# BoyBaykiller/IDKEngine

Measured on NVIDIA H100. Metric: Mrays/s Sponza-sized synthetic 1920x1080 8-bounce, higher is better.
Workload: dtype f32

## Files before the change

### idkengine_b200/csrc/idk_kernels.cuh

```cuda
#pragma once
#include "idk_device.cuh"
#include "../../include/idk_gpu_types.h"

#define IDK_BLOCK 256
#define IDK_WARPS (IDK_BLOCK / 32)
#define IDK_T2_BLOCK 256

struct DeviceScene {
    const float4* nodes;
    const float4* triRec;
    const int4* blasTris;
    const GpuBlasDesc* descs;
    const GpuBlasInstance* instances;
    const float4* xforms;
    const GpuMesh* meshes;
    const GpuMaterial* materials;
    const uint4* vertices;
    const GpuLight* lights;
    uint32_t instanceCount;
    uint32_t lightCount;
    float skyR, skyG, skyB;
    int stackSize;
    const float4* skyFaces;
    int skyFaceSize;
    const float4* tlasNodes;
    int useTlas;
    const float4* vtxFrame;
    const float4* surfRec;
    const struct TexRec* textures;
    uint32_t textureCount;
    const float* srgbLut;
};


#define IDK_TLAS_STACK_SIZE 24

struct __align__(16) PathState {
    float ox, oy, oz, prevIor;
    float pdx, pdy;
    uint32_t pix;
    uint32_t reseed;
    float tx, ty, tz;
    uint32_t rng;
    float rx, ry, rz;
    uint32_t pad;
};
static_assert(sizeof(PathState) == 64, "PathState must be 64 bytes");

struct HitRec { float bx, by, t; uint32_t tri; };

struct TraceCounters { unsigned long long steps, tris, instances, hits; unsigned int maxSteps[64]; };

__global__ void k_init_sample(uint32_t* counts, int nCounts, uint32_t* tickets, int nTickets, uint32_t primaryRays) {
    for (int i = threadIdx.x; i < nCounts; i += blockDim.x) counts[i] = i == 0 ? primaryRays : 0u;
    for (int i = threadIdx.x; i < nTickets; i += blockDim.x) tickets[i] = 0u;
}

__global__ void k_prepare_triangles(const int4* __restrict__ tris, const float* __restrict__ positions,
                                    float4* __restrict__ triRec, uint32_t count) {
    uint32_t i = blockIdx.x * blockDim.x + threadIdx.x;
    if (i >= count) return;
    int4 t = tris[i];
    f3 p0 = mk3(positions[3 * t.x], positions[3 * t.x + 1], positions[3 * t.x + 2]);
    f3 p1 = mk3(positions[3 * t.y], positions[3 * t.y + 1], positions[3 * t.y + 2]);
    f3 p2 = mk3(positions[3 * t.z], positions[3 * t.z + 1], positions[3 * t.z + 2]);
    f3 e1 = p1 - p0, e2 = p2 - p0;
    f3 n = cross3(e1, e2);
    triRec[4 * (size_t)i + 0] = make_float4(p0.x, p0.y, p0.z, e1.x);
    triRec[4 * (size_t)i + 1] = make_float4(e1.y, e1.z, e2.x, e2.y);
    triRec[4 * (size_t)i + 2] = make_float4(e2.z, n.x, n.y, n.z);
    triRec[4 * (size_t)i + 3] = make_float4(0.0f, 0.0f, 0.0f, 0.0f);
}

__global__ void k_prepare_vertices(const uint4* __restrict__ vertices, float4* __restrict__ vtxFrame, uint32_t count) {
    const uint32_t i = blockIdx.x * blockDim.x + threadIdx.x;
    if (i >= count) return;
    const uint4 v = vertices[i];
    const f3 n = decompress_sr11g11b10(v.w), t = decompress_sr11g11b10(v.z);
    vtxFrame[2 * (size_t)i] = make_float4(n.x, n.y, n.z, t.x);
    vtxFrame[2 * (size_t)i + 1] = make_float4(t.y, t.z, 0.0f, 0.0f);
}

__global__ void k_prepare_surfaces(const GpuMesh* __restrict__ meshes, const GpuMaterial* __restrict__ materials,
                                   float4* __restrict__ surfRec, uint32_t meshCount) {
    const uint32_t i = blockIdx.x * blockDim.x + threadIdx.x;
    if (i >= meshCount) return;
    const GpuMesh& mesh = meshes[i];
    const GpuMaterial& mat = materials[mesh.MaterialId];
    const uint32_t c = mat.BaseColorFactor;
    const f3 albedo = mk3((float)(c & 255u) / 255.0f, (float)((c >> 8) & 255u) / 255.0f, (float)((c >> 16) & 255u) / 255.0f);
    const float alpha = (float)((c >> 24) & 255u) / 255.0f;
    f3 emissive = mk3(mat.EmissiveFactor[0], mat.EmissiveFactor[1], mat.EmissiveFactor[2]);
    emissive = emissive * 1.0f + mesh.EmissiveBias * albedo;
    const f3 ab = mk3(mat.Absorbance[0], mat.Absorbance[1], mat.Absorbance[2]) + mk3(mesh.AbsorbanceBias[0], mesh.AbsorbanceBias[1], mesh.AbsorbanceBias[2]);
    const f3 absorbance = mk3(fmaxf(ab.x, 0.0f), fmaxf(ab.y, 0.0f), fmaxf(ab.z, 0.0f));
    const float metallic = clamp1(mat.MetallicFactor + mesh.SpecularBias, 0.0f, 1.0f);
    const float roughness = clamp1(mat.RoughnessFactor + mesh.RoughnessBias, 0.0f, 1.0f);
    const float transmission = clamp1(mat.TransmissionFactor + mesh.TransmissionBias, 0.0f, 1.0f);
    const float ior = fmaxf(mat.IOR + mesh.IORBias, 1.0f);
    const bool textured = (mat.BaseColorTexture | mat.MetallicRoughnessTexture | mat.NormalTexture | mat.EmissiveTexture | mat.TransmissionTexture) != 0;
    const uint32_t flags = (mat.IsVolumetric != 0 ? 1u : 0u) | (mesh.TintOnTransmissive != 0 ? 2u : 0u) | (textured ? 4u : 0u);
    float4* o = surfRec + 5 * (size_t)i;
    o[0] = make_float4(albedo.x, albedo.y, albedo.z, alpha);
    o[1] = make_float4(emissive.x, emissive.y, emissive.z, metallic);
    o[2] = make_float4(absorbance.x, absorbance.y, absorbance.z, roughness);
    o[3] = make_float4(transmission, ior, mat.AlphaCutoff, mesh.NormalMapStrength);
    o[4] = make_float4(__uint_as_float(flags), 0.0f, 0.0f, 0.0f);
}

struct AcceptAll {
    __device__ __forceinline__ bool operator()(const DeviceScene&, uint32_t, float, float, float) const { return true; }
    __device__ __forceinline__ AcceptAll at(const DeviceScene&, uint32_t, f3) const { return *this; }
};
template <bool STATS, bool ANY, class Accept = AcceptAll>
__device__ __forceinline__ bool intersect_blas(const DeviceScene& sc, const float4* nodes, uint32_t triOffset, f3 lo, f3 ld, f3 inv,
                                               bool rootTest, uint32_t* stack, HitRec& hit, uint32_t& S, uint32_t& T, float& cost,
                                               const Accept& accept = Accept()) {
    float tMinLeft, tMinRight;
    if (rootTest) {
        const float4 a = ldg4(nodes + 2), b = ldg4(nodes + 3);
        if (!(ray_box(lo, inv, a, b, tMinLeft) && tMinLeft < hit.t)) return false;
    }
    bool blasHit = false;
    uint32_t sp = 0;
    uint32_t top = 2;
    while (true) {
        if (STATS) { S++; cost += 1.0f; }
        const NodePair pr = ldg_pair(nodes + 2 * (size_t)top);
        const float4 lA = pr.lA, lB = pr.lB, rA = pr.rA, rB = pr.rB;
        const int lChild = __float_as_int(lA.w), lCount = __float_as_int(lB.w);
        const int rChild = __float_as_int(rA.w), rCount = __float_as_int(rB.w);

        const bool hitLeft = ray_box(lo, inv, lA, lB, tMinLeft) && tMinLeft <= hit.t;
        const bool hitRight = ray_box(lo, inv, rA, rB, tMinRight) && tMinRight <= hit.t;

        const bool intersectLeft = hitLeft && lCount > 0;
        const bool intersectRight = hitRight && rCount > 0;
        if (intersectLeft || intersectRight) {
            uint32_t first = intersectLeft ? (uint32_t)lChild : (uint32_t)rChild;
            uint32_t end = !intersectRight ? (uint32_t)(lChild + lCount) : (uint32_t)(rChild + rCount);
            first += triOffset;
            end += triOffset;
            if (STATS) { T += end - first; cost += (float)(end - first) * 1.1f; }
            for (uint32_t i = first; i < end; i++) {
                float4 a, b, c;
                ldg_tri(sc.triRec, i, a, b, c);
                float bx, by, t;
                if (ray_triangle(lo, ld, mk3(a.x, a.y, a.z), mk3(a.w, b.x, b.y), mk3(b.z, b.w, c.x), mk3(c.y, c.z, c.w), bx, by, t) && t < hit.t && accept(sc, i, bx, by, t)) {
                    blasHit = true;
                    hit.tri = i;
                    hit.bx = bx;
                    hit.by = by;
                    hit.t = t;
                    if (ANY) return true;
                }
            }
        }

        const bool traverseLeft = hitLeft && lCount == 0;
        const bool traverseRight = hitRight && rCount == 0;
        if (traverseLeft || traverseRight) {
            if (traverseLeft && traverseRight) {
                const bool leftFirst = ANY || tMinLeft < tMinRight;
                top = leftFirst ? (uint32_t)lChild : (uint32_t)rChild;
                stack[(sp++) * IDK_BLOCK] = leftFirst ? (uint32_t)rChild : (uint32_t)lChild;
            } else {
                top = traverseLeft ? (uint32_t)lChild : (uint32_t)rChild;
            }
        } else {
            if (sp == 0) break;
            top = stack[(--sp) * IDK_BLOCK];
        }
    }
    return blasHit;
}

template <bool STATS, bool ANY, class Accept = AcceptAll>
__device__ __forceinline__ bool trace_instance(const DeviceScene& sc, uint32_t inst, f3 o, f3 d, bool rootTest, uint32_t* stack,
                                               HitRec& hit, uint32_t& hitXform, uint32_t& S, uint32_t& T, uint32_t& I, float& cost,
                                               const Accept& accept = Accept()) {
    const GpuBlasInstance bi = sc.instances[inst];
    const int nodeOffset = sc.descs[bi.BlasId].NodeOffset;
    const uint32_t triOffset = (uint32_t)sc.descs[bi.BlasId].TriangleOffset;
    const float4* xf = sc.xforms + 9 * (size_t)bi.MeshTransformId + 3;
    const float4 r0 = ldg4(xf), r1 = ldg4(xf + 1), r2 = ldg4(xf + 2);
    const f3 lo = xform_point(r0, r1, r2, o);
    const f3 ld = xform_vector(r0, r1, r2, d);
    const f3 inv = mk3(1.0f / ld.x, 1.0f / ld.y, 1.0f / ld.z);
    if (STATS) I++;
    if (!intersect_blas<STATS, ANY>(sc, sc.nodes + 2 * (size_t)nodeOffset, triOffset, lo, ld, inv, rootTest, stack, hit, S, T, cost,
                                    accept.at(sc, bi.MeshTransformId, ld))) return false;
    hitXform = bi.MeshTransformId;
    return true;
}

template <bool STATS, bool ANY, class Accept = AcceptAll>
__device__ __forceinline__ bool trace_ray(const DeviceScene& sc, f3 o, f3 d, float tMax, bool traceLights,
                                          uint32_t* stack, HitRec& hit, uint32_t& hitXform, uint32_t& S, uint32_t& T, uint32_t& I, float& cost,
                                          const Accept& accept = Accept()) {
    hit.t = tMax;
    hit.tri = ~0u;
    hit.bx = 0.0f;
    hit.by = 0.0f;
    hitXform = 0;

    if (traceLights) {
        for (uint32_t i = 0; i < sc.lightCount; i++) {
            const GpuLight& L = sc.lights[i];
            float tMin, tMx;
            if (ray_sphere(o, d, mk3(L.Position[0], L.Position[1], L.Position[2]), L.Radius, tMin, tMx) && tMin < hit.t) {
                hit.t = tMin < 0.0f ? tMx : tMin;
                hitXform = i;
                hit.tri = ~0u;
                if (ANY) return true;
            }
        }
    }

    if (sc.useTlas) {
        const f3 inv = mk3(1.0f / d.x, 1.0f / d.y, 1.0f / d.z);
        uint32_t tstack[IDK_TLAS_STACK_SIZE];
        uint32_t sp = 0, top = 0;
        while (true) {
            const float4 pA = ldg4(sc.tlasNodes + 2 * (size_t)top);
            const uint32_t word = __float_as_uint(pA.w);
            const uint32_t id = word & 0x7FFFFFFFu;
            if (word >> 31) {
                const bool instHit = trace_instance<STATS, ANY>(sc, id, o, d, false, stack, hit, hitXform, S, T, I, cost, accept);
                if (ANY && instHit) return true;
                if (sp == 0) break;
                top = tstack[--sp];
                continue;
            }
            const NodePair pr = ldg_pair(sc.tlasNodes + 2 * (size_t)id);
            const float4 lA = pr.lA, lB = pr.lB, rA = pr.rA, rB = pr.rB;
            float tMinLeft, tMinRight;
            const bool traverseLeft = ray_box(o, inv, lA, lB, tMinLeft) && tMinLeft < hit.t;
            const bool traverseRight = ray_box(o, inv, rA, rB, tMinRight) && tMinRight < hit.t;
            if (traverseLeft || traverseRight) {
                if (traverseLeft && traverseRight) {
                    const bool leftCloser = tMinLeft < tMinRight;
                    top = leftCloser ? id : id + 1;
                    tstack[sp++] = leftCloser ? id + 1 : id;
                } else {
                    top = traverseLeft ? id : id + 1;
                }
            } else {
                if (sp == 0) break;
                top = tstack[--sp];
            }
        }
    } else {
        for (uint32_t inst = 0; inst < sc.instanceCount; inst++) {
            const bool instHit = trace_instance<STATS, ANY>(sc, inst, o, d, true, stack, hit, hitXform, S, T, I, cost, accept);
            if (ANY && instHit) return true;
        }
    }
    return !ANY && hit.t != tMax;
}

struct TraverseArgs {
    DeviceScene sc;
    const PathState* state;
    const uint32_t* perm;
    const uint32_t* count;
    uint32_t* ticket;
    HitRec* hits;
    uint32_t* hitXform;
    float* debugCost;
    TraceCounters* counters;
    int traceLights;
    int bounce;
};

template <bool STATS>
__global__ void __launch_bounds__(IDK_BLOCK) k_traverse(TraverseArgs a) {
    extern __shared__ uint32_t s_stack[];
    uint32_t* stack = s_stack + threadIdx.x;
    const uint32_t lane = threadIdx.x & 31;
    const uint32_t count = *a.count;
    uint32_t S = 0, T = 0, I = 0, H = 0;
    for (;;) {
        uint32_t base = 0;
        if (lane == 0) base = atomicAdd(a.ticket, 32u);
        base = __shfl_sync(0xffffffffu, base, 0);
        if (base >= count) break;
        const uint32_t gid = base + lane;
        if (gid < count) {
            const uint32_t src = a.perm ? a.perm[gid] : gid;
            const float4* sp = reinterpret_cast<const float4*>(a.state + src);
            const float4 s0 = sp[0], s1 = sp[1];
            const f3 o = mk3(s0.x, s0.y, s0.z);
            const f3 d = decode_unit_vec(s1.x, s1.y);
            HitRec hit;
            uint32_t xf;
            float cost = 0.0f;
            const uint32_t stepsBefore = S;
            trace_ray<STATS, false>(a.sc, o, d, IDK_FLOAT_MAX, a.traceLights != 0, stack, hit, xf, S, T, I, cost);
            if (STATS) atomicMax(&a.counters->maxSteps[a.bounce & 63], S - stepsBefore);
            reinterpret_cast<float4*>(a.hits)[gid] = make_float4(hit.bx, hit.by, hit.t, __uint_as_float(hit.tri));
            a.hitXform[gid] = xf;
            if (STATS) {
                a.debugCost[gid] = cost;
                if (hit.tri != ~0u) H++;
            }
        }
    }
    if (STATS) {
        for (int off = 16; off > 0; off >>= 1) {
            S += __shfl_down_sync(0xffffffffu, S, off);
            T += __shfl_down_sync(0xffffffffu, T, off);
            I += __shfl_down_sync(0xffffffffu, I, off);
            H += __shfl_down_sync(0xffffffffu, H, off);
        }
        if (lane == 0) {
            atomicAdd(&a.counters->steps, (unsigned long long)S);
            atomicAdd(&a.counters->tris, (unsigned long long)T);
            atomicAdd(&a.counters->instances, (unsigned long long)I);
            atomicAdd(&a.counters->hits, (unsigned long long)H);
        }
    }
}


struct TraverseTuning { int setupThreshold; int leafThreshold; int packRays; };
#define IDK_T2_SETUP_THRESHOLD 12
#define IDK_T2_LEAF_THRESHOLD 4

template <bool STATS, bool TLAS>
__global__ void __launch_bounds__(IDK_T2_BLOCK) k_traverse2(TraverseArgs a, TraverseTuning tune) {
    extern __shared__ __align__(128) unsigned char s_dyn[];
    const DeviceScene& sc = a.sc;
    uint32_t* stack = reinterpret_cast<uint32_t*>(s_dyn) + threadIdx.x;
    const uint32_t lane = threadIdx.x & 31;
    const uint32_t laneLt = (1u << lane) - 1u;
    const uint32_t count = *a.count;
    enum { ST_SETUP = 0, ST_BOX = 1, ST_LEAF = 2, ST_EXIT = 3, ST_TLAS = 4 };
    const uint32_t totalWarps = gridDim.x * (IDK_T2_BLOCK / 32);
    const uint32_t quota = tune.packRays ? 32u : min(32u, max(1u, (count + totalWarps - 1) / totalWarps));
    const int setupThreshold = max(1, min(tune.setupThreshold, (int)(quota * 3 / 8)));
    const int leafThreshold = max(1, min(tune.leafThreshold, (int)(quota / 8)));

    int state = ST_SETUP;
    bool haveRay = false, finished = false, blasHit = false;
    uint32_t gid = 0, inst = 0, curXf = 0, hitXf = 0;
    f3 wo = mk3(0, 0, 0), wd = mk3(0, 0, 1);
    f3 lo = wo, ld = wd, inv = wd;
    HitRec hit;
    hit.bx = hit.by = 0.0f; hit.t = 0.0f; hit.tri = ~0u;
    const float4* nodes = sc.nodes;
    uint32_t triOffset = 0, top = 2, sp = 0, first = 0, end = 0;
    uint32_t S = 0, T = 0, I = 0, H = 0, rayS0 = 0;
    float cost = 0.0f;
    uint32_t tstack[TLAS ? IDK_TLAS_STACK_SIZE : 1];
    uint32_t tsp = 0, ttop = 0;
    f3 winv = wd;

    for (;;) {
        const uint32_t mBox = __ballot_sync(0xffffffffu, state == ST_BOX);
        const uint32_t mSetup = __ballot_sync(0xffffffffu, state == ST_SETUP);
        const uint32_t mLeaf = __ballot_sync(0xffffffffu, state == ST_LEAF);
        const uint32_t mTlas = TLAS ? __ballot_sync(0xffffffffu, state == ST_TLAS) : 0u;
        if ((mSetup | mBox | mLeaf | mTlas) == 0u) break;

        if (mSetup && (__popc(mSetup) >= setupThreshold || (mBox | mLeaf | mTlas) == 0u)) {
            const bool mine = state == ST_SETUP;
            if (mine && haveRay && inst >= sc.instanceCount) {
                reinterpret_cast<float4*>(a.hits)[gid] = make_float4(hit.bx, hit.by, hit.t, __uint_as_float(hit.tri));
                a.hitXform[gid] = hitXf;
                if (STATS) {
                    a.debugCost[gid] = cost;
                    if (hit.tri != ~0u) H++;
                    atomicMax(&a.counters->maxSteps[a.bounce & 63], S - rayS0);
                }
                haveRay = false;
            }
            const bool needFetch = mine && !haveRay && lane < quota;
            if (mine && !haveRay && lane >= quota) state = ST_EXIT;
            const uint32_t fm = __ballot_sync(0xffffffffu, needFetch);
            if (fm) {
                const int leader = __ffs(fm) - 1;
                uint32_t base = 0;
                if ((int)lane == leader) base = atomicAdd(a.ticket, (uint32_t)__popc(fm));
                base = __shfl_sync(0xffffffffu, base, leader);
                bool got = false;
                float4 s0 = make_float4(0.0f, 0.0f, 0.0f, 0.0f), s1 = s0;
                if (needFetch) {
                    gid = base + __popc(fm & laneLt);
                    if (gid < count) {
                        const uint32_t src = a.perm ? a.perm[gid] : gid;
                        const float4* spp = reinterpret_cast<const float4*>(a.state + src);
                        s0 = spp[0]; s1 = spp[1];
                        got = true;
                    }
                }
                if (needFetch) {
                    if (got) {
                        wo = mk3(s0.x, s0.y, s0.z);
                        wd = decode_unit_vec(s1.x, s1.y);
                        hit.t = IDK_FLOAT_MAX; hit.tri = ~0u; hit.bx = 0.0f; hit.by = 0.0f;
                        hitXf = 0;
                        cost = 0.0f;
                        if (a.traceLights) {
                            for (uint32_t i = 0; i < sc.lightCount; i++) {
                                const GpuLight& L = sc.lights[i];
                                float tMin, tMx;
                                if (ray_sphere(wo, wd, mk3(L.Position[0], L.Position[1], L.Position[2]), L.Radius, tMin, tMx) && tMin < hit.t) {
                                    hit.t = tMin < 0.0f ? tMx : tMin;
                                    hitXf = i;
                                    hit.tri = ~0u;
                                }
                            }
                        }
                        inst = 0;
                        haveRay = true;
                        rayS0 = S;
                        if (TLAS) {
                            winv = mk3(1.0f / wd.x, 1.0f / wd.y, 1.0f / wd.z);
                            ttop = 0; tsp = 0;
                            state = ST_TLAS;
                        }
                    } else {
                        state = ST_EXIT;
                    }
                }
            }
            if (!TLAS && mine && haveRay && inst < sc.instanceCount) {
                const GpuBlasInstance bi = sc.instances[inst];
                const int nodeOffset = sc.descs[bi.BlasId].NodeOffset;
                triOffset = (uint32_t)sc.descs[bi.BlasId].TriangleOffset;
                const float4* xf = sc.xforms + 9 * (size_t)bi.MeshTransformId + 3;
                const float4 r0 = ldg4(xf), r1 = ldg4(xf + 1), r2 = ldg4(xf + 2);
                lo = xform_point(r0, r1, r2, wo);
                ld = xform_vector(r0, r1, r2, wd);
                inv = mk3(1.0f / ld.x, 1.0f / ld.y, 1.0f / ld.z);
                nodes = sc.nodes + 2 * (size_t)nodeOffset;
                curXf = bi.MeshTransformId;
                if (STATS) I++;
                const float4 ra = ldg4(nodes + 2), rb = ldg4(nodes + 3);
                float tRoot;
                if (ray_box(lo, inv, ra, rb, tRoot) && tRoot < hit.t) {
                    state = ST_BOX;
                    top = 2; sp = 0; blasHit = false; finished = false;
                } else {
                    inst++;
                }
            }
        } else if (TLAS && mTlas && (__popc(mTlas) >= setupThreshold || (mBox | mLeaf) == 0u)) {
            if (state == ST_TLAS) {
                const float4 pA = ldg4(sc.tlasNodes + 2 * (size_t)ttop);
                const uint32_t word = __float_as_uint(pA.w);
                const uint32_t id = word & 0x7FFFFFFFu;
                if (word >> 31) {
                    const GpuBlasInstance bi = sc.instances[id];
                    const int nodeOffset = sc.descs[bi.BlasId].NodeOffset;
                    triOffset = (uint32_t)sc.descs[bi.BlasId].TriangleOffset;
                    const float4* xf = sc.xforms + 9 * (size_t)bi.MeshTransformId + 3;
                    const float4 r0 = ldg4(xf), r1 = ldg4(xf + 1), r2 = ldg4(xf + 2);
                    lo = xform_point(r0, r1, r2, wo);
                    ld = xform_vector(r0, r1, r2, wd);
                    inv = mk3(1.0f / ld.x, 1.0f / ld.y, 1.0f / ld.z);
                    nodes = sc.nodes + 2 * (size_t)nodeOffset;
                    curXf = bi.MeshTransformId;
                    if (STATS) I++;
                    state = ST_BOX;
                    top = 2; sp = 0; blasHit = false; finished = false;
                } else {
                    const NodePair pr = ldg_pair(sc.tlasNodes + 2 * (size_t)id);
                    float tMinLeft, tMinRight;
                    const bool traverseLeft = ray_box(wo, winv, pr.lA, pr.lB, tMinLeft) && tMinLeft < hit.t;
                    const bool traverseRight = ray_box(wo, winv, pr.rA, pr.rB, tMinRight) && tMinRight < hit.t;
                    if (traverseLeft || traverseRight) {
                        if (traverseLeft && traverseRight) {
                            const bool leftCloser = tMinLeft < tMinRight;
                            ttop = leftCloser ? id : id + 1;
                            tstack[tsp++] = leftCloser ? id + 1 : id;
                        } else {
                            ttop = traverseLeft ? id : id + 1;
                        }
                    } else if (tsp == 0u) {
                        inst = 0xFFFFFFFFu;
                        state = ST_SETUP;
                    } else {
                        ttop = tstack[--tsp];
                    }
                }
            }
        } else if (mLeaf && (__popc(mLeaf) >= leafThreshold || mBox == 0u)) {
            if (state == ST_LEAF) {
                float4 ta, tb, tc;
                ldg_tri(sc.triRec, first, ta, tb, tc);
                float bx, by, t;
                if (ray_triangle(lo, ld, mk3(ta.x, ta.y, ta.z), mk3(ta.w, tb.x, tb.y), mk3(tb.z, tb.w, tc.x), mk3(tc.y, tc.z, tc.w), bx, by, t) && t < hit.t) {
                    blasHit = true;
                    hit.tri = first; hit.bx = bx; hit.by = by; hit.t = t;
                }
                first++;
                if (first == end) {
                    if (finished) {
                        if (blasHit) hitXf = curXf;
                        if (TLAS) {
                            if (tsp == 0u) { inst = 0xFFFFFFFFu; state = ST_SETUP; }
                            else { ttop = tstack[--tsp]; state = ST_TLAS; }
                        } else { inst++; state = ST_SETUP; }
                    } else {
                        state = ST_BOX;
                    }
                }
            }
        } else {
            if (state == ST_BOX) {
                if (STATS) { S++; cost += 1.0f; }
                const NodePair pr = ldg_pair(nodes + 2 * (size_t)top);
                const float4 lA = pr.lA, lB = pr.lB, rA = pr.rA, rB = pr.rB;
                const int lChild = __float_as_int(lA.w), lCount = __float_as_int(lB.w);
                const int rChild = __float_as_int(rA.w), rCount = __float_as_int(rB.w);
                float tMinLeft, tMinRight;
                const bool hitLeft = ray_box(lo, inv, lA, lB, tMinLeft) && tMinLeft <= hit.t;
                const bool hitRight = ray_box(lo, inv, rA, rB, tMinRight) && tMinRight <= hit.t;
                const bool intersectLeft = hitLeft && lCount > 0;
                const bool intersectRight = hitRight && rCount > 0;
                bool pending = false;
                if (intersectLeft || intersectRight) {
                    first = (intersectLeft ? (uint32_t)lChild : (uint32_t)rChild) + triOffset;
                    end = (!intersectRight ? (uint32_t)(lChild + lCount) : (uint32_t)(rChild + rCount)) + triOffset;
                    if (STATS) { T += end - first; cost += (float)(end - first) * 1.1f; }
                    pending = first < end;
                }
                const bool traverseLeft = hitLeft && lCount == 0;
                const bool traverseRight = hitRight && rCount == 0;
                if (traverseLeft || traverseRight) {
                    if (traverseLeft && traverseRight) {
                        const bool leftCloser = tMinLeft < tMinRight;
                        top = leftCloser ? (uint32_t)lChild : (uint32_t)rChild;
                        stack[(sp++) * IDK_T2_BLOCK] = leftCloser ? (uint32_t)rChild : (uint32_t)lChild;
                    } else {
                        top = traverseLeft ? (uint32_t)lChild : (uint32_t)rChild;
                    }
                } else if (sp == 0u) {
                    finished = true;
                } else {
                    top = stack[(--sp) * IDK_T2_BLOCK];
                }
                if (pending) {
                    state = ST_LEAF;
                } else if (finished) {
                    if (blasHit) hitXf = curXf;
                    if (TLAS) {
                        if (tsp == 0u) { inst = 0xFFFFFFFFu; state = ST_SETUP; }
                        else { ttop = tstack[--tsp]; state = ST_TLAS; }
                    } else { inst++; state = ST_SETUP; }
                }
            }
        }
    }
    if (STATS) {
        for (int off = 16; off > 0; off >>= 1) {
            S += __shfl_down_sync(0xffffffffu, S, off);
            T += __shfl_down_sync(0xffffffffu, T, off);
            I += __shfl_down_sync(0xffffffffu, I, off);
            H += __shfl_down_sync(0xffffffffu, H, off);
        }
        if (lane == 0) {
            atomicAdd(&a.counters->steps, (unsigned long long)S);
            atomicAdd(&a.counters->tris, (unsigned long long)T);
            atomicAdd(&a.counters->instances, (unsigned long long)I);
            atomicAdd(&a.counters->hits, (unsigned long long)H);
        }
    }
}

struct TraceRaysArgs {
    DeviceScene sc;
    const float4* rays;
    uint4* hits;
    uint32_t count;
    uint32_t* ticket;
    int traceLights;
};

__global__ void __launch_bounds__(IDK_BLOCK) k_trace_rays(TraceRaysArgs a) {
    extern __shared__ uint32_t s_stack[];
    uint32_t* stack = s_stack + threadIdx.x;
    const uint32_t lane = threadIdx.x & 31;
    for (;;) {
        uint32_t base = 0;
        if (lane == 0) base = atomicAdd(a.ticket, 32u);
        base = __shfl_sync(0xffffffffu, base, 0);
        if (base >= a.count) break;
        const uint32_t gid = base + lane;
        if (gid < a.count) {
            const float4 r0 = a.rays[2 * (size_t)gid], r1 = a.rays[2 * (size_t)gid + 1];
            HitRec hit;
            uint32_t xf, S = 0, T = 0, I = 0;
            float cost = 0.0f;
            trace_ray<true, false>(a.sc, mk3(r0.x, r0.y, r0.z), mk3(r1.x, r1.y, r1.z), r0.w, a.traceLights != 0, stack, hit, xf, S, T, I, cost);
            a.hits[2 * (size_t)gid] = make_uint4(__float_as_uint(hit.bx), __float_as_uint(hit.by), __float_as_uint(hit.t), hit.tri);
            a.hits[2 * (size_t)gid + 1] = make_uint4(xf, S, T, 0u);
        }
    }
}

struct FrameParams {
    float invProj[16];
    float invView[16];
    float viewPos[3];
    float focalLength, lenseRadius;
    int width, height;
    int stripeH, tileIndex, tileCount;
    uint32_t accumulatedSamples;
    int doDebugTraversal, doTraceLights, doRussianRoulette;
};

__device__ __forceinline__ bool tile_owns_row(const FrameParams& f, int y, int& localRow) {
    const int stripe = y / f.stripeH;
    if (f.tileCount > 1 && (stripe % f.tileCount) != f.tileIndex) return false;
    localRow = (f.tileCount > 1 ? (stripe / f.tileCount) : stripe) * f.stripeH + (y % f.stripeH);
    return true;
}

__global__ void __launch_bounds__(64) k_raygen(FrameParams f, PathState* __restrict__ state) {
    const uint32_t n = 20;
    const uint32_t idx = blockIdx.y * gridDim.x + blockIdx.x;
    const uint32_t columnSize = gridDim.y * n;
    const uint32_t fullColumnCount = gridDim.x / n;
    const uint32_t lastColumnWidth = gridDim.x % n;
    const uint32_t columnIdx = idx / columnSize;
    const uint32_t idxInColumn = idx % columnSize;
    uint32_t columnWidth = n;
    if (columnIdx == fullColumnCount) columnWidth = lastColumnWidth;
    const uint32_t swy = idxInColumn / columnWidth;
    const uint32_t swx = idxInColumn % columnWidth + columnIdx * n;
    const int x = (int)(swx * 8 + threadIdx.x), y = (int)(swy * 8 + threadIdx.y);
    if (x >= f.width || y >= f.height) return;
    int localRow;
    if (!tile_owns_row(f, y, localRow)) return;

    const uint32_t gidX = blockIdx.x * 8 + threadIdx.x, gidY = blockIdx.y * 8 + threadIdx.y;
    uint32_t seed = (uint32_t)(y * 4096 + x) * (f.accumulatedSamples + 1u);
    const float sx = rnd01(seed), sy = rnd01(seed);
    const float ndcx = ((float)x + sx) / (float)f.width * 2.0f - 1.0f;
    const float ndcy = ((float)y + sy) / (float)f.height * 2.0f - 1.0f;
    const float rvx = f.invProj[0] * ndcx + f.invProj[4] * ndcy;
    const float rvy = f.invProj[1] * ndcx + f.invProj[5] * ndcy;
    f3 camDir = normalize3(mat4_mul_xyz(f.invView, rvx, rvy, -1.0f, 0.0f));
    const f3 focalPoint = mk3(f.viewPos[0], f.viewPos[1], f.viewPos[2]) + camDir * f.focalLength;
    float dx, dy;
    sample_disk(seed, dx, dy);
    const f3 pointOnLense = mat4_mul_xyz(f.invView, f.lenseRadius * dx, f.lenseRadius * dy, 0.0f, 1.0f);
    camDir = normalize3(focalPoint - pointOnLense);

    float pdx, pdy;
    encode_unit_vec(camDir, pdx, pdy);
    const uint32_t li = (uint32_t)localRow * (uint32_t)f.width + (uint32_t)x;
    float4* out = reinterpret_cast<float4*>(state + li);
    out[0] = make_float4(pointOnLense.x, pointOnLense.y, pointOnLense.z, 1.0f);
    out[1] = make_float4(pdx, pdy, __uint_as_float(li), __uint_as_float(gidY * 4096u + gidX));
    out[2] = make_float4(1.0f, 1.0f, 1.0f, __uint_as_float(seed));
    out[3] = make_float4(0.0f, 0.0f, 0.0f, 0.0f);
}

struct Surface {
    f3 Albedo; float Alpha;
    f3 Normal, Emissive, Absorbance;
    float Metallic, Roughness, Transmission, IOR, AlphaCutoff;
    bool IsVolumetric, TintOnTransmissive;
};


__device__ __forceinline__ float4 tex_sample(const DeviceScene& sc, unsigned long long handle, float u, float v) {
    return tex_sample_raw(sc.textures, sc.srgbLut, handle, u, v);
}
__device__ __forceinline__ void interp_texcoord(const DeviceScene& sc, int4 tri, float b0, float b1, float b2, float& u, float& v) {
    const uint4 v0 = __ldg(sc.vertices + tri.x), v1 = __ldg(sc.vertices + tri.y), v2 = __ldg(sc.vertices + tri.z);
    u = (__uint_as_float(v0.x) * b0 + __uint_as_float(v1.x) * b1) + __uint_as_float(v2.x) * b2;
    v = (__uint_as_float(v0.y) * b0 + __uint_as_float(v1.y) * b1) + __uint_as_float(v2.y) * b2;
}
__device__ __forceinline__ void surface_textured(const DeviceScene& sc, int meshId, float u, float v, Surface& s) {
    const GpuMesh& mesh = sc.meshes[meshId];
    const GpuMaterial& m = sc.materials[mesh.MaterialId];
    const uint32_t c = m.BaseColorFactor;
    const float4 base = tex_sample(sc, m.BaseColorTexture, u, v);
    s.Albedo = mk3(base.x * ((float)(c & 255u) / 255.0f), base.y * ((float)((c >> 8) & 255u) / 255.0f), base.z * ((float)((c >> 16) & 255u) / 255.0f));
    s.Alpha = base.w * ((float)((c >> 24) & 255u) / 255.0f);
    const float4 nt = tex_sample(sc, m.NormalTexture, u, v);
    s.Normal = mk3(nt.x * 2.0f - 1.0f, nt.y * 2.0f - 1.0f, sqrtf(fmaxf(1.0f - (nt.x * nt.x + nt.y * nt.y), 0.0f)));
    const float4 et = tex_sample(sc, m.EmissiveTexture, u, v);
    s.Emissive = mk3(et.x * m.EmissiveFactor[0], et.y * m.EmissiveFactor[1], et.z * m.EmissiveFactor[2]);
    s.Absorbance = mk3(m.Absorbance[0], m.Absorbance[1], m.Absorbance[2]);
    const float4 mr = tex_sample(sc, m.MetallicRoughnessTexture, u, v);
    s.Metallic = mr.x * m.MetallicFactor;
    s.Roughness = mr.y * m.RoughnessFactor;
    s.Transmission = tex_sample(sc, m.TransmissionTexture, u, v).x * m.TransmissionFactor;
    s.IOR = m.IOR;
    s.AlphaCutoff = m.AlphaCutoff;
    s.IsVolumetric = m.IsVolumetric != 0;
    s.Emissive = s.Emissive * 1.0f + mesh.EmissiveBias * s.Albedo;
    const f3 ab = s.Absorbance + mk3(mesh.AbsorbanceBias[0], mesh.AbsorbanceBias[1], mesh.AbsorbanceBias[2]);
    s.Absorbance = mk3(fmaxf(ab.x, 0.0f), fmaxf(ab.y, 0.0f), fmaxf(ab.z, 0.0f));
    s.Metallic = clamp1(s.Metallic + mesh.SpecularBias, 0.0f, 1.0f);
    s.Roughness = clamp1(s.Roughness + mesh.RoughnessBias, 0.0f, 1.0f);
    s.Transmission = clamp1(s.Transmission + mesh.TransmissionBias, 0.0f, 1.0f);
    s.IOR = fmaxf(s.IOR + mesh.IORBias, 1.0f);
    s.TintOnTransmissive = mesh.TintOnTransmissive != 0;
}

__device__ __forceinline__ void sky_face_to_cube(int face, int sc, int tc, int size, int& X, int& Y, int& Z) {
    switch (face) {
        case 0: X = size; Y = -tc; Z = -sc; break;
        case 1: X = -size; Y = -tc; Z = sc; break;
        case 2: X = sc; Y = size; Z = tc; break;
        case 3: X = sc; Y = -size; Z = -tc; break;
        case 4: X = sc; Y = -tc; Z = size; break;
        default: X = -sc; Y = -tc; Z = -size; break;
    }
}
struct CubeTexel { int face, x, y; };

__device__ __forceinline__ CubeTexel cube_texel_edge(int face, int x, int y, int size) {
    if (x >= 0 && x < size && y >= 0 && y < size) return CubeTexel{face, x, y};
    int s2 = 2 * x + 1 - size, t2 = 2 * y + 1 - size;
    int X, Y, Z;
    sky_face_to_cube(face, s2, t2, size, X, Y, Z);
    if (X > size || X < -size) { X = X > 0 ? size : -size; if (Y == size || Y == -size) Y += Y > 0 ? -1 : 1; else Z += Z > 0 ? -1 : 1; }
    else if (Y > size || Y < -size) { Y = Y > 0 ? size : -size; if (X == size || X == -size) X += X > 0 ? -1 : 1; else Z += Z > 0 ? -1 : 1; }
    else { Z = Z > 0 ? size : -size; if (X == size || X == -size) X += X > 0 ? -1 : 1; else Y += Y > 0 ? -1 : 1; }
    int nf, ns, nt;
    if (X == size) { nf = 0; ns = -Z; nt = -Y; } else if (X == -size) { nf = 1; ns = Z; nt = -Y; }
    else if (Y == size) { nf = 2; ns = X; nt = Z; } else if (Y == -size) { nf = 3; ns = X; nt = -Z; }
    else if (Z == size) { nf = 4; ns = X; nt = -Y; } else { nf = 5; ns = -X; nt = -Y; }
    return CubeTexel{nf, (ns + size - 1) / 2, (nt + size - 1) / 2};
}

__device__ __forceinline__ int cube_face_st(f3 d, float& s, float& t) {
    const float ax = fabsf(d.x), ay = fabsf(d.y), az = fabsf(d.z);
    int face;
    float scc, tc, ma;
    if (ax >= ay && ax >= az) { face = d.x >= 0.0f ? 0 : 1; scc = d.x >= 0.0f ? -d.z : d.z; tc = -d.y; ma = ax; }
    else if (ay >= az) { face = d.y >= 0.0f ? 2 : 3; scc = d.x; tc = d.y >= 0.0f ? d.z : -d.z; ma = ay; }
    else { face = d.z >= 0.0f ? 4 : 5; scc = d.z >= 0.0f ? d.x : -d.x; tc = -d.y; ma = az; }
    s = 0.5f * (scc / ma + 1.0f); t = 0.5f * (tc / ma + 1.0f);
    return face;
}

struct CubeFootprint { CubeTexel t00, t10, t01, t11; float fx, fy; int corner; };
__device__ __forceinline__ CubeFootprint cube_footprint(f3 d, int size) {
    float s, t;
    const int face = cube_face_st(d, s, t);
    const float px = s * (float)size - 0.5f, py = t * (float)size - 0.5f;
    const float fx0 = floorf(px), fy0 = floorf(py);
    CubeFootprint fp;
    fp.fx = px - fx0; fp.fy = py - fy0;
    const int x0 = (int)fx0, x1 = (int)fx0 + 1, y0 = (int)fy0, y1 = (int)fy0 + 1;
    const bool ox0 = x0 < 0, ox1 = x1 >= size, oy0 = y0 < 0, oy1 = y1 >= size;
    fp.corner = -1;
    if ((ox0 || ox1) && (oy0 || oy1)) fp.corner = (ox0 && oy0) ? 0 : (ox1 && oy0) ? 1 : (ox0 && oy1) ? 2 : 3;
    const CubeTexel none = {face, 0, 0};
    fp.t00 = fp.corner == 0 ? none : cube_texel_edge(face, x0, y0, size);
    fp.t10 = fp.corner == 1 ? none : cube_texel_edge(face, x1, y0, size);
    fp.t01 = fp.corner == 2 ? none : cube_texel_edge(face, x0, y1, size);
    fp.t11 = fp.corner == 3 ? none : cube_texel_edge(face, x1, y1, size);
    return fp;
}

__device__ __forceinline__ f3 sky_texel_in(const DeviceScene& sc, CubeTexel c) {
    const float4 t = __ldg(sc.skyFaces + ((size_t)c.face * sc.skyFaceSize + c.y) * sc.skyFaceSize + c.x);
    return mk3(t.x, t.y, t.z);
}

__device__ __forceinline__ f3 sample_sky(const DeviceScene& sc, f3 d) {
    if (sc.skyFaceSize == 0) return mk3(sc.skyR, sc.skyG, sc.skyB);
    const CubeFootprint fp = cube_footprint(d, sc.skyFaceSize);
    const f3 zero = mk3(0, 0, 0);
    f3 t00 = fp.corner == 0 ? zero : sky_texel_in(sc, fp.t00);
    f3 t10 = fp.corner == 1 ? zero : sky_texel_in(sc, fp.t10);
    f3 t01 = fp.corner == 2 ? zero : sky_texel_in(sc, fp.t01);
    f3 t11 = fp.corner == 3 ? zero : sky_texel_in(sc, fp.t11);
    if (fp.corner >= 0) {
        const f3 mean = ((t00 + t10) + (t01 + t11)) / 3.0f;
        if (fp.corner == 0) t00 = mean; else if (fp.corner == 1) t10 = mean; else if (fp.corner == 2) t01 = mean; else t11 = mean;
    }
    const f3 a = mix3(t00, t10, fp.fx);
    const f3 b = mix3(t01, t11, fp.fx);
    return mix3(a, b, fp.fy);
}

struct ShadeArgs {
    DeviceScene sc;
    FrameParams f;
    PathState* state;
    float4* aov;
    const uint32_t* alive;
    const HitRec* hits;
    const uint32_t* hitXform;
    const float* debugCost;
    const uint32_t* count;
    uint32_t* survivors;
    uint32_t* keysTmp;
    float4* radiance;
    float4* aovAlbedoFinal;
    float4* aovNormalFinal;
    const uint32_t* slotDelta;
    uint32_t stripePixels;
    int exportState;
    int firstHit;
    int lastBounce;
    int outputAovs;
};

#define IDK_EPOCH_MASK 0x3FFFFFFFu
__device__ __forceinline__ unsigned long long pack_status(uint32_t epoch, uint32_t flag, uint32_t value) {
    return ((unsigned long long)(epoch & IDK_EPOCH_MASK) << 34) | ((unsigned long long)flag << 32) | value;
}
__device__ __forceinline__ uint32_t status_epoch(unsigned long long sv) { return (uint32_t)(sv >> 34) & IDK_EPOCH_MASK; }

template <bool TEX>
__global__ void __launch_bounds__(IDK_BLOCK, 3) k_shade(ShadeArgs a) {
    const uint32_t count = *a.count;
    const DeviceScene& sc = a.sc;
    const FrameParams& f = a.f;

    for (uint32_t gid = blockIdx.x * blockDim.x + threadIdx.x; gid < count; gid += gridDim.x * blockDim.x) {
        bool survive = false;
        PathState st;
        float4 aov0 = make_float4(0.0f, 0.0f, 0.0f, 1.0f), aov1 = make_float4(0.0f, 0.0f, 0.0f, 0.0f);
        uint32_t sortingKey = 0;
        const uint32_t src = a.alive ? a.alive[gid] : gid;
        {
            {
                const float4* sp = reinterpret_cast<const float4*>(a.state + src);
                float4 v0 = sp[0], v1 = sp[1], v2 = sp[2], v3 = sp[3];
                st.ox = v0.x; st.oy = v0.y; st.oz = v0.z; st.prevIor = v0.w;
                st.pdx = v1.x; st.pdy = v1.y; st.pix = __float_as_uint(v1.z); st.reseed = __float_as_uint(v1.w);
                st.tx = v2.x; st.ty = v2.y; st.tz = v2.z; st.rng = __float_as_uint(v2.w);
                st.rx = v3.x; st.ry = v3.y; st.rz = v3.z; st.pad = 0;
            }
            if (a.outputAovs && !a.firstHit) { aov0 = a.aov[2 * (size_t)src]; aov1 = a.aov[2 * (size_t)src + 1]; }
            const uint32_t slot = (a.slotDelta && !a.firstHit) ? gid + a.slotDelta[src / a.stripePixels] : gid;
            uint32_t rng = a.firstHit ? st.rng : (slot * 4096u + f.accumulatedSamples);
            const uint32_t reseed = a.firstHit ? st.reseed : slot;

            const float4 hv = reinterpret_cast<const float4*>(a.hits)[gid];
            const float hitT = hv.z;
            const uint32_t hitTri = __float_as_uint(hv.w);
            const uint32_t hitXf = a.hitXform[gid];
            const bool hitScene = hitT != IDK_FLOAT_MAX;
            const f3 rayDir = decode_unit_vec(st.pdx, st.pdy);
            f3 origin = mk3(st.ox, st.oy, st.oz);
            f3 thr = mk3(st.tx, st.ty, st.tz);
            f3 rad = mk3(st.rx, st.ry, st.rz);

            if (a.firstHit && f.doDebugTraversal) {
                st.prevIor = a.debugCost[gid];
                survive = false;
            } else if (hitScene) {
                origin = origin + rayDir * hitT;
                Surface s;
                s.Albedo = mk3(1.0f, 1.0f, 1.0f); s.Alpha = 1.0f;
                s.Normal = mk3(0.0f, 0.0f, 0.0f); s.Emissive = mk3(0.0f, 0.0f, 0.0f); s.Absorbance = mk3(0.0f, 0.0f, 0.0f);
                s.Metallic = 0.0f; s.Roughness = 0.0f; s.Transmission = 0.0f; s.IOR = 1.5f; s.AlphaCutoff = 0.5f;
                s.IsVolumetric = false; s.TintOnTransmissive = true;
                f3 geometricNormal = mk3(0.0f, 0.0f, 0.0f);
                bool passThrough = false;
                const bool hitLight = hitTri == ~0u;
                if (!hitLight) {
                    sortingKey = hitTri;
                    const int4 tri = __ldg(sc.blasTris + hitTri);
                    const float4* vf = sc.vtxFrame;
                    const float4 a0 = ldg4(vf + 2 * (size_t)tri.x), a1 = ldg4(vf + 2 * (size_t)tri.x + 1);
                    const float4 c0 = ldg4(vf + 2 * (size_t)tri.y), c1 = ldg4(vf + 2 * (size_t)tri.y + 1);
                    const float4 e0 = ldg4(vf + 2 * (size_t)tri.z), e1 = ldg4(vf + 2 * (size_t)tri.z + 1);
                    const float4* xf = sc.xforms + 9 * (size_t)hitXf + 3;
                    const float4 r0 = ldg4(xf), r1 = ldg4(xf + 1), r2 = ldg4(xf + 2);
                    const float4* sr = sc.surfRec + 5 * (size_t)tri.w;
                    const float4 s0 = ldg4(sr), s1 = ldg4(sr + 1), s2 = ldg4(sr + 2), s3 = ldg4(sr + 3), s4 = ldg4(sr + 4);
                    const float b0 = hv.x, b1 = hv.y, b2 = 1.0f - hv.x - hv.y;
                    const f3 interpNormal = normalize3((mk3(a0.x, a0.y, a0.z) * b0 + mk3(c0.x, c0.y, c0.z) * b1) + mk3(e0.x, e0.y, e0.z) * b2);
                    const f3 interpTangent = normalize3((mk3(a0.w, a1.x, a1.y) * b0 + mk3(c0.w, c1.x, c1.y) * b1) + mk3(e0.w, e1.x, e1.y) * b2);
                    const float normalMapStrength = s3.w;

                    s.Albedo = mk3(s0.x, s0.y, s0.z);
                    s.Alpha = s0.w;
                    s.Normal = mk3(1.0f, 1.0f, 0.0f);
                    s.Emissive = mk3(s1.x, s1.y, s1.z);
                    s.Metallic = s1.w;
                    s.Absorbance = mk3(s2.x, s2.y, s2.z);
                    s.Roughness = s2.w;
                    s.Transmission = s3.x;
                    s.IOR = s3.y;
                    s.AlphaCutoff = s3.z;
                    s.IsVolumetric = (__float_as_uint(s4.x) & 1u) != 0;
                    s.TintOnTransmissive = (__float_as_uint(s4.x) & 2u) != 0;
                    if (TEX && (__float_as_uint(s4.x) & 4u)) {
                        float tu, tv;
                        interp_texcoord(sc, tri, b0, b1, b2, tu, tv);
                        surface_textured(sc, tri.w, tu, tv, s);
                    }

                    const float alphaCutoff = (s.AlphaCutoff == 2.0f) ? rnd01(rng) : s.AlphaCutoff;
                    if (s.Alpha < alphaCutoff) {
                        origin = origin + rayDir * 0.001f;
                        passThrough = true;
                    } else {
                        const f3 worldNormal = normalize3(xform_normal(r0, r1, r2, interpNormal));
                        const f3 worldTangent = normalize3(xform_normal(r0, r1, r2, interpTangent));
                        const f3 N = normalize3(worldNormal);
                        const f3 T = normalize3(worldTangent);
                        const f3 B = normalize3(cross3(N, T));
                        const f3 tbnN = (T * s.Normal.x + B * s.Normal.y) + N * s.Normal.z;
                        s.Normal = normalize3(mix3(worldNormal, tbnN, normalMapStrength));
                        const float4 tr = ldg4(sc.triRec + 4 * (size_t)hitTri + 2);
                        geometricNormal = normalize3(mk3(tr.y, tr.z, tr.w));
                        geometricNormal = normalize3(xform_normal(r0, r1, r2, geometricNormal));
                    }
                } else if (f.doTraceLights) {
                    sortingKey = hitXf;
                    const GpuLight& L = sc.lights[hitXf];
                    s.Emissive = mk3(L.Color[0], L.Color[1], L.Color[2]);
                    s.Albedo = s.Emissive;
                    s.Normal = (origin - mk3(L.Position[0], L.Position[1], L.Position[2])) / L.Radius;
                    geometricNormal = s.Normal;
                }

                if (passThrough) {
                    survive = true;
                } else {
                    float prevIor = a.firstHit ? 1.0f : st.prevIor;
                    const bool fromInside = dot3(-rayDir, geometricNormal) < 0.0f;
                    if (fromInside) {
                        if (a.firstHit) prevIor = s.IOR;
                        geometricNormal = geometricNormal * -1.0f;
                        if (s.IsVolumetric) {
                            const f3 e = -s.Absorbance * hitT;
                            thr = thr * mk3(det_exp(e.x), det_exp(e.y), det_exp(e.z));
                        }
                    }
                    float cosTheta = dot3(-rayDir, s.Normal);
                    if (cosTheta < 0.0f) s.Normal = s.Normal * -1.0f;

                    rad = rad + s.Emissive * thr;

                    Surface m = s;
                    m.Roughness *= m.Roughness;
                    cosTheta = dot3(-rayDir, m.Normal);
                    {
                        const float diffuseChance = 1.0f - m.Metallic - m.Transmission;
                        const float r0f = (prevIor - m.IOR) / (prevIor + m.IOR);
                        const float f0 = r0f * r0f;
                        const float fres = f0 + (1.0f - f0) * pow5f(1.0f - cosTheta);
                        m.Metallic = mix1(m.Metallic, 1.0f, fres);
                        m.Transmission = fmaxf(1.0f - diffuseChance - m.Metallic, 0.0f);
                    }
                    uint32_t bsdfType;
                    {
                        const float rnd = rnd01(rng);
                        if (m.Metallic > rnd) bsdfType = 1u;
                        else if (m.Metallic + m.Transmission > rnd) bsdfType = 2u;
                        else bsdfType = 0u;
                    }
                    f3 diffuseRayDir;
                    {
                        uint32_t tmp = reseed;
                        const float g = 1.32471795724474602596f;
                        const float a1 = 1.0f / g, a2 = 1.0f / (g * g);
                        const float r2u = fract1((float)f.accumulatedSamples * a1), r2v = fract1((float)f.accumulatedSamples * a2);
                        const float po0 = rnd01(tmp), po1 = rnd01(tmp);
                        const float u = fract1(r2u + po0), v = fract1(r2v + po1);
                        diffuseRayDir = normalize3(m.Normal + sample_sphere(u, v));
                    }
                    f3 newDir, bsdf;
                    float newIor;
                    if (bsdfType == 0u) {
                        newDir = diffuseRayDir; newIor = prevIor; bsdf = m.Albedo;
                    } else if (bsdfType == 1u) {
                        newDir = normalize3(mix3(reflect3(rayDir, m.Normal), diffuseRayDir, m.Roughness));
                        bsdf = m.Albedo; newIor = prevIor;
                    } else {
                        newIor = fromInside ? 1.0f : m.IOR;
                        f3 refr;
                        bool tir;
                        if (!m.IsVolumetric) {
                            refr = rayDir; tir = false; newIor = 1.0f;
                        } else {
                            refr = refract3(rayDir, m.Normal, prevIor / newIor);
                            tir = refr.x == 0.0f && refr.y == 0.0f && refr.z == 0.0f;
                            if (tir) { refr = reflect3(rayDir, m.Normal); newIor = prevIor; }
                        }
                        newDir = normalize3(mix3(refr, !tir ? -diffuseRayDir : diffuseRayDir, m.Roughness));
                        const bool gltfWantsTint = m.IsVolumetric || !fromInside;
                        bsdf = (gltfWantsTint && m.TintOnTransmissive) ? m.Albedo : mk3(1.0f, 1.0f, 1.0f);
                    }
                    thr = thr * bsdf;

                    if (a.outputAovs) {
                        const float dc = 1.0f - s.Metallic - s.Transmission;
                        const float weight = dc + s.Metallic * s.Roughness + s.Transmission * s.Roughness;
                        if (a.firstHit) {
                            const f3 al = s.Albedo * weight, no = s.Normal * weight;
                            aov0 = make_float4(al.x, al.y, al.z, 1.0f - weight);
                            aov1 = make_float4(no.x, no.y, no.z, 0.0f);
                        } else {
                            const f3 al = mk3(aov0.x, aov0.y, aov0.z) + aov0.w * s.Albedo * weight;
                            const f3 no = mk3(aov1.x, aov1.y, aov1.z) + aov0.w * s.Normal * weight;
                            aov0 = make_float4(al.x, al.y, al.z, aov0.w * (1.0f - weight));
                            aov1 = make_float4(no.x, no.y, no.z, 0.0f);
                        }
                    }

                    bool terminate = false;
                    if (!a.firstHit && f.doRussianRoulette) {
                        const float p = fmaxf(thr.x, fmaxf(thr.y, thr.z));
                        if (rnd01(rng) > p) terminate = true;
                        else thr = thr / p;
                    }
                    if (!terminate) {
                        if (bsdfType == 2u) geometricNormal = geometricNormal * -1.0f;
                        origin = origin + geometricNormal * 0.001f;
                        st.prevIor = newIor;
                        encode_unit_vec(newDir, st.pdx, st.pdy);
                        survive = true;
                    }
                }
            } else {
                const f3 albedo = sample_sky(sc, rayDir);
                if (a.outputAovs) {
                    const f3 fn = cubemap_face_normal(rayDir);
                    if (a.firstHit) {
                        aov0 = make_float4(albedo.x, albedo.y, albedo.z, 0.0f);
                        aov1 = make_float4(fn.x, fn.y, fn.z, 0.0f);
                    } else {
                        const f3 al = mk3(aov0.x, aov0.y, aov0.z) + aov0.w * albedo;
                        const f3 no = mk3(aov1.x, aov1.y, aov1.z) + aov0.w * fn;
                        aov0 = make_float4(al.x, al.y, al.z, 0.0f);
                        aov1 = make_float4(no.x, no.y, no.z, 0.0f);
                    }
                }
                rad = rad + albedo * thr;
                survive = false;
            }
            st.ox = origin.x; st.oy = origin.y; st.oz = origin.z;
            st.tx = thr.x; st.ty = thr.y; st.tz = thr.z;
            st.rx = rad.x; st.ry = rad.y; st.rz = rad.z;

            if (!survive || a.lastBounce) {
                a.radiance[src] = make_float4(st.rx, st.ry, st.rz, st.prevIor);
                if (a.outputAovs) { a.aovAlbedoFinal[src] = aov0; a.aovNormalFinal[src] = aov1; }
            }
            if ((survive && !a.lastBounce) || a.exportState) {
                float4* op = reinterpret_cast<float4*>(a.state + src);
                op[0] = make_float4(st.ox, st.oy, st.oz, st.prevIor);
                op[1] = make_float4(st.pdx, st.pdy, __uint_as_float(src), 0.0f);
                op[2] = make_float4(st.tx, st.ty, st.tz, 0.0f);
                op[3] = make_float4(st.rx, st.ry, st.rz, 0.0f);
                if (a.outputAovs) { a.aov[2 * (size_t)src] = aov0; a.aov[2 * (size_t)src + 1] = aov1; }
            }
            if (!a.lastBounce) {
                a.survivors[gid] = survive ? src : ~0u;
                if (a.keysTmp) a.keysTmp[gid] = sortingKey & 0x1FFFFFu;
            }
        }
    }
}

#define IDK_COMPACT_ITEMS 8
struct CompactArgs {
    const uint32_t* survivors;
    const uint32_t* keysTmp;
    const uint32_t* count;
    uint32_t* aliveOut;
    uint32_t* keysOut;
    uint32_t* countOut;
    uint32_t* ticket;
    unsigned long long* tileStatus;
    uint32_t epoch;
};

__global__ void __launch_bounds__(IDK_BLOCK) k_compact(CompactArgs a) {
    __shared__ uint32_t s_tile;
    __shared__ uint32_t s_warpCount[IDK_WARPS];
    __shared__ uint32_t s_base;
    const uint32_t count = *a.count;
    const uint32_t tileSize = IDK_BLOCK * IDK_COMPACT_ITEMS;
    const uint32_t numTiles = (count + tileSize - 1) / tileSize;
    const uint32_t lane = threadIdx.x & 31, warp = threadIdx.x >> 5;
    for (;;) {
        __syncthreads();
        if (threadIdx.x == 0) s_tile = atomicAdd(a.ticket, 1u);
        __syncthreads();
        const uint32_t tile = s_tile;
        if (tile >= numTiles) break;
        const uint32_t first = tile * tileSize + threadIdx.x * IDK_COMPACT_ITEMS;
        uint32_t v[IDK_COMPACT_ITEMS];
        uint32_t mine = 0;
#pragma unroll
        for (int i = 0; i < IDK_COMPACT_ITEMS; i++) {
            const uint32_t s = first + i;
            v[i] = s < count ? a.survivors[s] : ~0u;
            mine += v[i] != ~0u ? 1u : 0u;
        }
        uint32_t incl = mine;
#pragma unroll
        for (int off = 1; off < 32; off <<= 1) {
            const uint32_t n = __shfl_up_sync(0xffffffffu, incl, off);
            if ((int)lane >= off) incl += n;
        }
        if (lane == 31) s_warpCount[warp] = incl;
        __syncthreads();
        uint32_t warpOffset = 0, blockTotal = 0;
#pragma unroll
        for (int w = 0; w < IDK_WARPS; w++) {
            const uint32_t c = s_warpCount[w];
            if (w < (int)warp) warpOffset += c;
            blockTotal += c;
        }
        if (threadIdx.x == 0) {
            uint32_t exclusive = 0;
            if (tile > 0) {
                atomicExch(&a.tileStatus[tile], pack_status(a.epoch, 1u, blockTotal));
                int look = (int)tile - 1;
                while (look >= 0) {
                    const unsigned long long sv = *((volatile unsigned long long*)&a.tileStatus[look]);
                    if (status_epoch(sv) != (a.epoch & IDK_EPOCH_MASK)) continue;
                    const uint32_t flag = (uint32_t)(sv >> 32) & 3u;
                    exclusive += (uint32_t)sv;
                    if (flag == 2u) break;
                    look--;
                }
            }
            __threadfence();
            atomicExch(&a.tileStatus[tile], pack_status(a.epoch, 2u, exclusive + blockTotal));
            if (tile == numTiles - 1) *a.countOut = exclusive + blockTotal;
            s_base = exclusive;
        }
        __syncthreads();
        uint32_t dst = s_base + warpOffset + (incl - mine);
#pragma unroll
        for (int i = 0; i < IDK_COMPACT_ITEMS; i++) {
            if (v[i] != ~0u) {
                a.aliveOut[dst] = v[i];
                if (a.keysOut) a.keysOut[dst] = a.keysTmp[first + i];
                dst++;
            }
        }
    }
}

__device__ __forceinline__ f3 turbo_colormap(float x) {
    x = clamp1(x, 0.0f, 1.0f);
    const float v0 = 1.0f, v1 = x, v2 = x * x, v3 = x * x * x;
    const float w0 = v2 * v2, w1 = v3 * v2;
    return mk3((((v0 * 0.13572138f + v1 * 4.61539260f) + v2 * -42.66032258f) + v3 * 132.13108234f) + (w0 * -152.94239396f + w1 * 59.28637943f),
               (((v0 * 0.09140261f + v1 * 2.19418839f) + v2 * 4.84296658f) + v3 * -14.18503333f) + (w0 * 4.27729857f + w1 * 2.82956604f),
               (((v0 * 0.10667330f + v1 * 12.64194608f) + v2 * -60.58204836f) + v3 * 110.36276771f) + (w0 * -89.90310912f + w1 * 27.34824973f));
}

#define IDK_MAX_PEERS 16
struct GatherArgs {
    float4* peerImage[IDK_MAX_PEERS];
    uint32_t* peerFlags[IDK_MAX_PEERS];
    const int* tileRows;
    uint32_t* doneCounter;
    int world, rank, width;
    uint32_t epoch;
};

__global__ void __launch_bounds__(IDK_BLOCK) k_accumulate_scatter(const float4* __restrict__ radiance, float4* __restrict__ result,
                                                                  uint32_t count, uint32_t accumulatedSamples, int debugTraversal,
                                                                  GatherArgs g);

#define IDK_MAX_STRIPES 4096
struct SlotExchangeArgs {
    const uint32_t* alive;
    const uint32_t* count;
    unsigned long long* peerTable[IDK_MAX_PEERS];
    uint32_t* delta;
    uint32_t* timedOut;
    long long timeoutCycles;
    uint32_t epoch;
    int world, rank;
    uint32_t stripePixels, nLocalStripes, nStripes;
};

__global__ void __launch_bounds__(256) k_slot_exchange(SlotExchangeArgs a) {
    __shared__ uint32_t s_val[IDK_MAX_STRIPES + 1];
    __shared__ uint32_t s_start[IDK_MAX_STRIPES / 2 + 2];
    __shared__ uint32_t s_part[256];
    const uint32_t count = *a.count;
    const uint32_t tid = threadIdx.x;
    for (uint32_t t = tid; t <= a.nLocalStripes; t += blockDim.x) {
        uint32_t lo = 0, hi = count;
        if (t == a.nLocalStripes) lo = count;
        else {
            const uint32_t firstPixel = t * a.stripePixels;
            while (lo < hi) {
                const uint32_t mid = (lo + hi) >> 1;
                if (a.alive[mid] < firstPixel) lo = mid + 1; else hi = mid;
            }
        }
        s_start[t] = lo;
    }
    __syncthreads();
    for (uint32_t t = tid; t < a.nLocalStripes; t += blockDim.x) {
        const unsigned long long word = ((unsigned long long)a.epoch << 32) | (unsigned long long)(s_start[t + 1] - s_start[t]);
        for (int p = 0; p < a.world; p++) *((volatile unsigned long long*)&a.peerTable[p][t * (uint32_t)a.world + (uint32_t)a.rank]) = word;
    }
    __threadfence_system();
    const unsigned long long* mine = a.peerTable[a.rank];
    const long long t0 = clock64();
    for (uint32_t s = tid; s < a.nStripes; s += blockDim.x) {
        unsigned long long w;
        for (;;) {
            w = *((volatile const unsigned long long*)&mine[s]);
            if ((uint32_t)(w >> 32) == a.epoch) break;
            if (clock64() - t0 > a.timeoutCycles) { *a.timedOut = 2u; w = 0; break; }
        }
        s_val[s] = (uint32_t)w;
    }
    __syncthreads();
    const uint32_t chunk = (a.nStripes + blockDim.x - 1) / blockDim.x;
    const uint32_t c0 = min(tid * chunk, a.nStripes), c1 = min(c0 + chunk, a.nStripes);
    uint32_t sum = 0;
    for (uint32_t s = c0; s < c1; s++) sum += s_val[s];
    s_part[tid] = sum;
    __syncthreads();
    if (tid == 0) {
        uint32_t run = 0;
        for (uint32_t i = 0; i < blockDim.x; i++) { const uint32_t v = s_part[i]; s_part[i] = run; run += v; }
    }
    __syncthreads();
    uint32_t run = s_part[tid];
    for (uint32_t s = c0; s < c1; s++) { const uint32_t v = s_val[s]; s_val[s] = run; run += v; }
    __syncthreads();
    for (uint32_t t = tid; t < a.nLocalStripes; t += blockDim.x) a.delta[t] = s_val[t * (uint32_t)a.world + (uint32_t)a.rank] - s_start[t];
}

__global__ void __launch_bounds__(32) k_gather_wait(const uint32_t* flags, int world, uint32_t epoch, uint32_t* timedOut, long long timeoutCycles) {
    const int p = threadIdx.x;
    if (p < world) {
        const long long t0 = clock64();
        while (*((volatile const uint32_t*)&flags[p]) != epoch) {
            if (clock64() - t0 > timeoutCycles) { *timedOut = 1u; break; }
        }
    }
    __threadfence_system();
}

__global__ void __launch_bounds__(IDK_BLOCK) k_accumulate(const float4* __restrict__ radiance, const float4* __restrict__ aovAlbedo,
                                                          const float4* __restrict__ aovNormal, float4* __restrict__ result,
                                                          float4* __restrict__ albedo, float4* __restrict__ normal,
                                                          uint32_t count, uint32_t accumulatedSamples, int debugTraversal, int outputAovs) {
    const float w = 1.0f / ((float)accumulatedSamples + 1.0f);
    for (uint32_t i = blockIdx.x * blockDim.x + threadIdx.x; i < count; i += gridDim.x * blockDim.x) {
        const float4 r = radiance[i];
        f3 nr = mk3(r.x, r.y, r.z);
        if (debugTraversal) nr = turbo_colormap(r.w / 150.0f);
        const float4 last = result[i];
        const f3 o = mix3(mk3(last.x, last.y, last.z), nr, w);
        result[i] = make_float4(o.x, o.y, o.z, 1.0f);
        if (outputAovs) {
            const float4 la = albedo[i], ln = normal[i], a = aovAlbedo[i], n = aovNormal[i];
            const f3 oa = mix3(mk3(la.x, la.y, la.z), mk3(a.x, a.y, a.z), w);
            const f3 on = mix3(mk3(ln.x, ln.y, ln.z), mk3(n.x, n.y, n.z), w);
            albedo[i] = make_float4(oa.x, oa.y, oa.z, 1.0f);
            normal[i] = make_float4(on.x, on.y, on.z, 1.0f);
        }
    }
}


__global__ void __launch_bounds__(IDK_BLOCK) k_accumulate_scatter(const float4* __restrict__ radiance, float4* __restrict__ result,
                                                                  uint32_t count, uint32_t accumulatedSamples, int debugTraversal,
                                                                  GatherArgs g) {
    __shared__ bool s_last;
    const float w = 1.0f / ((float)accumulatedSamples + 1.0f);
    for (uint32_t i = blockIdx.x * blockDim.x + threadIdx.x; i < count; i += gridDim.x * blockDim.x) {
        const float4 r = radiance[i];
        f3 nr = mk3(r.x, r.y, r.z);
        if (debugTraversal) nr = turbo_colormap(r.w / 150.0f);
        const float4 last = result[i];
        const f3 o = mix3(mk3(last.x, last.y, last.z), nr, w);
        const float4 v = make_float4(o.x, o.y, o.z, 1.0f);
        result[i] = v;
        const uint32_t row = i / (uint32_t)g.width, x = i - row * (uint32_t)g.width;
        const size_t dst = (size_t)g.tileRows[row] * (size_t)g.width + x;
        for (int p = 0; p < g.world; p++) g.peerImage[p][dst] = v;
    }
    __threadfence_system();
    __syncthreads();
    if (threadIdx.x == 0) s_last = atomicAdd(g.doneCounter, 1u) == gridDim.x - 1;
    __syncthreads();
    if (s_last) {
        __threadfence_system();
        if ((int)threadIdx.x < g.world) {
            *((volatile uint32_t*)&g.peerFlags[threadIdx.x][g.rank]) = g.epoch;
            __threadfence_system();
        }
    }
}

__global__ void __launch_bounds__(IDK_BLOCK) k_accumulate_aov(const float4* __restrict__ aovAlbedo, const float4* __restrict__ aovNormal,
                                                              float4* __restrict__ albedo, float4* __restrict__ normal,
                                                              uint32_t count, uint32_t accumulatedSamples) {
    const float w = 1.0f / ((float)accumulatedSamples + 1.0f);
    for (uint32_t i = blockIdx.x * blockDim.x + threadIdx.x; i < count; i += gridDim.x * blockDim.x) {
        const float4 la = albedo[i], ln = normal[i], a = aovAlbedo[i], n = aovNormal[i];
        const f3 oa = mix3(mk3(la.x, la.y, la.z), mk3(a.x, a.y, a.z), w);
        const f3 on = mix3(mk3(ln.x, ln.y, ln.z), mk3(n.x, n.y, n.z), w);
        albedo[i] = make_float4(oa.x, oa.y, oa.z, 1.0f);
        normal[i] = make_float4(on.x, on.y, on.z, 1.0f);
    }
}
```

### idkengine_b200/csrc/idkpt.cu

```cuda
#include <cuda_runtime.h>
#include <stdio.h>
#include <stdlib.h>
#include <string.h>
#include <string>
#include <vector>
#include <algorithm>
#include <cmath>

#include "../../include/idkpt.h"
#include "idk_kernels.cuh"
#include "idk_sort.cuh"
#include "idk_shadows.cuh"
#include "idk_dynamic.cuh"
#include "idk_post.cuh"
#include "idk_point_shadows.cuh"
#include "idk_volumetric.cuh"
#include "idk_deferred.cuh"
#include "idk_ssr_taa.cuh"
#include "idk_vrs.cuh"
#include "idk_gbuffer.cuh"
#include "idk_transparency.cuh"
#include "idk_lights_skybox.cuh"
#include "idk_textures_host.h"

#define IDKPT_ABI_VERSION 4u

struct DevBuf {
    void* p = nullptr;
    size_t bytes = 0;
};

struct IdkCtxBase {
    int device = 0;
    int smCount = 132;
    cudaStream_t stream = nullptr;
    std::string lastError;
    cudaEvent_t timing[4] = {};
};

struct TextureTable {
    DevBuf pixels, recs, srgbLut;
};

#define IDK_MAX_LANES 16

struct Lane {
    cudaStream_t stream = nullptr;
    cudaEvent_t radianceReady = nullptr;
    cudaEvent_t accDone = nullptr;
    bool accPending = false;
    bool allocated = false;
    DevBuf state, aov, alive[2], survivors, keysTmp, sortedAlive, hits, hitXform, debugCost, radiance, aovAlbedoFinal, aovNormalFinal;
    DevBuf countsDev;
    DevBuf tickets;
    DevBuf tileStatus;
    uint32_t epoch = 0;
    DevBuf keys;
    IdkSortScratch sortScratch;
    DevBuf slotDelta;
    uint32_t slotEpoch = 0;
};

struct IdkPtCtx : IdkCtxBase {
    static inline thread_local std::string createError;

    int width = 0, height = 0;
    int stripeH = 8, tileIndex = 0, tileCount = 1;
    std::vector<int> rows;
    uint32_t nLocal = 0;
    uint32_t accumulatedSamples = 0;

    bool haveScene = false;
    DeviceScene sc = {};
    IdkPtSceneDesc counts = {};
    DevBuf nodes, triRec, blasTris, positions, descs, instances, xforms, meshes, materials, vertices, lights, tlas, vtxFrame, surfRec;
    std::vector<GpuLight> hostLights;
    float sky[3] = {0.0f, 0.0f, 0.0f};
    DevBuf skyFaces;
    int skyFaceSize = 0;
    TextureTable tex;
    std::vector<uint64_t> hostMaterialMaxHandle;

    DevBuf scratch[3];

    std::vector<GpuPointShadow> pointShadows;
    std::vector<int32_t> pointShadowSizes;
    std::vector<PointShadowDev> pointShadowRecs;
    DevBuf pointShadowDev, pointShadowMaps;
    DevBuf pointShadowLights;

    DevBuf volMarch, volDepth, volOut;
    int volW = 0, volH = 0;

    DevBuf gbufStage, rtStage, rtPtrs, ssaoOut, deferredOut;
    int ssaoW = 0, ssaoH = 0;
    int deferredW = 0, deferredH = 0;

    DevBuf ssrOut, ssrMerged, taaHist[2];
    int ssrW = 0, ssrH = 0;
    int taaW = 0, taaH = 0;
    int taaFrame = 0;
    int taaLast = -1;

    DevBuf vrsRates, vrsDebug, vrsOffsets;
    int vrsW = 0, vrsH = 0;

    DevBuf gbImages, gbPrev;
    int gbW = 0, gbH = 0;

    DevBuf bloomDown, bloomUp, postConsts, ldr;
    DevBuf oidn[4], denoiseWork[2], denoised;
    bool haveDenoised = false;

    DevBuf unskinned, joints, refitParents, refitLocks, tlasScratch;
    uint64_t unskinnedCount = 0;
    std::vector<uint32_t> unskinnedMaxJoint;
    std::vector<GpuBlasDesc> hostDescs;
    size_t nodeBytes = 0;

    Lane lanes[IDK_MAX_LANES];
    int laneCount = 8;
    int nextLane = 0;
    bool asyncPending = false;
    DevBuf images[3];
    DevBuf counters;
    DevBuf countLog;
    uint32_t epochStart = 0;
    uint32_t slotEpochStart = 0;
    bool exportEnabled = false;

    int traverseBlocks = 0, traverseBlocksStats = 0, shadeBlocks = 0, traceRaysBlocks = 0, compactBlocks = 0;
    int traverse1Blocks = 0, traverse1BlocksStats = 0;
    int traverseBlocksLane = 0, traverse1BlocksLane = 0;
    size_t stackBytes = 0;
    size_t traverse2Smem = 0;

    std::vector<cudaEvent_t> events;
    cudaStreamAttrValue l2Window = {};

    int gatherWorld = 0, gatherRank = 0;
    DevBuf gatherImage[2], gatherFlags[2], gatherRows, gatherScratch;
    void* peerImage[2][IDK_MAX_PEERS] = {};
    void* peerFlags[2][IDK_MAX_PEERS] = {};
    bool peerMapped[IDK_MAX_PEERS] = {};
    uint32_t gatherEpoch = 0;
    double gatherTimeoutMs = 30000.0;
    int clockKHz = 1980000;
    int gatherCurrent = -1;
    bool peerIsIpc = false;
    bool globalSlots = false;
    int nStripes = 0, nLocalStripes = 0;
    DevBuf slotTable;
    void* peerSlotTable[IDK_MAX_PEERS] = {};

    cudaStream_t copyStream = nullptr;
    cudaEvent_t snapDone = nullptr, copyDone = nullptr;
    DevBuf presentSnap;
    bool copyPending = false;
};

#define CK(call)                                                                                   \
    do {                                                                                           \
        cudaError_t e_ = (call);                                                                   \
        if (e_ != cudaSuccess) {                                                                   \
            char buf_[512];                                                                        \
            snprintf(buf_, sizeof(buf_), "%s failed: %s (%s:%d)", #call, cudaGetErrorString(e_), __FILE__, __LINE__); \
            ctx->lastError = buf_;                                                                 \
            return IDKPT_ERR_CUDA;                                                                 \
        }                                                                                          \
    } while (0)

template <class Ctx> static int fail(Ctx* ctx, int code, const char* msg) {
    (ctx ? ctx->lastError : Ctx::createError) = msg;
    return code;
}

static int fail(IdkCtxBase* ctx, const char* who, int code, const char* what) {
    ctx->lastError = std::string(who) + ": " + what;
    return code;
}

static cudaError_t ensure(DevBuf& b, size_t bytes) {
    if (bytes <= b.bytes && b.p) return cudaSuccess;
    if (b.p) cudaFree(b.p);
    b.p = nullptr;
    b.bytes = 0;
    if (bytes == 0) return cudaSuccess;
    cudaError_t e = cudaMalloc(&b.p, bytes);
    if (e == cudaSuccess) b.bytes = bytes;
    return e;
}

static void release(DevBuf& b) {
    if (b.p) cudaFree(b.p);
    b.p = nullptr;
    b.bytes = 0;
}

static int upload(IdkCtxBase* ctx, DevBuf& b, const void* src, size_t bytes) {
    CK(ensure(b, std::max<size_t>(bytes, 16)));
    if (bytes) CK(cudaMemcpyAsync(b.p, src, bytes, cudaMemcpyHostToDevice, ctx->stream));
    return IDKPT_OK;
}

static int create_stream(IdkCtxBase* ctx) {
    CK(cudaStreamCreateWithFlags(&ctx->stream, cudaStreamNonBlocking));
    for (cudaEvent_t& e : ctx->timing) CK(cudaEventCreate(&e));
    return IDKPT_OK;
}

static void destroy_stream(IdkCtxBase* ctx) {
    for (cudaEvent_t e : ctx->timing) if (e) cudaEventDestroy(e);
    if (ctx->stream) cudaStreamDestroy(ctx->stream);
}

template <class Work>
static int run_timed(IdkCtxBase* ctx, const char* who, float* ms, Work&& work, void* dst = nullptr, const void* src = nullptr, size_t bytes = 0) {
    CK(cudaEventRecord(ctx->timing[0], ctx->stream));
    if (int rc = work()) return rc;
    cudaError_t e = cudaGetLastError();
    if (e == cudaSuccess) {
        CK(cudaEventRecord(ctx->timing[1], ctx->stream));
        if (dst) CK(cudaMemcpyAsync(dst, src, bytes, cudaMemcpyDeviceToHost, ctx->stream));
        e = cudaStreamSynchronize(ctx->stream);
    }
    if (e != cudaSuccess) return fail(ctx, who, IDKPT_ERR_CUDA, cudaGetErrorString(e));
    if (ms) CK(cudaEventElapsedTime(ms, ctx->timing[0], ctx->timing[1]));
    return IDKPT_OK;
}

static void compute_tile_rows(IdkPtCtx* ctx) {
    ctx->rows.clear();
    for (int y = 0; y < ctx->height; y++)
        if (ctx->tileCount <= 1 || ((y / ctx->stripeH) % ctx->tileCount) == ctx->tileIndex) ctx->rows.push_back(y);
    ctx->nLocal = (uint32_t)(ctx->rows.size() * (size_t)ctx->width);
    ctx->nStripes = (ctx->height + ctx->stripeH - 1) / ctx->stripeH;
    ctx->nLocalStripes = 0;
    for (int s = 0; s < ctx->nStripes; s++)
        if (ctx->tileCount <= 1 || (s % ctx->tileCount) == ctx->tileIndex) ctx->nLocalStripes++;
}

static int configure_launches(IdkPtCtx* ctx) {
    const int stackSize = std::max(1, ctx->sc.stackSize);
    ctx->stackBytes = (size_t)stackSize * IDK_BLOCK * sizeof(uint32_t);
    if (ctx->stackBytes > 200 * 1024) return fail(ctx, IDKPT_ERR_UNSUPPORTED, "BlasStackSize too large for the shared-memory traversal stack");
    CK(cudaFuncSetAttribute(k_traverse<false>, cudaFuncAttributeMaxDynamicSharedMemorySize, (int)ctx->stackBytes));
    CK(cudaFuncSetAttribute(k_traverse<true>, cudaFuncAttributeMaxDynamicSharedMemorySize, (int)ctx->stackBytes));
    CK(cudaFuncSetAttribute(k_trace_rays, cudaFuncAttributeMaxDynamicSharedMemorySize, (int)ctx->stackBytes));
    CK(cudaFuncSetAttribute(k_trace_rays_any, cudaFuncAttributeMaxDynamicSharedMemorySize, (int)ctx->stackBytes));
    CK(cudaFuncSetAttribute(k_shadows_ray_traced, cudaFuncAttributeMaxDynamicSharedMemorySize, (int)ctx->stackBytes));
    CK(cudaFuncSetAttribute(k_point_shadow_faces, cudaFuncAttributeMaxDynamicSharedMemorySize, (int)ctx->stackBytes));
    CK(cudaFuncSetAttribute(k_gbuffer, cudaFuncAttributeMaxDynamicSharedMemorySize, (int)ctx->stackBytes));
    CK(cudaFuncSetAttribute(k_transparency<false>, cudaFuncAttributeMaxDynamicSharedMemorySize, (int)ctx->stackBytes));
    CK(cudaFuncSetAttribute(k_transparency<true>, cudaFuncAttributeMaxDynamicSharedMemorySize, (int)ctx->stackBytes));
    ctx->traverse2Smem = (size_t)stackSize * IDK_T2_BLOCK * sizeof(uint32_t);
    CK(cudaFuncSetAttribute(k_traverse2<false, false>, cudaFuncAttributeMaxDynamicSharedMemorySize, (int)ctx->traverse2Smem));
    CK(cudaFuncSetAttribute(k_traverse2<true, false>, cudaFuncAttributeMaxDynamicSharedMemorySize, (int)ctx->traverse2Smem));
    CK(cudaFuncSetAttribute(k_traverse2<false, true>, cudaFuncAttributeMaxDynamicSharedMemorySize, (int)ctx->traverse2Smem));
    CK(cudaFuncSetAttribute(k_traverse2<true, true>, cudaFuncAttributeMaxDynamicSharedMemorySize, (int)ctx->traverse2Smem));
    int n = 0;
    CK(cudaOccupancyMaxActiveBlocksPerMultiprocessor(&n, k_traverse<false>, IDK_BLOCK, ctx->stackBytes));
    ctx->traverse1Blocks = std::max(1, n) * ctx->smCount;
    CK(cudaOccupancyMaxActiveBlocksPerMultiprocessor(&n, k_traverse<true>, IDK_BLOCK, ctx->stackBytes));
    ctx->traverse1BlocksStats = std::max(1, n) * ctx->smCount;
    if (ctx->sc.useTlas) {
        CK(cudaOccupancyMaxActiveBlocksPerMultiprocessor(&n, k_traverse2<false, true>, IDK_T2_BLOCK, ctx->traverse2Smem));
        ctx->traverseBlocks = std::max(1, n) * ctx->smCount;
        CK(cudaOccupancyMaxActiveBlocksPerMultiprocessor(&n, k_traverse2<true, true>, IDK_T2_BLOCK, ctx->traverse2Smem));
        ctx->traverseBlocksStats = std::max(1, n) * ctx->smCount;
    } else {
        CK(cudaOccupancyMaxActiveBlocksPerMultiprocessor(&n, k_traverse2<false, false>, IDK_T2_BLOCK, ctx->traverse2Smem));
        ctx->traverseBlocks = std::max(1, n) * ctx->smCount;
        CK(cudaOccupancyMaxActiveBlocksPerMultiprocessor(&n, k_traverse2<true, false>, IDK_T2_BLOCK, ctx->traverse2Smem));
        ctx->traverseBlocksStats = std::max(1, n) * ctx->smCount;
    }
    CK(cudaOccupancyMaxActiveBlocksPerMultiprocessor(&n, k_trace_rays, IDK_BLOCK, ctx->stackBytes));
    ctx->traceRaysBlocks = std::max(1, n) * ctx->smCount;
    CK(cudaOccupancyMaxActiveBlocksPerMultiprocessor(&n, k_shade<false>, IDK_BLOCK, 0));
    ctx->shadeBlocks = std::max(1, n) * ctx->smCount;
    CK(cudaOccupancyMaxActiveBlocksPerMultiprocessor(&n, k_compact, IDK_BLOCK, 0));
    ctx->compactBlocks = std::max(1, std::min(n, 4)) * ctx->smCount;
    {
        const int lanes = std::max(1, ctx->laneCount);
        const int perSm2 = (ctx->traverseBlocks / ctx->smCount + lanes - 1) / lanes, perSm1 = (ctx->traverse1Blocks / ctx->smCount + lanes - 1) / lanes;
        ctx->traverseBlocksLane = std::max(1, perSm2) * ctx->smCount;
        ctx->traverse1BlocksLane = std::max(1, perSm1) * ctx->smCount;
    }
    return IDKPT_OK;
}

static int allocate_lane(IdkPtCtx* ctx, Lane& ln) {
    const size_t n = std::max<uint32_t>(ctx->nLocal, 1);
    CK(ensure(ln.state, n * sizeof(PathState)));
    CK(ensure(ln.aov, n * 32));
    for (int i = 0; i < 2; i++) CK(ensure(ln.alive[i], n * 4));
    CK(ensure(ln.survivors, n * 4));
    CK(ensure(ln.hits, n * 16));
    CK(ensure(ln.hitXform, n * 4));
    CK(ensure(ln.debugCost, n * 4));
    CK(ensure(ln.radiance, n * 16));
    CK(ensure(ln.aovAlbedoFinal, n * 16));
    CK(ensure(ln.aovNormalFinal, n * 16));
    CK(ensure(ln.countsDev, (IDKPT_MAX_RAY_DEPTH + 1) * sizeof(uint32_t)));
    CK(ensure(ln.tickets, 2 * (IDKPT_MAX_RAY_DEPTH + 1) * sizeof(uint32_t)));
    CK(ensure(ln.tileStatus, ((n + IDK_BLOCK * IDK_COMPACT_ITEMS - 1) / (IDK_BLOCK * IDK_COMPACT_ITEMS) + 1) * sizeof(unsigned long long)));
    if (ctx->globalSlots && ctx->tileCount > 1) CK(ensure(ln.slotDelta, (size_t)std::max(1, ctx->nLocalStripes) * sizeof(uint32_t)));
    CK(cudaMemsetAsync(ln.tileStatus.p, 0, ln.tileStatus.bytes, ctx->stream));
    if (!ln.stream) CK(cudaStreamCreateWithFlags(&ln.stream, cudaStreamNonBlocking));
    if (!ln.radianceReady) CK(cudaEventCreateWithFlags(&ln.radianceReady, cudaEventDisableTiming));
    if (!ln.accDone) CK(cudaEventCreateWithFlags(&ln.accDone, cudaEventDisableTiming));
    CK(cudaStreamSynchronize(ctx->stream));
    ln.epoch = ctx->epochStart;
    CK(cudaStreamSetAttribute(ln.stream, cudaStreamAttributeAccessPolicyWindow, &ctx->l2Window));
    ln.accPending = false;
    ln.allocated = true;
    return IDKPT_OK;
}

static void release_lane(Lane& ln, bool keepStream) {
    DevBuf* all[] = {&ln.state, &ln.aov, &ln.alive[0], &ln.alive[1], &ln.survivors, &ln.keysTmp, &ln.sortedAlive, &ln.hits, &ln.hitXform, &ln.debugCost,
                     &ln.radiance, &ln.aovAlbedoFinal, &ln.aovNormalFinal, &ln.countsDev, &ln.tickets, &ln.tileStatus, &ln.keys, &ln.slotDelta};
    for (DevBuf* b : all) release(*b);
    idk_sort_release(ln.sortScratch);
    ln.allocated = false;
    ln.accPending = false;
    if (!keepStream) {
        if (ln.stream) { cudaStreamDestroy(ln.stream); ln.stream = nullptr; }
        if (ln.radianceReady) { cudaEventDestroy(ln.radianceReady); ln.radianceReady = nullptr; }
        if (ln.accDone) { cudaEventDestroy(ln.accDone); ln.accDone = nullptr; }
    }
}

static cudaError_t drain(IdkPtCtx* ctx) {
    cudaError_t first = cudaSuccess;
    for (int i = 0; i < IDK_MAX_LANES; i++)
        if (ctx->lanes[i].stream) { cudaError_t e = cudaStreamSynchronize(ctx->lanes[i].stream); if (first == cudaSuccess) first = e; }
    if (ctx->stream) { cudaError_t e = cudaStreamSynchronize(ctx->stream); if (first == cudaSuccess) first = e; }
    for (int i = 0; i < IDK_MAX_LANES; i++) ctx->lanes[i].accPending = false;
    ctx->asyncPending = false;
    return first;
}

static int check_device_errors(IdkPtCtx* ctx, cudaError_t se, const char* who) {
    if (se != cudaSuccess) {
        ctx->lastError = std::string(who) + ": kernel execution failed: " + cudaGetErrorString(se);
        return IDKPT_ERR_CUDA;
    }
    if (ctx->gatherWorld > 1) {
        uint32_t timedOut = 0;
        CK(cudaMemcpy(&timedOut, (uint32_t*)ctx->gatherScratch.p + 1, 4, cudaMemcpyDeviceToHost));
        if (timedOut) {
            cudaMemset((uint32_t*)ctx->gatherScratch.p + 1, 0, 4);
            return fail(ctx, IDKPT_ERR_CUDA, timedOut == 2u ? "idkpt_compute: timed out waiting for a peer rank's per-stripe alive counts (multi-GPU global slots)"
                                                            : "idkpt_compute: timed out waiting for a peer rank's tile (multi-GPU gather)");
        }
    }
    return IDKPT_OK;
}

#define DRAIN_PENDING(who)                                                         \
    do {                                                                           \
        if (ctx->asyncPending) {                                                   \
            cudaSetDevice(ctx->device);                                            \
            int rc_ = check_device_errors(ctx, drain(ctx), who);                   \
            if (rc_) return rc_;                                                   \
        }                                                                          \
    } while (0)

static int allocate_wavefront(IdkPtCtx* ctx) {
    const size_t n = std::max<uint32_t>(ctx->nLocal, 1);
    for (int i = 1; i < IDK_MAX_LANES; i++) if (ctx->lanes[i].allocated) release_lane(ctx->lanes[i], true);
    int rc = allocate_lane(ctx, ctx->lanes[0]);
    if (rc) return rc;
    for (int i = 0; i < 3; i++) {
        CK(ensure(ctx->images[i], n * 16));
        CK(cudaMemsetAsync(ctx->images[i].p, 0, n * 16, ctx->stream));
    }
    CK(ensure(ctx->counters, sizeof(TraceCounters)));
    return IDKPT_OK;
}

static const char* validate_material_textures(const GpuMaterial& m, uint64_t textureCount, const char* msg) {
    const uint64_t h[5] = {m.BaseColorTexture, m.MetallicRoughnessTexture, m.NormalTexture, m.EmissiveTexture, m.TransmissionTexture};
    for (int i = 0; i < 5; i++) if (h[i] > textureCount) return msg;
    return nullptr;
}

static uint64_t material_max_handle(const GpuMaterial& m) {
    return std::max(std::max(std::max(m.BaseColorTexture, m.MetallicRoughnessTexture), std::max(m.NormalTexture, m.EmissiveTexture)), m.TransmissionTexture);
}

static int upload_textures(IdkCtxBase* ctx, TextureTable& t, const IdkPtTextureDesc* textures, uint64_t count) {
    IdkPtSceneDesc tmp = {};
    tmp.Textures = textures; tmp.TextureCount = count;
    const std::vector<size_t> off = idk_texture_offsets(&tmp);
    CK(ensure(t.pixels, std::max<size_t>(off[count], 16)));
    std::vector<TexRec> recs;
    CK(idk_upload_texture_table(textures, count, off, t.pixels.p, ctx->stream, recs));
    int rc;
    if ((rc = upload(ctx, t.recs, recs.data(), recs.size() * sizeof(TexRec)))) return rc;
    float lut[256];
    idk_srgb_lut(lut);
    if ((rc = upload(ctx, t.srgbLut, lut, sizeof(lut)))) return rc;
    CK(cudaStreamSynchronize(ctx->stream));
    return IDKPT_OK;
}

static int texture_error(IdkCtxBase* ctx, const char* who, const char* terr) {
    return fail(ctx, who, strstr(terr, "not supported") ? IDKPT_ERR_UNSUPPORTED : IDKPT_ERR_INVALID_ARGUMENT, terr);
}

static int validate_scene(IdkCtxBase* ctx, const char* who, const IdkPtSceneDesc* s) {
    if (!s->BlasTriangles || !s->BlasDescs || !s->BlasInstances || !s->MeshTransforms || !s->Meshes || !s->Materials || !s->Vertices || !s->VertexPositions)
        return fail(ctx, who, IDKPT_ERR_INVALID_ARGUMENT, "a required array is null");
    if (s->LightCount > IDK_GPU_MAX_UBO_LIGHT_COUNT) return fail(ctx, who, IDKPT_ERR_INVALID_ARGUMENT, "more than 256 lights");
    for (uint64_t i = 0; i < s->BlasInstanceCount; i++)
        if (s->BlasInstances[i].BlasId >= s->BlasDescCount || s->BlasInstances[i].MeshTransformId >= s->MeshTransformCount)
            return fail(ctx, who, IDKPT_ERR_INVALID_ARGUMENT, "BlasInstance references a missing BLAS or transform");
    for (uint64_t i = 0; i < s->BlasDescCount; i++) {
        const GpuBlasDesc& d = s->BlasDescs[i];
        if (d.TriangleOffset < 0 || d.TriangleCount < 0 || (uint64_t)d.TriangleOffset + d.TriangleCount > s->BlasTriangleCount)
            return fail(ctx, who, IDKPT_ERR_INVALID_ARGUMENT, "GpuBlasDesc triangle range outside the array");
    }
    const uint64_t lim = std::min(s->VertexPositionCount, s->VertexCount);
    for (uint64_t i = 0; i < s->BlasTriangleCount; i++) {
        const GpuBlasTriangle& t = s->BlasTriangles[i];
        if ((uint64_t)(uint32_t)t.X >= lim || (uint64_t)(uint32_t)t.Y >= lim || (uint64_t)(uint32_t)t.Z >= lim || t.MeshId < 0 || (uint64_t)t.MeshId >= s->MeshCount)
            return fail(ctx, who, IDKPT_ERR_INVALID_ARGUMENT, "GpuBlasTriangle index out of range");
    }
    for (uint64_t i = 0; i < s->MeshCount; i++)
        if (s->Meshes[i].MaterialId < 0 || (uint64_t)s->Meshes[i].MaterialId >= s->MaterialCount) return fail(ctx, who, IDKPT_ERR_INVALID_ARGUMENT, "GpuMesh.MaterialId out of range");
    if (const char* terr = idk_validate_textures(s)) return texture_error(ctx, who, terr);
    return IDKPT_OK;
}

static bool tlas_nodes_valid(const GpuTlasNode* t, uint64_t first, uint64_t count, uint64_t nodeCount, uint64_t instanceCount) {
    for (uint64_t i = 0; i < count; i++) {
        const uint32_t w = t[i].IsLeafAndChildOrInstanceId, id = w & 0x7FFFFFFFu;
        if ((w >> 31) ? (id >= instanceCount) : (id <= first + i || (uint64_t)id + 1 >= nodeCount)) return false;
    }
    return true;
}

static const char* validate_blas(const GpuBlasNode* nodes, const GpuBlasDesc& d, int blasStackSize) {
    const int n = d.NodeCount;
    if (n < 4 || (n & 1)) return "idkpt_set_scene: BLAS node count must be even and >= 4";
    if (nodes[1].TriCount != 0 || nodes[1].TriStartOrChild != 2) return "idkpt_set_scene: BLAS root must be interior with children at 2 (BLAS.cs:16-22)";
    std::vector<int> req((size_t)n / 2, 0);
    for (int p = n / 2 - 1; p >= 1; p--) {
        int need[2] = {-1, -1};
        for (int c = 0; c < 2; c++) {
            const GpuBlasNode& nd = nodes[2 * p + c];
            if (nd.TriCount > 0) {
                if (nd.TriStartOrChild < 0 || (int64_t)nd.TriStartOrChild + nd.TriCount > d.TriangleCount) return "idkpt_set_scene: BLAS leaf triangle range outside the BLAS";
            } else if (nd.TriCount == 0) {
                const int ch = nd.TriStartOrChild;
                if (ch <= 2 * p || (ch & 1) || ch + 1 >= n) return "idkpt_set_scene: BLAS child index out of range / not in DFS order";
                need[c] = req[(size_t)ch / 2];
            } else {
                return "idkpt_set_scene: negative TriCount in a BLAS node";
            }
        }
        req[p] = (need[0] >= 0 && need[1] >= 0) ? std::max(need[0], need[1]) + 1 : std::max(need[0], std::max(need[1], 0));
    }
    if (req[1] > blasStackSize) return "idkpt_set_scene: BlasStackSize smaller than the traversal stack this BLAS needs";
    return nullptr;
}

static int tlas_height(const GpuTlasNode* t, uint64_t count) {
    std::vector<int> need(count, 0);
    for (int64_t i = (int64_t)count - 1; i >= 0; i--) {
        const uint32_t w = t[i].IsLeafAndChildOrInstanceId, c = w & 0x7FFFFFFFu;
        need[i] = (w >> 31) ? 0 : 1 + std::max(need[c], need[c + 1]);
    }
    return count ? need[0] : 0;
}

static void gather_teardown(IdkPtCtx* ctx) {
    for (int b = 0; b < 2; b++)
        for (int p = 0; p < IDK_MAX_PEERS; p++) {
            if (ctx->peerMapped[p] && p != ctx->gatherRank && ctx->peerIsIpc) {
                if (ctx->peerImage[b][p]) cudaIpcCloseMemHandle(ctx->peerImage[b][p]);
                if (ctx->peerFlags[b][p]) cudaIpcCloseMemHandle(ctx->peerFlags[b][p]);
            }
            ctx->peerImage[b][p] = nullptr;
            ctx->peerFlags[b][p] = nullptr;
        }
    for (int p = 0; p < IDK_MAX_PEERS; p++) {
        if (ctx->peerMapped[p] && p != ctx->gatherRank && ctx->peerIsIpc && ctx->peerSlotTable[p]) cudaIpcCloseMemHandle(ctx->peerSlotTable[p]);
        ctx->peerSlotTable[p] = nullptr;
        ctx->peerMapped[p] = false;
    }
    ctx->peerIsIpc = false;
    release(ctx->slotTable);
    for (int i = 0; i < IDK_MAX_LANES; i++) ctx->lanes[i].slotEpoch = 0;
    for (int b = 0; b < 2; b++) { release(ctx->gatherImage[b]); release(ctx->gatherFlags[b]); }
    release(ctx->gatherRows);
    release(ctx->gatherScratch);
    ctx->gatherWorld = 0;
    ctx->gatherCurrent = -1;
    ctx->gatherEpoch = 0;
}

static int upload_sphere_mesh(IdkPtCtx* ctx) {
    float3 vertices[IDK_SPHERE_VERTICES];
    uint32_t triangles[IDK_SPHERE_TRIANGLES];
    sphere_mesh_tables(vertices, triangles);
    CK(cudaMemcpyToSymbolAsync(c_sphere_vertices, vertices, sizeof(vertices), 0, cudaMemcpyHostToDevice, ctx->stream));
    CK(cudaMemcpyToSymbolAsync(c_sphere_triangles, triangles, sizeof(triangles), 0, cudaMemcpyHostToDevice, ctx->stream));
    CK(cudaStreamSynchronize(ctx->stream));
    return IDKPT_OK;
}

extern "C" {

IDKPT_API uint32_t idkpt_abi_version(void) { return IDKPT_ABI_VERSION; }

IDKPT_API const char* idkpt_last_error(IdkPtCtx* ctx) { return ctx ? ctx->lastError.c_str() : IdkPtCtx::createError.c_str(); }

IDKPT_API int idkpt_create(const IdkPtCreateInfo* ci, IdkPtCtx** out) {
    if (!ci || !out) return fail<IdkPtCtx>(nullptr, IDKPT_ERR_INVALID_ARGUMENT, "idkpt_create: null argument");
    *out = nullptr;
    if (ci->Width <= 0 || ci->Height <= 0 || ci->Width > 4096 * 4 || ci->Height > 4096 * 4)
        return fail<IdkPtCtx>(nullptr, IDKPT_ERR_INVALID_ARGUMENT, "idkpt_create: invalid image size");
    int stripe = ci->TileStripeHeight > 0 ? ci->TileStripeHeight : 8;
    int tcount = ci->TileCount > 1 ? ci->TileCount : 1;
    if ((ci->Flags & IDKPT_CREATE_GLOBAL_SLOTS) && tcount > 1 && (ci->Height + stripe - 1) / stripe > IDK_MAX_STRIPES)
        return fail<IdkPtCtx>(nullptr, IDKPT_ERR_UNSUPPORTED, "idkpt_create: IDKPT_CREATE_GLOBAL_SLOTS supports at most 4096 stripes (raise TileStripeHeight)");
    if (tcount > 1 && (ci->TileIndex < 0 || ci->TileIndex >= tcount))
        return fail<IdkPtCtx>(nullptr, IDKPT_ERR_INVALID_ARGUMENT, "idkpt_create: TileIndex out of range");
    int deviceCount = 0;
    cudaError_t e = cudaGetDeviceCount(&deviceCount);
    if (e != cudaSuccess || deviceCount == 0)
        return fail<IdkPtCtx>(nullptr, IDKPT_ERR_NO_DEVICE, "idkpt_create: no CUDA device (libidkpt has no CPU fallback)");
    if (ci->Device < 0 || ci->Device >= deviceCount)
        return fail<IdkPtCtx>(nullptr, IDKPT_ERR_INVALID_ARGUMENT, "idkpt_create: device ordinal out of range");
    if (cudaSetDevice(ci->Device) != cudaSuccess) return fail<IdkPtCtx>(nullptr, IDKPT_ERR_CUDA, "idkpt_create: cudaSetDevice failed");
    cudaDeviceProp prop;
    if (cudaGetDeviceProperties(&prop, ci->Device) != cudaSuccess) return fail<IdkPtCtx>(nullptr, IDKPT_ERR_CUDA, "idkpt_create: cudaGetDeviceProperties failed");
    if (prop.major != 9 || prop.minor != 0) {
        char buf[512];
        snprintf(buf, sizeof(buf), "idkpt_create: device '%s' is sm_%d%d; libidkpt is built for sm_90a only", prop.name, prop.major, prop.minor);
        return fail<IdkPtCtx>(nullptr, IDKPT_ERR_NO_DEVICE, buf);
    }
    IdkPtCtx* ctx = new IdkPtCtx();
    ctx->device = ci->Device;
    ctx->smCount = prop.multiProcessorCount;
    ctx->width = ci->Width;
    ctx->height = ci->Height;
    ctx->stripeH = stripe;
    ctx->tileIndex = tcount > 1 ? ci->TileIndex : 0;
    ctx->tileCount = tcount;
    if (const int fl = (ci->Flags >> 8) & 15) ctx->laneCount = std::min(IDK_MAX_LANES, fl);
    ctx->globalSlots = (ci->Flags & IDKPT_CREATE_GLOBAL_SLOTS) != 0;
    if (const char* v = getenv("IDKPT_LANES")) ctx->laneCount = std::max(1, std::min(IDK_MAX_LANES, atoi(v)));
    if (const char* v = getenv("IDKPT_DEBUG_EPOCH_START")) ctx->epochStart = (uint32_t)strtoul(v, nullptr, 0) & IDK_EPOCH_MASK;
    if (const char* v = getenv("IDKPT_DEBUG_SLOT_EPOCH_START")) ctx->slotEpochStart = (uint32_t)strtoul(v, nullptr, 0) & ~1u;
    if (const char* v = getenv("IDKPT_GATHER_TIMEOUT_MS")) ctx->gatherTimeoutMs = std::max(1.0, atof(v));
    ctx->clockKHz = prop.clockRate;
    compute_tile_rows(ctx);
    int rc = create_stream(ctx);
    if (rc == IDKPT_OK) rc = allocate_wavefront(ctx);
    if (rc == IDKPT_OK) rc = upload_sphere_mesh(ctx);
    if (rc != IDKPT_OK) {
        IdkPtCtx::createError = ctx->lastError;
        idkpt_destroy(ctx);
        return rc;
    }
    ctx->sky[0] = ctx->sky[1] = ctx->sky[2] = 0.0f;
    *out = ctx;
    return IDKPT_OK;
}

IDKPT_API void idkpt_destroy(IdkPtCtx* ctx) {
    if (!ctx) return;
    cudaSetDevice(ctx->device);
    drain(ctx);
    DevBuf* all[] = {&ctx->nodes, &ctx->triRec, &ctx->blasTris, &ctx->positions, &ctx->descs, &ctx->instances, &ctx->xforms,
                     &ctx->meshes, &ctx->materials, &ctx->vertices, &ctx->lights, &ctx->tlas, &ctx->vtxFrame, &ctx->surfRec,
                     &ctx->images[0], &ctx->images[1], &ctx->images[2], &ctx->counters, &ctx->countLog, &ctx->skyFaces,
                     &ctx->tex.pixels, &ctx->tex.recs, &ctx->tex.srgbLut, &ctx->bloomDown, &ctx->bloomUp, &ctx->postConsts, &ctx->ldr,
                     &ctx->unskinned, &ctx->joints, &ctx->refitParents, &ctx->refitLocks, &ctx->scratch[0], &ctx->scratch[1], &ctx->scratch[2],
                     &ctx->tlasScratch, &ctx->oidn[0], &ctx->oidn[1], &ctx->oidn[2], &ctx->oidn[3], &ctx->denoiseWork[0], &ctx->denoiseWork[1], &ctx->denoised,
                     &ctx->pointShadowDev, &ctx->pointShadowMaps, &ctx->pointShadowLights, &ctx->volMarch, &ctx->volDepth, &ctx->volOut,
                     &ctx->gbufStage, &ctx->rtStage, &ctx->rtPtrs, &ctx->ssaoOut, &ctx->deferredOut,
                     &ctx->ssrOut, &ctx->ssrMerged, &ctx->taaHist[0], &ctx->taaHist[1], &ctx->vrsRates, &ctx->vrsDebug, &ctx->vrsOffsets,
                     &ctx->gbImages, &ctx->gbPrev};
    for (DevBuf* b : all) release(*b);
    for (int i = 0; i < IDK_MAX_LANES; i++) release_lane(ctx->lanes[i], false);
// ... 56 lines not shown
    if ((rc = upload(ctx, ctx->positions, s->VertexPositions, s->VertexPositionCount * sizeof(PackedVec3)))) return rc;
    if ((rc = upload(ctx, ctx->descs, s->BlasDescs, s->BlasDescCount * sizeof(GpuBlasDesc)))) return rc;
    if ((rc = upload(ctx, ctx->instances, s->BlasInstances, s->BlasInstanceCount * sizeof(GpuBlasInstance)))) return rc;
    if ((rc = upload(ctx, ctx->xforms, s->MeshTransforms, s->MeshTransformCount * sizeof(GpuMeshTransform)))) return rc;
    if ((rc = upload(ctx, ctx->meshes, s->Meshes, s->MeshCount * sizeof(GpuMesh)))) return rc;
    if ((rc = upload(ctx, ctx->materials, s->Materials, s->MaterialCount * sizeof(GpuMaterial)))) return rc;
    if ((rc = upload(ctx, ctx->vertices, s->Vertices, s->VertexCount * sizeof(GpuVertex)))) return rc;
    if ((rc = upload(ctx, ctx->lights, s->Lights, s->LightCount * sizeof(GpuLight)))) return rc;
    if ((rc = upload(ctx, ctx->tlas, s->TlasNodes, s->UseTlas ? s->TlasNodeCount * sizeof(GpuTlasNode) : 0))) return rc;
    if ((rc = upload_textures(ctx, ctx->tex, s->Textures, s->TextureCount))) return rc;
    ctx->hostMaterialMaxHandle.assign(s->MaterialCount, 0);
    for (uint64_t i = 0; i < s->MaterialCount; i++) ctx->hostMaterialMaxHandle[i] = material_max_handle(s->Materials[i]);

    CK(ensure(ctx->vtxFrame, std::max<size_t>(s->VertexCount, 1) * 32));
    CK(ensure(ctx->surfRec, std::max<size_t>(s->MeshCount, 1) * 80));
    if (s->VertexCount) {
        const uint32_t nv = (uint32_t)s->VertexCount;
        k_prepare_vertices<<<(nv + 255) / 256, 256, 0, ctx->stream>>>((const uint4*)ctx->vertices.p, (float4*)ctx->vtxFrame.p, nv);
    }
    if (s->MeshCount) {
        const uint32_t nm = (uint32_t)s->MeshCount;
        k_prepare_surfaces<<<(nm + 255) / 256, 256, 0, ctx->stream>>>((const GpuMesh*)ctx->meshes.p, (const GpuMaterial*)ctx->materials.p, (float4*)ctx->surfRec.p, nm);
    }
    CK(cudaGetLastError());
    if (s->BlasTriangleCount) {
        const uint32_t n = (uint32_t)s->BlasTriangleCount;
        k_prepare_triangles<<<(n + 255) / 256, 256, 0, ctx->stream>>>((const int4*)ctx->blasTris.p, (const float*)ctx->positions.p, (float4*)((char*)ctx->nodes.p + nodeBytes), n);
        CK(cudaGetLastError());
    }

    DeviceScene& sc = ctx->sc;
    sc.nodes = (const float4*)ctx->nodes.p;
    sc.triRec = (const float4*)((char*)ctx->nodes.p + nodeBytes);
    sc.blasTris = (const int4*)ctx->blasTris.p;
    sc.descs = (const GpuBlasDesc*)ctx->descs.p;
    sc.instances = (const GpuBlasInstance*)ctx->instances.p;
    sc.xforms = (const float4*)ctx->xforms.p;
    sc.meshes = (const GpuMesh*)ctx->meshes.p;
    sc.materials = (const GpuMaterial*)ctx->materials.p;
    sc.vertices = (const uint4*)ctx->vertices.p;
    sc.lights = (const GpuLight*)ctx->lights.p;
    sc.instanceCount = (uint32_t)s->BlasInstanceCount;
    sc.lightCount = (uint32_t)s->LightCount;
    sc.skyR = ctx->sky[0]; sc.skyG = ctx->sky[1]; sc.skyB = ctx->sky[2];
    sc.skyFaces = ctx->skyFaceSize ? (const float4*)ctx->skyFaces.p : nullptr;
    sc.skyFaceSize = ctx->skyFaceSize;
    sc.stackSize = std::max(1, s->BlasStackSize);
    sc.tlasNodes = (const float4*)ctx->tlas.p;
    sc.useTlas = s->UseTlas ? 1 : 0;
    sc.vtxFrame = (const float4*)ctx->vtxFrame.p;
    sc.surfRec = (const float4*)ctx->surfRec.p;
    sc.textures = (const TexRec*)ctx->tex.recs.p;
    sc.textureCount = (uint32_t)s->TextureCount;
    sc.srgbLut = (const float*)ctx->tex.srgbLut.p;
    ctx->counts = *s;
    ctx->hostLights.assign(s->Lights, s->Lights + s->LightCount);
    ctx->hostDescs.assign(s->BlasDescs, s->BlasDescs + s->BlasDescCount);
    ctx->nodeBytes = nodeBytes;
    if ((rc = configure_launches(ctx))) return rc;
    {
        cudaDeviceProp prop;
        CK(cudaGetDeviceProperties(&prop, ctx->device));
        cudaStreamAttrValue& attr = ctx->l2Window;
        memset(&attr, 0, sizeof(attr));
        if (prop.persistingL2CacheMaxSize > 0 && prop.accessPolicyMaxWindowSize > 0) {
            const size_t bvhBytes = nodeBytes + triRecBytes;
            const size_t setAside = std::min<size_t>((size_t)prop.persistingL2CacheMaxSize, std::max<size_t>(bvhBytes, 1 << 20));
            CK(cudaDeviceSetLimit(cudaLimitPersistingL2CacheSize, setAside));
            const size_t window = std::min<size_t>(bvhBytes, (size_t)prop.accessPolicyMaxWindowSize);
            attr.accessPolicyWindow.base_ptr = ctx->nodes.p;
            attr.accessPolicyWindow.num_bytes = window;
            attr.accessPolicyWindow.hitRatio = window <= setAside ? 1.0f : (float)((double)setAside / (double)window);
            attr.accessPolicyWindow.hitProp = cudaAccessPropertyPersisting;
            attr.accessPolicyWindow.missProp = cudaAccessPropertyNormal;
        } else {
            attr.accessPolicyWindow.num_bytes = 0;
        }
        CK(cudaStreamSetAttribute(ctx->stream, cudaStreamAttributeAccessPolicyWindow, &attr));
        for (int i = 0; i < IDK_MAX_LANES; i++)
            if (ctx->lanes[i].stream) CK(cudaStreamSetAttribute(ctx->lanes[i].stream, cudaStreamAttributeAccessPolicyWindow, &attr));
    }
    CK(cudaStreamSynchronize(ctx->stream));
    ctx->haveScene = true;
    ctx->accumulatedSamples = 0;
    return IDKPT_OK;
}

IDKPT_API int idkpt_update_range(IdkPtCtx* ctx, IdkPtArrayId which, uint64_t first, uint64_t count, const void* data) {
    if (!ctx || !data) return fail(ctx, IDKPT_ERR_INVALID_ARGUMENT, "idkpt_update_range: null argument");
    DRAIN_PENDING("idkpt_update_range");
    if (!ctx->haveScene) return fail(ctx, IDKPT_ERR_NO_SCENE, "idkpt_update_range: no scene");
    CK(cudaSetDevice(ctx->device));
    DevBuf* b = nullptr;
    size_t elem = 0;
    uint64_t limit = 0;
    switch (which) {
        case IDKPT_ARRAY_MESH_TRANSFORMS: b = &ctx->xforms; elem = sizeof(GpuMeshTransform); limit = ctx->counts.MeshTransformCount; break;
        case IDKPT_ARRAY_MESHES: b = &ctx->meshes; elem = sizeof(GpuMesh); limit = ctx->counts.MeshCount; break;
        case IDKPT_ARRAY_MATERIALS: b = &ctx->materials; elem = sizeof(GpuMaterial); limit = ctx->counts.MaterialCount; break;
        case IDKPT_ARRAY_LIGHTS: b = &ctx->lights; elem = sizeof(GpuLight); limit = ctx->counts.LightCount; break;
        case IDKPT_ARRAY_TLAS_NODES: b = &ctx->tlas; elem = sizeof(GpuTlasNode); limit = ctx->counts.UseTlas ? ctx->counts.TlasNodeCount : 0; break;
        default: return fail(ctx, IDKPT_ERR_INVALID_ARGUMENT, "idkpt_update_range: unknown array id");
    }
    if (first > limit || count > limit - first) return fail(ctx, IDKPT_ERR_INVALID_ARGUMENT, "idkpt_update_range: range outside the array");
    if (which == IDKPT_ARRAY_MESHES) {
        const GpuMesh* m = (const GpuMesh*)data;
        for (uint64_t i = 0; i < count; i++)
            if (m[i].MaterialId < 0 || (uint64_t)m[i].MaterialId >= ctx->counts.MaterialCount)
                return fail(ctx, IDKPT_ERR_INVALID_ARGUMENT, "idkpt_update_range: GpuMesh.MaterialId out of range");
    }
    if (which == IDKPT_ARRAY_TLAS_NODES) {
        const GpuTlasNode* t = (const GpuTlasNode*)data;
        if (!tlas_nodes_valid(t, first, count, ctx->counts.TlasNodeCount, ctx->counts.BlasInstanceCount))
            return fail(ctx, IDKPT_ERR_INVALID_ARGUMENT, "idkpt_update_range: malformed TLAS node (child / instance id out of range)");
        if (first == 0 && count == ctx->counts.TlasNodeCount && tlas_height(t, count) > IDK_TLAS_STACK_SIZE)
            return fail(ctx, IDKPT_ERR_UNSUPPORTED, "idkpt_update_range: TLAS deeper than the 24-entry traversal stack of the TLAS walk (BVHIntersect.glsl:4)");
    }
    if (which == IDKPT_ARRAY_MATERIALS) {
        const GpuMaterial* m = (const GpuMaterial*)data;
        for (uint64_t i = 0; i < count; i++)
            if (const char* err = validate_material_textures(m[i], ctx->counts.TextureCount, "idkpt_update_range: material texture handle outside the texture table"))
                return fail(ctx, IDKPT_ERR_INVALID_ARGUMENT, err);
        for (uint64_t i = 0; i < count; i++) ctx->hostMaterialMaxHandle[first + i] = material_max_handle(m[i]);
    }
    CK(cudaMemcpyAsync((char*)b->p + first * elem, data, count * elem, cudaMemcpyHostToDevice, ctx->stream));
    if (which == IDKPT_ARRAY_LIGHTS) std::copy((const GpuLight*)data, (const GpuLight*)data + count, ctx->hostLights.begin() + first);
    if ((which == IDKPT_ARRAY_MESHES || which == IDKPT_ARRAY_MATERIALS) && ctx->counts.MeshCount) {
        const uint32_t nm = (uint32_t)ctx->counts.MeshCount;
        k_prepare_surfaces<<<(nm + 255) / 256, 256, 0, ctx->stream>>>((const GpuMesh*)ctx->meshes.p, (const GpuMaterial*)ctx->materials.p, (float4*)ctx->surfRec.p, nm);
        CK(cudaGetLastError());
    }
    CK(cudaStreamSynchronize(ctx->stream));
    ctx->accumulatedSamples = 0;
    return IDKPT_OK;
}

IDKPT_API int idkpt_set_sky(IdkPtCtx* ctx, const IdkPtSkyDesc* sky) {
    if (!ctx || !sky) return fail(ctx, IDKPT_ERR_INVALID_ARGUMENT, "idkpt_set_sky: null argument");
    DRAIN_PENDING("idkpt_set_sky");
    if (sky->FaceSize < 0 || sky->FaceSize > 8192) return fail(ctx, IDKPT_ERR_INVALID_ARGUMENT, "idkpt_set_sky: invalid FaceSize");
    CK(cudaSetDevice(ctx->device));
    if (sky->FaceSize > 0) {
        const size_t faceBytes = (size_t)sky->FaceSize * sky->FaceSize * 16;
        for (int i = 0; i < 6; i++) if (!sky->Faces[i]) return fail(ctx, IDKPT_ERR_INVALID_ARGUMENT, "idkpt_set_sky: a cubemap face is null");
        CK(ensure(ctx->skyFaces, 6 * faceBytes));
        for (int i = 0; i < 6; i++) CK(cudaMemcpyAsync((char*)ctx->skyFaces.p + i * faceBytes, sky->Faces[i], faceBytes, cudaMemcpyHostToDevice, ctx->stream));
        CK(cudaStreamSynchronize(ctx->stream));
    }
    ctx->skyFaceSize = sky->FaceSize;
    for (int i = 0; i < 3; i++) ctx->sky[i] = sky->Color[i];
    ctx->sc.skyR = ctx->sky[0]; ctx->sc.skyG = ctx->sky[1]; ctx->sc.skyB = ctx->sky[2];
    ctx->sc.skyFaces = ctx->skyFaceSize ? (const float4*)ctx->skyFaces.p : nullptr;
    ctx->sc.skyFaceSize = ctx->skyFaceSize;
    ctx->accumulatedSamples = 0;
    return IDKPT_OK;
}

IDKPT_API int idkpt_set_textures(IdkPtCtx* ctx, const IdkPtTextureDesc* textures, uint64_t count) {
    if (!ctx || (!textures && count)) return fail(ctx, IDKPT_ERR_INVALID_ARGUMENT, "idkpt_set_textures: null argument");
    DRAIN_PENDING("idkpt_set_textures");
    if (!ctx->haveScene) return fail(ctx, IDKPT_ERR_NO_SCENE, "idkpt_set_textures: no scene");
    IdkPtSceneDesc tmp = {};
    tmp.Textures = textures; tmp.TextureCount = count;
    if (const char* terr = idk_validate_textures(&tmp)) return texture_error(ctx, "idkpt_set_textures", terr);
    for (uint64_t h : ctx->hostMaterialMaxHandle)
        if (h > count) return fail(ctx, IDKPT_ERR_INVALID_ARGUMENT, "idkpt_set_textures: a material references a texture beyond the new table");
    CK(cudaSetDevice(ctx->device));
    CK(cudaStreamSynchronize(ctx->stream));
    int rc = upload_textures(ctx, ctx->tex, textures, count);
    if (rc) return rc;
    ctx->sc.textures = (const TexRec*)ctx->tex.recs.p;
    ctx->sc.textureCount = (uint32_t)count;
    ctx->sc.srgbLut = (const float*)ctx->tex.srgbLut.p;
    ctx->counts.TextureCount = count;
    ctx->accumulatedSamples = 0;
    return IDKPT_OK;
}

IDKPT_API int idkpt_resize(IdkPtCtx* ctx, int32_t width, int32_t height) {
    if (!ctx) return IDKPT_ERR_INVALID_ARGUMENT;
    DRAIN_PENDING("idkpt_resize");
    if (width <= 0 || height <= 0 || width > 16384 || height > 16384) return fail(ctx, IDKPT_ERR_INVALID_ARGUMENT, "idkpt_resize: invalid size");
    if (ctx->globalSlots && ctx->tileCount > 1 && (height + ctx->stripeH - 1) / ctx->stripeH > IDK_MAX_STRIPES)
        return fail(ctx, IDKPT_ERR_UNSUPPORTED, "idkpt_resize: IDKPT_CREATE_GLOBAL_SLOTS supports at most 4096 stripes");
    CK(cudaSetDevice(ctx->device));
    CK(cudaStreamSynchronize(ctx->stream));
    if (ctx->copyPending) { CK(cudaEventSynchronize(ctx->copyDone)); ctx->copyPending = false; }
    gather_teardown(ctx);
    ctx->haveDenoised = false;
    for (int i = 0; i < 4; i++) release(ctx->oidn[i]);
    release(ctx->denoiseWork[0]); release(ctx->denoiseWork[1]); release(ctx->denoised);
    ctx->width = width;
    ctx->height = height;
    compute_tile_rows(ctx);
    int rc = allocate_wavefront(ctx);
    if (rc) return rc;
    for (int i = 0; i < IDK_MAX_LANES; i++) {
        release(ctx->lanes[i].keys);
        release(ctx->lanes[i].keysTmp);
        release(ctx->lanes[i].sortedAlive);
    }
    ctx->accumulatedSamples = 0;
    return IDKPT_OK;
}

IDKPT_API int idkpt_reset_accumulation(IdkPtCtx* ctx) {
    if (!ctx) return IDKPT_ERR_INVALID_ARGUMENT;
    ctx->accumulatedSamples = 0;
    return IDKPT_OK;
}

IDKPT_API uint32_t idkpt_accumulated_samples(IdkPtCtx* ctx) { return ctx ? ctx->accumulatedSamples : 0; }

IDKPT_API int idkpt_set_accumulated_samples(IdkPtCtx* ctx, uint32_t n) {
    if (!ctx) return IDKPT_ERR_INVALID_ARGUMENT;
    ctx->accumulatedSamples = n;
    return IDKPT_OK;
}

struct EventPool {
    IdkPtCtx* ctx;
    size_t used = 0;
    struct Span { size_t a, b; int cat; int bounce; };
    std::vector<Span> spans;
    bool enabled;
    cudaEvent_t get() {
        if (used == ctx->events.size()) {
            cudaEvent_t e;
            cudaEventCreate(&e);
            ctx->events.push_back(e);
        }
        return ctx->events[used++];
    }
    size_t begin() {
        if (!enabled) return 0;
        size_t i = used;
        cudaEventRecord(get(), ctx->stream);
        return i;
    }
    void end(size_t a, int cat, int bounce = -1) {
        if (!enabled) return;
        size_t i = used;
        cudaEventRecord(get(), ctx->stream);
        spans.push_back({a, i, cat, bounce});
    }
};

IDKPT_API int idkpt_stream_handle(IdkPtCtx* ctx, void** stream) {
    if (!ctx || !stream) return IDKPT_ERR_INVALID_ARGUMENT;
    *stream = (void*)ctx->stream;
    return IDKPT_OK;
}

IDKPT_API int idkpt_sync(IdkPtCtx* ctx) {
    if (!ctx) return IDKPT_ERR_INVALID_ARGUMENT;
    CK(cudaSetDevice(ctx->device));
    return check_device_errors(ctx, drain(ctx), "idkpt_sync");
}

IDKPT_API int idkpt_compute(IdkPtCtx* ctx, const GpuPerFrameData* frame, const IdkPtSettings* st, IdkPtStats* stats) {
    if (!ctx || !frame || !st) return fail(ctx, IDKPT_ERR_INVALID_ARGUMENT, "idkpt_compute: null argument");
    if (!ctx->haveScene) return fail(ctx, IDKPT_ERR_NO_SCENE, "idkpt_compute: idkpt_set_scene has not been called");
    if (st->RayDepth < 1 || st->RayDepth > IDKPT_MAX_RAY_DEPTH) return fail(ctx, IDKPT_ERR_INVALID_ARGUMENT, "idkpt_compute: RayDepth out of range");
    if (st->SamplesPerPixel < 1) return fail(ctx, IDKPT_ERR_INVALID_ARGUMENT, "idkpt_compute: SamplesPerPixel must be >= 1");
    CK(cudaSetDevice(ctx->device));
    if (stats) memset(stats, 0, sizeof(*stats));
    const uint32_t n = ctx->nLocal;
    if (n == 0) { ctx->accumulatedSamples += st->SamplesPerPixel; return IDKPT_OK; }

    const bool wantStats = st->CollectStats != 0 || st->Gpu.DoDebugBVHTraversal != 0;
    const bool sorting = st->DoRaySorting != 0;
    const bool aovs = st->OutputAOVs != 0;
    const bool async = stats == nullptr && !wantStats && !ctx->exportEnabled && ctx->laneCount > 1;
    const bool globalSlots = ctx->globalSlots && ctx->tileCount > 1;
    if (globalSlots && ctx->gatherWorld < 2)
        return fail(ctx, IDKPT_ERR_INVALID_ARGUMENT, "idkpt_compute: IDKPT_CREATE_GLOBAL_SLOTS needs the peers connected (idkpt_gather_import / idkpt_gather_connect)");
    if (globalSlots && sorting)
        return fail(ctx, IDKPT_ERR_UNSUPPORTED, "idkpt_compute: ray sorting reorders the slots by a tile-local key sort; not available with IDKPT_CREATE_GLOBAL_SLOTS");
    if (!async && ctx->asyncPending) {
        int rc = check_device_errors(ctx, drain(ctx), "idkpt_compute");
        if (rc) return rc;
    }

    FrameParams f;
    memcpy(f.invProj, frame->InvProjection, sizeof(f.invProj));
    memcpy(f.invView, frame->InvView, sizeof(f.invView));
    memcpy(f.viewPos, frame->ViewPos, sizeof(f.viewPos));
    f.focalLength = st->Gpu.FocalLength;
    f.lenseRadius = st->Gpu.LenseRadius;
    f.width = ctx->width; f.height = ctx->height;
    f.stripeH = ctx->stripeH; f.tileIndex = ctx->tileIndex; f.tileCount = ctx->tileCount;
    f.doDebugTraversal = st->Gpu.DoDebugBVHTraversal;
    f.doTraceLights = st->Gpu.DoTraceLights;
    f.doRussianRoulette = st->Gpu.DoRussianRoulette;

    EventPool ev{ctx, 0, {}, stats != nullptr};
    const size_t evTotal = ev.begin();
    uint32_t launches = 0, traverseLaunches = 0;
    std::vector<uint32_t> hostCounts(stats ? (size_t)st->SamplesPerPixel * (IDKPT_MAX_RAY_DEPTH + 1) : 0, 0);
    DevBuf& countLog = ctx->countLog;
    if (stats) CK(ensure(countLog, hostCounts.size() * sizeof(uint32_t)));
    if (wantStats) CK(cudaMemsetAsync(ctx->counters.p, 0, sizeof(TraceCounters), ctx->stream));

    const dim3 rgGrid((ctx->width + 7) / 8, (ctx->height + 7) / 8), rgBlock(8, 8);
    const int accBlocks = std::min<int>((int)((n + IDK_BLOCK - 1) / IDK_BLOCK), ctx->smCount * 8);

    for (int s = 0; s < st->SamplesPerPixel; s++) {
        Lane& ln = ctx->lanes[async ? ctx->nextLane : 0];
        if (async) {
            ctx->nextLane = (ctx->nextLane + 1) % ctx->laneCount;
            if (!ln.allocated)
                for (int i = 0; i < ctx->laneCount; i++)
                    if (!ctx->lanes[i].allocated) { int rc = allocate_lane(ctx, ctx->lanes[i]); if (rc) return rc; }
            if (ln.accPending) CK(cudaStreamWaitEvent(ln.stream, ln.accDone, 0));
        }
        const cudaStream_t ls = async ? ln.stream : ctx->stream;
        if (sorting) {
            CK(ensure(ln.keys, (size_t)n * 4));
            CK(ensure(ln.keysTmp, (size_t)n * 4));
            CK(ensure(ln.sortedAlive, (size_t)n * 4));
            if (idk_sort_prepare(ln.sortScratch, n)) return fail(ctx, IDKPT_ERR_OUT_OF_MEMORY, "idkpt_compute: sort scratch allocation failed");
        }
        uint32_t* counts = (uint32_t*)ln.countsDev.p;
        uint32_t* tickets = (uint32_t*)ln.tickets.p;
        f.accumulatedSamples = ctx->accumulatedSamples;
        k_init_sample<<<1, 256, 0, ls>>>(counts, IDKPT_MAX_RAY_DEPTH + 1, tickets, 2 * (IDKPT_MAX_RAY_DEPTH + 1), n);
        launches++;

        size_t e0 = ev.begin();
        k_raygen<<<rgGrid, rgBlock, 0, ls>>>(f, (PathState*)ln.state.p);
        ev.end(e0, 3);
        launches++;

        for (int j = 0; j < st->RayDepth; j++) {
            const bool first = j == 0;
            const bool last = j == st->RayDepth - 1;
            const uint32_t* alive = first ? nullptr : (const uint32_t*)ln.alive[j & 1].p;
            if (sorting && j > 1) {
                e0 = ev.begin();
                int nl = idk_sort_by_key(ln.sortScratch, (const uint32_t*)ln.keys.p, alive, (uint32_t*)ln.sortedAlive.p, counts + j, n, ctx->smCount, ls);
                ev.end(e0, 2);
                if (nl < 0) return fail(ctx, IDKPT_ERR_CUDA, "idkpt_compute: sort launch failed");
                launches += (uint32_t)nl;
                alive = (const uint32_t*)ln.sortedAlive.p;
            }

            if (globalSlots && !first) {
                SlotExchangeArgs xa;
                memset(&xa, 0, sizeof(xa));
                if (++ln.slotEpoch == 0u) ln.slotEpoch = 2u;
                const uint32_t epoch = ln.slotEpoch;
                const size_t laneIdx = (size_t)(&ln - ctx->lanes);
                for (int p = 0; p < ctx->gatherWorld; p++)
                    xa.peerTable[p] = (unsigned long long*)ctx->peerSlotTable[p] + (laneIdx * 2 + (epoch & 1u)) * (size_t)ctx->nStripes;
                xa.alive = alive; xa.count = counts + j;
                xa.delta = (uint32_t*)ln.slotDelta.p;
                xa.timedOut = (uint32_t*)ctx->gatherScratch.p + 1;
                xa.timeoutCycles = (long long)(ctx->gatherTimeoutMs * (double)ctx->clockKHz);
                xa.epoch = epoch;
                xa.world = ctx->gatherWorld; xa.rank = ctx->gatherRank;
                xa.stripePixels = (uint32_t)ctx->stripeH * (uint32_t)ctx->width;
                xa.nLocalStripes = (uint32_t)ctx->nLocalStripes; xa.nStripes = (uint32_t)ctx->nStripes;
                k_slot_exchange<<<1, 256, 0, ls>>>(xa);
                launches++;
            }

            TraverseArgs ta;
            ta.sc = ctx->sc;
            ta.state = (const PathState*)ln.state.p;
            ta.perm = alive;
            ta.count = counts + j;
            ta.ticket = tickets + 2 * j;
            ta.hits = (HitRec*)ln.hits.p;
            ta.hitXform = (uint32_t*)ln.hitXform.p;
            ta.debugCost = (float*)ln.debugCost.p;
            ta.counters = (TraceCounters*)ctx->counters.p;
            ta.traceLights = st->Gpu.DoTraceLights;
            ta.bounce = j;
            e0 = ev.begin();
            if (first) {
                if (wantStats) k_traverse<true><<<ctx->traverse1BlocksStats, IDK_BLOCK, ctx->stackBytes, ls>>>(ta);
                else k_traverse<false><<<async ? ctx->traverse1BlocksLane : ctx->traverse1Blocks, IDK_BLOCK, ctx->stackBytes, ls>>>(ta);
            } else {
                const int tb = async ? ctx->traverseBlocksLane : ctx->traverseBlocks;
                const TraverseTuning tune = {IDK_T2_SETUP_THRESHOLD, IDK_T2_LEAF_THRESHOLD, async ? 1 : 0};
                if (ctx->sc.useTlas) {
                    if (wantStats) k_traverse2<true, true><<<ctx->traverseBlocksStats, IDK_T2_BLOCK, ctx->traverse2Smem, ls>>>(ta, tune);
                    else k_traverse2<false, true><<<tb, IDK_T2_BLOCK, ctx->traverse2Smem, ls>>>(ta, tune);
                } else {
                    if (wantStats) k_traverse2<true, false><<<ctx->traverseBlocksStats, IDK_T2_BLOCK, ctx->traverse2Smem, ls>>>(ta, tune);
                    else k_traverse2<false, false><<<tb, IDK_T2_BLOCK, ctx->traverse2Smem, ls>>>(ta, tune);
                }
            }
            ev.end(e0, 0, j);
            launches++;
            traverseLaunches++;

            ShadeArgs sa;
            sa.sc = ctx->sc;
            sa.f = f;
            sa.state = (PathState*)ln.state.p;
            sa.aov = (float4*)ln.aov.p;
            sa.alive = alive;
            sa.hits = (const HitRec*)ln.hits.p;
            sa.hitXform = (const uint32_t*)ln.hitXform.p;
            sa.debugCost = (const float*)ln.debugCost.p;
            sa.count = counts + j;
            sa.survivors = (uint32_t*)ln.survivors.p;
            sa.keysTmp = sorting ? (uint32_t*)ln.keysTmp.p : nullptr;
            sa.radiance = (float4*)ln.radiance.p;
            sa.aovAlbedoFinal = (float4*)ln.aovAlbedoFinal.p;
            sa.aovNormalFinal = (float4*)ln.aovNormalFinal.p;
            sa.slotDelta = (globalSlots && !first) ? (const uint32_t*)ln.slotDelta.p : nullptr;
            sa.stripePixels = (uint32_t)ctx->stripeH * (uint32_t)ctx->width;
            sa.exportState = ctx->exportEnabled ? 1 : 0;
            sa.firstHit = first ? 1 : 0;
            sa.lastBounce = last ? 1 : 0;
            sa.outputAovs = aovs ? 1 : 0;
            e0 = ev.begin();
            if (ctx->sc.textureCount) k_shade<true><<<ctx->shadeBlocks, IDK_BLOCK, 0, ls>>>(sa);
            else k_shade<false><<<ctx->shadeBlocks, IDK_BLOCK, 0, ls>>>(sa);
            launches++;
            if (!last) {
                CompactArgs ca;
                ca.survivors = (const uint32_t*)ln.survivors.p;
                ca.keysTmp = sorting ? (const uint32_t*)ln.keysTmp.p : nullptr;
                ca.count = counts + j;
                ca.aliveOut = (uint32_t*)ln.alive[(j + 1) & 1].p;
                ca.keysOut = sorting ? (uint32_t*)ln.keys.p : nullptr;
                ca.countOut = counts + j + 1;
                ca.ticket = tickets + 2 * j + 1;
                ca.tileStatus = (unsigned long long*)ln.tileStatus.p;
                if (ln.epoch >= IDK_EPOCH_MASK) {
                    CK(cudaMemsetAsync(ln.tileStatus.p, 0, ln.tileStatus.bytes, ls));
                    ln.epoch = 0;
                }
                ca.epoch = ++ln.epoch;
                const size_t ec = ev.begin();
                k_compact<<<ctx->compactBlocks, IDK_BLOCK, 0, ls>>>(ca);
                ev.end(ec, 5);
                launches++;
            }
            ev.end(e0, 1, j);
        }

        if (async) {
            CK(cudaEventRecord(ln.radianceReady, ls));
            CK(cudaStreamWaitEvent(ctx->stream, ln.radianceReady, 0));
        }
        e0 = ev.begin();
        const bool gatherNow = ctx->gatherWorld > 1 && s == st->SamplesPerPixel - 1;
        if (gatherNow) {
            const int b = (int)((ctx->gatherEpoch + 1) & 1u);
            GatherArgs g;
            memset(&g, 0, sizeof(g));
            for (int p = 0; p < ctx->gatherWorld; p++) { g.peerImage[p] = (float4*)ctx->peerImage[b][p]; g.peerFlags[p] = (uint32_t*)ctx->peerFlags[b][p]; }
            g.tileRows = (const int*)ctx->gatherRows.p;
            g.doneCounter = (uint32_t*)ctx->gatherScratch.p;
            g.world = ctx->gatherWorld; g.rank = ctx->gatherRank; g.width = ctx->width;
            g.epoch = ++ctx->gatherEpoch;
            CK(cudaMemsetAsync(ctx->gatherScratch.p, 0, 4, ctx->stream));
            k_accumulate_scatter<<<accBlocks, IDK_BLOCK, 0, ctx->stream>>>((const float4*)ln.radiance.p, (float4*)ctx->images[0].p, n,
                                                                           ctx->accumulatedSamples, st->Gpu.DoDebugBVHTraversal, g);
            if (aovs)
                k_accumulate_aov<<<accBlocks, IDK_BLOCK, 0, ctx->stream>>>((const float4*)ln.aovAlbedoFinal.p, (const float4*)ln.aovNormalFinal.p,
                                                                           (float4*)ctx->images[1].p, (float4*)ctx->images[2].p, n, ctx->accumulatedSamples);
            if (async) { CK(cudaEventRecord(ln.accDone, ctx->stream)); ln.accPending = true; }
            k_gather_wait<<<1, 32, 0, ctx->stream>>>((const uint32_t*)ctx->gatherFlags[b].p, ctx->gatherWorld, g.epoch, (uint32_t*)ctx->gatherScratch.p + 1,
                                                     (long long)(ctx->gatherTimeoutMs * (double)ctx->clockKHz));
            ctx->gatherCurrent = b;
            launches += aovs ? 3 : 2;
        } else {
            k_accumulate<<<accBlocks, IDK_BLOCK, 0, ctx->stream>>>((const float4*)ln.radiance.p, (const float4*)ln.aovAlbedoFinal.p,
                                                                   (const float4*)ln.aovNormalFinal.p, (float4*)ctx->images[0].p,
                                                                   (float4*)ctx->images[1].p, (float4*)ctx->images[2].p, n,
                                                                   ctx->accumulatedSamples, st->Gpu.DoDebugBVHTraversal, aovs ? 1 : 0);
            if (async) { CK(cudaEventRecord(ln.accDone, ctx->stream)); ln.accPending = true; }
            launches++;
        }
        ev.end(e0, 3);
        ev.end(e0, 6);
        if (stats) CK(cudaMemcpyAsync((uint32_t*)countLog.p + (size_t)s * (IDKPT_MAX_RAY_DEPTH + 1), counts,
                                      (IDKPT_MAX_RAY_DEPTH + 1) * sizeof(uint32_t), cudaMemcpyDeviceToDevice, ctx->stream));
        ctx->accumulatedSamples++;
    }
    ev.end(evTotal, 4);
    CK(cudaGetLastError());
    if (async) {
        ctx->asyncPending = true;
        return IDKPT_OK;
    }
    {
        int rc = check_device_errors(ctx, cudaStreamSynchronize(ctx->stream), "idkpt_compute");
        if (rc) return rc;
    }
    if (stats) {
        CK(cudaMemcpy(hostCounts.data(), countLog.p, hostCounts.size() * sizeof(uint32_t), cudaMemcpyDeviceToHost));
        for (int s = 0; s < st->SamplesPerPixel; s++)
            for (int j = 0; j < st->RayDepth; j++) {
                const uint64_t c = hostCounts[(size_t)s * (IDKPT_MAX_RAY_DEPTH + 1) + j];
                stats->BounceRays[j] += c;
                stats->Rays += c;
            }
        if (wantStats) {
            TraceCounters tc;
            CK(cudaMemcpy(&tc, ctx->counters.p, sizeof(tc), cudaMemcpyDeviceToHost));
            stats->NodePairFetches = tc.steps;
            stats->TriangleTests = tc.tris;
            stats->InstanceVisits = tc.instances;
            stats->Hits = tc.hits;
            for (int j = 0; j < IDKPT_MAX_RAY_DEPTH; j++) stats->BounceMaxSteps[j] = tc.maxSteps[j];
        }
        for (const EventPool::Span& sp : ev.spans) {
            float ms = 0.0f;
            cudaEventElapsedTime(&ms, ctx->events[sp.a], ctx->events[sp.b]);
            switch (sp.cat) {
                case 0: stats->TraverseMs += ms; if (sp.bounce >= 0) stats->BounceTraverseMs[sp.bounce] += ms; break;
                case 1: stats->ShadeMs += ms; if (sp.bounce >= 0) stats->BounceShadeMs[sp.bounce] += ms; break;
                case 2: stats->SortMs += ms; break;
                case 3: stats->OtherMs += ms; break;
                case 5: stats->CompactMs += ms; break;
                case 6: stats->AccumulateMs += ms; break;
                default: stats->TotalMs = ms; break;
            }
        }
        stats->KernelLaunches = launches;
        stats->TraverseLaunches = traverseLaunches;
    }
    return IDKPT_OK;
}

static int image_copy(IdkPtCtx* ctx, IdkPtImage which, void* host, uint64_t bytes, bool toHost) {
    if (!ctx || !host) return fail(ctx, IDKPT_ERR_INVALID_ARGUMENT, "idkpt image copy: null argument");
    if (which == IDKPT_IMAGE_DENOISED) {
        if (!toHost || !ctx->haveDenoised) return fail(ctx, IDKPT_ERR_INVALID_ARGUMENT, "idkpt image copy: no denoised image (call idkpt_denoise)");
        if (bytes < (uint64_t)ctx->width * ctx->height * 16) return fail(ctx, IDKPT_ERR_INVALID_ARGUMENT, "idkpt image copy: buffer smaller than width*height*16");
        CK(cudaSetDevice(ctx->device));
        CK(cudaMemcpyAsync(host, ctx->denoised.p, (size_t)ctx->width * ctx->height * 16, cudaMemcpyDeviceToHost, ctx->stream));
        CK(cudaStreamSynchronize(ctx->stream));
        return IDKPT_OK;
    }
    if ((int)which < 0 || (int)which > 2) return fail(ctx, IDKPT_ERR_INVALID_ARGUMENT, "idkpt image copy: unknown image");
    if (bytes < (uint64_t)ctx->width * ctx->height * 16) return fail(ctx, IDKPT_ERR_INVALID_ARGUMENT, "idkpt image copy: buffer smaller than width*height*16");
    CK(cudaSetDevice(ctx->device));
    const size_t rowBytes = (size_t)ctx->width * 16;
    size_t i = 0;
    while (i < ctx->rows.size()) {
        size_t j = i;
        while (j + 1 < ctx->rows.size() && ctx->rows[j + 1] == ctx->rows[j] + 1) j++;
        char* h = (char*)host + (size_t)ctx->rows[i] * rowBytes;
        char* d = (char*)ctx->images[which].p + i * rowBytes;
        if (toHost) CK(cudaMemcpyAsync(h, d, (j - i + 1) * rowBytes, cudaMemcpyDeviceToHost, ctx->stream));
        else CK(cudaMemcpyAsync(d, h, (j - i + 1) * rowBytes, cudaMemcpyHostToDevice, ctx->stream));
        i = j + 1;
    }
    CK(cudaStreamSynchronize(ctx->stream));
    return IDKPT_OK;
}

IDKPT_API int idkpt_read_result(IdkPtCtx* ctx, IdkPtImage which, void* dst, uint64_t bytes) { return image_copy(ctx, which, dst, bytes, true); }
IDKPT_API int idkpt_write_result(IdkPtCtx* ctx, IdkPtImage which, const void* src, uint64_t bytes) { return image_copy(ctx, which, (void*)src, bytes, false); }

IDKPT_API int idkpt_present_async(IdkPtCtx* ctx, IdkPtImage which, void* dstHost, uint64_t bytes) {
    if (!ctx || !dstHost) return fail(ctx, IDKPT_ERR_INVALID_ARGUMENT, "idkpt_present_async: null argument");
    if ((int)which < 0 || (int)which > 3) return fail(ctx, IDKPT_ERR_INVALID_ARGUMENT, "idkpt_present_async: unknown image");
    if (bytes < (uint64_t)ctx->width * ctx->height * 16) return fail(ctx, IDKPT_ERR_INVALID_ARGUMENT, "idkpt_present_async: buffer smaller than width*height*16");
    CK(cudaSetDevice(ctx->device));
    const bool gathered = (int)which == 3;
    if (gathered && (ctx->gatherWorld < 2 || ctx->gatherCurrent < 0)) return fail(ctx, IDKPT_ERR_INVALID_ARGUMENT, "idkpt_present_async: no gathered frame yet");
    if (!ctx->copyStream) {
        CK(cudaStreamCreateWithFlags(&ctx->copyStream, cudaStreamNonBlocking));
        CK(cudaEventCreateWithFlags(&ctx->snapDone, cudaEventDisableTiming));
        CK(cudaEventCreateWithFlags(&ctx->copyDone, cudaEventDisableTiming));
    }
    const size_t n = gathered ? (size_t)ctx->width * ctx->height * 16 : (size_t)ctx->nLocal * 16;
    CK(ensure(ctx->presentSnap, std::max<size_t>(n, 16)));
    if (ctx->copyPending) CK(cudaStreamWaitEvent(ctx->stream, ctx->copyDone, 0));
    CK(cudaMemcpyAsync(ctx->presentSnap.p, gathered ? ctx->gatherImage[ctx->gatherCurrent].p : ctx->images[which].p, n, cudaMemcpyDeviceToDevice, ctx->stream));
    CK(cudaEventRecord(ctx->snapDone, ctx->stream));
    CK(cudaStreamWaitEvent(ctx->copyStream, ctx->snapDone, 0));
    const size_t rowBytes = (size_t)ctx->width * 16;
    if (gathered) {
        CK(cudaMemcpyAsync(dstHost, ctx->presentSnap.p, n, cudaMemcpyDeviceToHost, ctx->copyStream));
    } else if (!ctx->rows.empty()) {
        const size_t stripeBytes = (size_t)ctx->stripeH * rowBytes;
        const size_t fullStripes = ctx->rows.size() / (size_t)ctx->stripeH, tailRows = ctx->rows.size() % (size_t)ctx->stripeH;
        char* h0 = (char*)dstHost + (size_t)ctx->rows[0] * rowBytes;
        if (fullStripes)
            CK(cudaMemcpy2DAsync(h0, stripeBytes * (size_t)ctx->tileCount, ctx->presentSnap.p, stripeBytes, stripeBytes, fullStripes,
                                 cudaMemcpyDeviceToHost, ctx->copyStream));
        if (tailRows)
            CK(cudaMemcpyAsync((char*)dstHost + (size_t)ctx->rows[fullStripes * ctx->stripeH] * rowBytes, (char*)ctx->presentSnap.p + fullStripes * stripeBytes,
                               tailRows * rowBytes, cudaMemcpyDeviceToHost, ctx->copyStream));
    }
    CK(cudaEventRecord(ctx->copyDone, ctx->copyStream));
    ctx->copyPending = true;
    return IDKPT_OK;
}

IDKPT_API int idkpt_present_wait(IdkPtCtx* ctx) {
    if (!ctx) return IDKPT_ERR_INVALID_ARGUMENT;
    if (ctx->copyPending) {
        CK(cudaSetDevice(ctx->device));
        CK(cudaEventSynchronize(ctx->copyDone));
        ctx->copyPending = false;
    }
    return IDKPT_OK;
}

IDKPT_API int idkpt_register_host_buffer(IdkPtCtx* ctx, void* hostPtr, uint64_t bytes) {
    if (!ctx || !hostPtr || !bytes) return fail(ctx, IDKPT_ERR_INVALID_ARGUMENT, "idkpt_register_host_buffer: null argument");
    CK(cudaSetDevice(ctx->device));
    CK(cudaHostRegister(hostPtr, bytes, cudaHostRegisterPortable));
    return IDKPT_OK;
}

IDKPT_API int idkpt_unregister_host_buffer(IdkPtCtx* ctx, void* hostPtr) {
    if (!ctx || !hostPtr) return fail(ctx, IDKPT_ERR_INVALID_ARGUMENT, "idkpt_unregister_host_buffer: null argument");
    CK(cudaSetDevice(ctx->device));
    if (ctx->copyPending) { CK(cudaEventSynchronize(ctx->copyDone)); ctx->copyPending = false; }
    CK(cudaHostUnregister(hostPtr));
    return IDKPT_OK;
}

__global__ void k_denoise_import(const float* __restrict__ rgb, float4* __restrict__ out, int count);
static int preload_kernels(IdkPtCtx* ctx) {
    cudaFuncAttributes fa;
#define IDK_PRELOAD(k) CK(cudaFuncGetAttributes(&fa, k))
    IDK_PRELOAD(k_init_sample); IDK_PRELOAD(k_prepare_triangles); IDK_PRELOAD(k_prepare_vertices); IDK_PRELOAD(k_prepare_surfaces);
    IDK_PRELOAD(k_raygen); IDK_PRELOAD(k_traverse<false>); IDK_PRELOAD(k_traverse<true>);
    IDK_PRELOAD((k_traverse2<false, false>)); IDK_PRELOAD((k_traverse2<true, false>));
    IDK_PRELOAD((k_traverse2<false, true>)); IDK_PRELOAD((k_traverse2<true, true>));
    IDK_PRELOAD(k_shade<false>); IDK_PRELOAD(k_shade<true>); IDK_PRELOAD(k_compact); IDK_PRELOAD(k_slot_exchange);
    IDK_PRELOAD(k_accumulate); IDK_PRELOAD(k_accumulate_aov); IDK_PRELOAD(k_accumulate_scatter); IDK_PRELOAD(k_gather_wait);
    IDK_PRELOAD(k_sort_histogram); IDK_PRELOAD(k_sort_scan); IDK_PRELOAD(k_sort_scatter);
    IDK_PRELOAD(k_trace_rays); IDK_PRELOAD(k_trace_rays_any); IDK_PRELOAD(k_shadows_ray_traced);
    IDK_PRELOAD(k_skin_vertices); IDK_PRELOAD(k_refit_prepare); IDK_PRELOAD(k_refit_climb); IDK_PRELOAD(k_tlas_build);
    IDK_PRELOAD(k_bloom_down); IDK_PRELOAD(k_bloom_up); IDK_PRELOAD(k_agx_matrices); IDK_PRELOAD(k_tonemap);
    IDK_PRELOAD(k_denoise_prepare); IDK_PRELOAD(k_denoise_atrous); IDK_PRELOAD(k_denoise_finish); IDK_PRELOAD(k_denoise_import);
    IDK_PRELOAD(k_bcn_decode); IDK_PRELOAD(k_point_shadow_faces); IDK_PRELOAD(k_volumetric_march); IDK_PRELOAD(k_volumetric_upscale);
    IDK_PRELOAD(k_ssao); IDK_PRELOAD(k_deferred_lighting); IDK_PRELOAD(k_ssr); IDK_PRELOAD(k_taa_resolve);
    IDK_PRELOAD(k_shading_rate); IDK_PRELOAD(k_vrs_scan); IDK_PRELOAD(k_deferred_lighting_vrs); IDK_PRELOAD(k_gbuffer);
    IDK_PRELOAD(k_transparency<false>); IDK_PRELOAD(k_transparency<true>); IDK_PRELOAD(k_lights_skybox);
#undef IDK_PRELOAD
    return IDKPT_OK;
}

static size_t slot_table_words(const IdkPtCtx* ctx) { return (size_t)IDK_MAX_LANES * 2 * (size_t)std::max(1, ctx->nStripes); }
static int gather_allocate(IdkPtCtx* ctx) {
    { int rc = preload_kernels(ctx); if (rc) return rc; }
    const size_t imgBytes = (size_t)ctx->width * ctx->height * 16;
    for (int b = 0; b < 2; b++) {
        CK(ensure(ctx->gatherImage[b], imgBytes));
        CK(ensure(ctx->gatherFlags[b], IDK_MAX_PEERS * sizeof(uint32_t)));
        CK(cudaMemsetAsync(ctx->gatherImage[b].p, 0, imgBytes, ctx->stream));
        CK(cudaMemsetAsync(ctx->gatherFlags[b].p, 0, IDK_MAX_PEERS * sizeof(uint32_t), ctx->stream));
    }
    if (ctx->laneCount > 1)
        for (int i = 0; i < ctx->laneCount; i++)
            if (!ctx->lanes[i].allocated) { int rc = allocate_lane(ctx, ctx->lanes[i]); if (rc) return rc; }
    CK(ensure(ctx->slotTable, slot_table_words(ctx) * sizeof(unsigned long long)));
    CK(cudaMemsetAsync(ctx->slotTable.p, 0, ctx->slotTable.bytes, ctx->stream));
    CK(ensure(ctx->gatherScratch, 16));
    CK(cudaMemsetAsync(ctx->gatherScratch.p, 0, 16, ctx->stream));
    CK(ensure(ctx->gatherRows, std::max<size_t>(ctx->rows.size(), 1) * sizeof(int)));
    if (!ctx->rows.empty()) CK(cudaMemcpyAsync(ctx->gatherRows.p, ctx->rows.data(), ctx->rows.size() * sizeof(int), cudaMemcpyHostToDevice, ctx->stream));
    CK(cudaStreamSynchronize(ctx->stream));
    return IDKPT_OK;
}

IDKPT_API int idkpt_gather_export(IdkPtCtx* ctx, void* handlesOut, uint64_t bytes) {
    if (!ctx || !handlesOut) return fail(ctx, IDKPT_ERR_INVALID_ARGUMENT, "idkpt_gather_export: null argument");
    DRAIN_PENDING("idkpt_gather_export");
    if (bytes < IDKPT_GATHER_HANDLE_BYTES) return fail(ctx, IDKPT_ERR_INVALID_ARGUMENT, "idkpt_gather_export: need IDKPT_GATHER_HANDLE_BYTES (320) bytes");
    CK(cudaSetDevice(ctx->device));
    { int rc = gather_allocate(ctx); if (rc) return rc; }
    cudaIpcMemHandle_t* out = (cudaIpcMemHandle_t*)handlesOut;
    for (int b = 0; b < 2; b++) {
        CK(cudaIpcGetMemHandle(&out[b], ctx->gatherImage[b].p));
        CK(cudaIpcGetMemHandle(&out[2 + b], ctx->gatherFlags[b].p));
    }
    CK(cudaIpcGetMemHandle(&out[4], ctx->slotTable.p));
    return IDKPT_OK;
}

IDKPT_API int idkpt_gather_import(IdkPtCtx* ctx, int32_t rank, int32_t world, const void* allHandles, uint64_t bytes) {
    if (!ctx || !allHandles) return fail(ctx, IDKPT_ERR_INVALID_ARGUMENT, "idkpt_gather_import: null argument");
    DRAIN_PENDING("idkpt_gather_import");
    if (world < 2 || world > IDK_MAX_PEERS || rank < 0 || rank >= world) return fail(ctx, IDKPT_ERR_INVALID_ARGUMENT, "idkpt_gather_import: invalid rank / world");
    if (world != ctx->tileCount || rank != ctx->tileIndex) return fail(ctx, IDKPT_ERR_INVALID_ARGUMENT, "idkpt_gather_import: rank / world must equal TileIndex / TileCount");
    if (bytes < (uint64_t)world * IDKPT_GATHER_HANDLE_BYTES) return fail(ctx, IDKPT_ERR_INVALID_ARGUMENT, "idkpt_gather_import: handle buffer too small");
    if (!ctx->gatherImage[0].p) return fail(ctx, IDKPT_ERR_INVALID_ARGUMENT, "idkpt_gather_import: call idkpt_gather_export first");
    if (ctx->gatherWorld > 1) return fail(ctx, IDKPT_ERR_INVALID_ARGUMENT, "idkpt_gather_import: peers are already connected (idkpt_resize disconnects them)");
    CK(cudaSetDevice(ctx->device));
    const cudaIpcMemHandle_t* hs = (const cudaIpcMemHandle_t*)allHandles;
    ctx->peerIsIpc = true;
    for (int p = 0; p < world; p++) {
        for (int b = 0; b < 2; b++) {
            if (p == rank) {
                ctx->peerImage[b][p] = ctx->gatherImage[b].p;
                ctx->peerFlags[b][p] = ctx->gatherFlags[b].p;
            } else {
                CK(cudaIpcOpenMemHandle(&ctx->peerImage[b][p], hs[5 * p + b], cudaIpcMemLazyEnablePeerAccess));
                CK(cudaIpcOpenMemHandle(&ctx->peerFlags[b][p], hs[5 * p + 2 + b], cudaIpcMemLazyEnablePeerAccess));
            }
        }
        if (p == rank) ctx->peerSlotTable[p] = ctx->slotTable.p;
        else CK(cudaIpcOpenMemHandle(&ctx->peerSlotTable[p], hs[5 * p + 4], cudaIpcMemLazyEnablePeerAccess));
        ctx->peerMapped[p] = true;
    }
    ctx->gatherWorld = world;
    ctx->gatherRank = rank;
    ctx->gatherEpoch = 0;
    ctx->gatherCurrent = -1;
    for (int i = 0; i < IDK_MAX_LANES; i++) ctx->lanes[i].slotEpoch = ctx->slotEpochStart;
    return IDKPT_OK;
}

IDKPT_API int idkpt_gather_connect(IdkPtCtx** ctxs, int32_t world) {
    if (!ctxs || world < 2 || world > IDK_MAX_PEERS) return fail(ctxs && world > 0 ? ctxs[0] : nullptr, IDKPT_ERR_INVALID_ARGUMENT, "idkpt_gather_connect: invalid argument");
    for (int r = 0; r < world; r++) {
        IdkPtCtx* ctx = ctxs[r];
        if (!ctx) return fail(ctxs[0], IDKPT_ERR_INVALID_ARGUMENT, "idkpt_gather_connect: null context");
        if (ctx->tileCount != world || ctx->tileIndex != r) return fail(ctx, IDKPT_ERR_INVALID_ARGUMENT, "idkpt_gather_connect: context r must have TileIndex r and TileCount world");
        if (ctx->width != ctxs[0]->width || ctx->height != ctxs[0]->height || ctx->stripeH != ctxs[0]->stripeH || ctx->laneCount != ctxs[0]->laneCount ||
            ctx->globalSlots != ctxs[0]->globalSlots)
            return fail(ctx, IDKPT_ERR_INVALID_ARGUMENT, "idkpt_gather_connect: contexts differ in size, stripe height, lanes or flags");
        DRAIN_PENDING("idkpt_gather_connect");
        if (ctx->gatherWorld > 1) return fail(ctx, IDKPT_ERR_INVALID_ARGUMENT, "idkpt_gather_connect: peers are already connected");
        CK(cudaSetDevice(ctx->device));
        int rc = gather_allocate(ctx);
        if (rc) return rc;
    }
    for (int r = 0; r < world; r++) {
        IdkPtCtx* ctx = ctxs[r];
        CK(cudaSetDevice(ctx->device));
        for (int p = 0; p < world; p++) {
            if (ctxs[p]->device != ctx->device) {
                int can = 0;
                CK(cudaDeviceCanAccessPeer(&can, ctx->device, ctxs[p]->device));
                if (!can) return fail(ctx, IDKPT_ERR_UNSUPPORTED, "idkpt_gather_connect: no peer access between two of the devices");
                const cudaError_t e = cudaDeviceEnablePeerAccess(ctxs[p]->device, 0);
                if (e == cudaErrorPeerAccessAlreadyEnabled) cudaGetLastError();
                else CK(e);
            }
            for (int b = 0; b < 2; b++) {
                ctx->peerImage[b][p] = ctxs[p]->gatherImage[b].p;
                ctx->peerFlags[b][p] = ctxs[p]->gatherFlags[b].p;
            }
            ctx->peerSlotTable[p] = ctxs[p]->slotTable.p;
            ctx->peerMapped[p] = true;
        }
        ctx->peerIsIpc = false;
        ctx->gatherWorld = world;
        ctx->gatherRank = r;
        ctx->gatherEpoch = 0;
        ctx->gatherCurrent = -1;
        for (int i = 0; i < IDK_MAX_LANES; i++) ctx->lanes[i].slotEpoch = ctx->slotEpochStart;
    }
    return IDKPT_OK;
}

IDKPT_API int idkpt_gather_device_ptr(IdkPtCtx* ctx, void** devPtr, uint64_t* bytes) {
    if (!ctx || !devPtr) return fail(ctx, IDKPT_ERR_INVALID_ARGUMENT, "idkpt_gather_device_ptr: null argument");
    DRAIN_PENDING("idkpt_gather_device_ptr");
    if (ctx->gatherWorld < 2 || ctx->gatherCurrent < 0) return fail(ctx, IDKPT_ERR_INVALID_ARGUMENT, "idkpt_gather_device_ptr: no gathered frame yet");
    *devPtr = ctx->gatherImage[ctx->gatherCurrent].p;
    if (bytes) *bytes = (uint64_t)ctx->width * ctx->height * 16;
    return IDKPT_OK;
}

IDKPT_API int idkpt_result_device_ptr(IdkPtCtx* ctx, IdkPtImage which, void** devPtr, uint64_t* bytes) {
    if (!ctx || !devPtr || (int)which < 0 || (int)which > 2) return fail(ctx, IDKPT_ERR_INVALID_ARGUMENT, "idkpt_result_device_ptr: invalid argument");
    DRAIN_PENDING("idkpt_result_device_ptr");
    *devPtr = ctx->images[which].p;
    if (bytes) *bytes = (uint64_t)ctx->nLocal * 16;
    return IDKPT_OK;
}

IDKPT_API int idkpt_tile_rows(IdkPtCtx* ctx, int32_t* rowCount, int32_t* rowsOut, int32_t capacity) {
    if (!ctx || !rowCount) return IDKPT_ERR_INVALID_ARGUMENT;
    *rowCount = (int32_t)ctx->rows.size();
    if (rowsOut) for (int i = 0; i < capacity && i < (int)ctx->rows.size(); i++) rowsOut[i] = ctx->rows[i];
    return IDKPT_OK;
}

IDKPT_API int idkpt_read_wavefront_rays(IdkPtCtx* ctx, GpuWavefrontRay* dst, uint64_t count) {
    if (!ctx) return IDKPT_ERR_INVALID_ARGUMENT;
    DRAIN_PENDING("idkpt_read_wavefront_rays");
    if (!dst) {
        ctx->exportEnabled = count != 0;
        return IDKPT_OK;
    }
    if (!ctx->exportEnabled) return fail(ctx, IDKPT_ERR_INVALID_ARGUMENT, "idkpt_read_wavefront_rays: arm the export first (dst = NULL, count = 1) and call idkpt_compute");
    if (count < (uint64_t)ctx->width * ctx->height) return fail(ctx, IDKPT_ERR_INVALID_ARGUMENT, "idkpt_read_wavefront_rays: buffer smaller than width*height");
    CK(cudaSetDevice(ctx->device));
    std::vector<PathState> tmp(ctx->nLocal);
    CK(cudaMemcpyAsync(tmp.data(), ctx->lanes[0].state.p, (size_t)ctx->nLocal * sizeof(PathState), cudaMemcpyDeviceToHost, ctx->stream));
    CK(cudaStreamSynchronize(ctx->stream));
    for (size_t i = 0; i < ctx->rows.size(); i++) {
        for (int x = 0; x < ctx->width; x++) {
            const PathState& s = tmp[i * (size_t)ctx->width + x];
            GpuWavefrontRay& w = dst[(size_t)ctx->rows[i] * ctx->width + x];
            w.Origin[0] = s.ox; w.Origin[1] = s.oy; w.Origin[2] = s.oz; w.PreviousIOROrTraverseCost = s.prevIor;
            w.Throughput[0] = s.tx; w.Throughput[1] = s.ty; w.Throughput[2] = s.tz; w.PackedDirectionX = s.pdx;
            w.Radiance[0] = s.rx; w.Radiance[1] = s.ry; w.Radiance[2] = s.rz; w.PackedDirectionY = s.pdy;
        }
    }
    return IDKPT_OK;
}


static inline int ilogb_int(int v) { int r = 0; while (v > 1) { v >>= 1; r++; } return r; }

IDKPT_API int idkpt_post_process(IdkPtCtx* ctx, const IdkPtPostSettings* s, IdkPtImage source, uint8_t* rgba8Out, float* kernelMs) {
    if (!ctx || !s) return fail(ctx, IDKPT_ERR_INVALID_ARGUMENT, "idkpt_post_process: null argument");
    if (kernelMs) *kernelMs = 0.0f;
    const int w = ctx->width, h = ctx->height;
    const float4* src = nullptr;
    if (source == IDKPT_IMAGE_GATHERED) {
        if (ctx->gatherWorld < 2 || ctx->gatherCurrent < 0) return fail(ctx, IDKPT_ERR_INVALID_ARGUMENT, "idkpt_post_process: no gathered frame yet");
        src = (const float4*)ctx->gatherImage[ctx->gatherCurrent].p;
    } else if (source == IDKPT_IMAGE_DENOISED) {
        if (!ctx->haveDenoised) return fail(ctx, IDKPT_ERR_INVALID_ARGUMENT, "idkpt_post_process: no denoised image (call idkpt_denoise)");
        src = (const float4*)ctx->denoised.p;
    } else if ((int)source >= 0 && (int)source <= 2) {
        if (ctx->tileCount != 1) return fail(ctx, IDKPT_ERR_INVALID_ARGUMENT, "idkpt_post_process: a tiled context holds only its own rows; use IDKPT_IMAGE_GATHERED");
        src = (const float4*)ctx->images[source].p;
    } else return fail(ctx, IDKPT_ERR_INVALID_ARGUMENT, "idkpt_post_process: unknown image");
    if (s->IsBloom && (w < 2 || h < 2)) return fail(ctx, IDKPT_ERR_INVALID_ARGUMENT, "idkpt_post_process: bloom needs an image of at least 2x2");
    if (s->IsBloom && (s->BloomMinusLods < 0 || s->BloomMinusLods > 30)) return fail(ctx, IDKPT_ERR_INVALID_ARGUMENT, "idkpt_post_process: BloomMinusLods out of range");
    CK(cudaSetDevice(ctx->device));
    CK(ensure(ctx->ldr, (size_t)w * h * 4));
    CK(ensure(ctx->postConsts, sizeof(PostTonemapConsts)));
    const dim3 blk(256);
    auto grid = [](int gw, int gh) { return dim3((unsigned)((gw + 31) / 32), (unsigned)((gh + 7) / 8)); };
    return run_timed(ctx, "idkpt_post_process", kernelMs, [&]() -> int {
        PostImage bloomResult = {nullptr, nullptr, 0, 0};
        if (s->IsBloom) {
            const int w2 = w / 2, h2 = h / 2;
            const int levels = std::max(ilogb_int(std::max(w2, h2)) + 1 - s->BloomMinusLods, 2);
            std::vector<size_t> off(levels + 1, 0);
            std::vector<int> lw(levels), lh(levels);
            for (int l = 0; l < levels; l++) {
                lw[l] = std::max(1, w2 / (1 << std::min(l, 30))); lh[l] = std::max(1, h2 / (1 << std::min(l, 30)));
                off[l + 1] = off[l] + (size_t)lw[l] * lh[l];
            }
            cudaError_t ce = ensure(ctx->bloomDown, off[levels] * 8);
            if (ce == cudaSuccess) ce = ensure(ctx->bloomUp, off[levels - 1] * 8);
            if (ce != cudaSuccess) return fail(ctx, IDKPT_ERR_OUT_OF_MEMORY, "idkpt_post_process: bloom allocation failed");
            uint2* down = (uint2*)ctx->bloomDown.p;
            uint2* up = (uint2*)ctx->bloomUp.p;
            for (int l = 0; l < levels; l++) {
                BloomDownArgs a;
                a.src = l == 0 ? PostImage{src, nullptr, w, h} : PostImage{nullptr, down + off[l - 1], lw[l - 1], lh[l - 1]};
                a.dst = down + off[l]; a.dw = lw[l]; a.dh = lh[l];
                a.prefilter = l == 0; a.maxColor = s->BloomMaxColor; a.threshold = s->BloomThreshold;
                k_bloom_down<<<grid(a.dw, a.dh), blk, 0, ctx->stream>>>(a);
            }
            for (int l = levels - 2; l >= 0; l--) {
                BloomUpArgs a;
                a.up = l == levels - 2 ? PostImage{nullptr, down + off[l + 1], lw[l + 1], lh[l + 1]} : PostImage{nullptr, up + off[l + 1], lw[l + 1], lh[l + 1]};
                a.down = PostImage{nullptr, down + off[l + 1], lw[l + 1], lh[l + 1]};
                a.dst = up + off[l]; a.dw = lw[l]; a.dh = lh[l];
                k_bloom_up<<<grid(a.dw, a.dh), blk, 0, ctx->stream>>>(a);
            }
            bloomResult = PostImage{nullptr, up, lw[0], lh[0]};
        }
        k_agx_matrices<<<1, 1, 0, ctx->stream>>>(s->Exposure, s->Compression, (PostTonemapConsts*)ctx->postConsts.p);
        TonemapArgs t;
        t.src0 = PostImage{src, nullptr, w, h};
        t.src1 = bloomResult;
        t.dst = (uchar4*)ctx->ldr.p; t.w = w; t.h = h;
        t.saturation = s->Saturation; t.linear = s->Linear; t.peak = s->Peak; t.doTonemap = s->DoTonemapAndSrgbTransform ? 1 : 0;
        t.consts = (const PostTonemapConsts*)ctx->postConsts.p;
        k_tonemap<<<grid(w, h), blk, 0, ctx->stream>>>(t);
        return IDKPT_OK;
    }, rgba8Out, ctx->ldr.p, (size_t)w * h * 4);
}

IDKPT_API int idkpt_ldr_device_ptr(IdkPtCtx* ctx, void** devPtr, uint64_t* bytes) {
    if (!ctx || !devPtr) return fail(ctx, IDKPT_ERR_INVALID_ARGUMENT, "idkpt_ldr_device_ptr: null argument");
    DRAIN_PENDING("idkpt_ldr_device_ptr");
    if (!ctx->ldr.p) return fail(ctx, IDKPT_ERR_INVALID_ARGUMENT, "idkpt_ldr_device_ptr: call idkpt_post_process first");
    *devPtr = ctx->ldr.p;
    if (bytes) *bytes = (uint64_t)ctx->width * ctx->height * 4;
    return IDKPT_OK;
}

static int denoise_alloc(IdkPtCtx* ctx) {
    const size_t n = (size_t)ctx->width * ctx->height;
    for (int i = 0; i < 4; i++) CK(ensure(ctx->oidn[i], n * 12));
    for (int i = 0; i < 2; i++) CK(ensure(ctx->denoiseWork[i], n * 16));
    CK(ensure(ctx->denoised, n * 16));
    return IDKPT_OK;
}

IDKPT_API int idkpt_denoise(IdkPtCtx* ctx, const IdkPtDenoiseSettings* s, float* kernelMs) {
    if (!ctx || !s) return fail(ctx, IDKPT_ERR_INVALID_ARGUMENT, "idkpt_denoise: null argument");
    if (kernelMs) *kernelMs = 0.0f;
    if (ctx->tileCount != 1) return fail(ctx, IDKPT_ERR_UNSUPPORTED, "idkpt_denoise: the AOV images of a tiled context hold only its own rows");
    if (s->Iterations < 0 || s->Iterations > 12 || !(s->SigmaColor > 0.0f) || !(s->SigmaNormal > 0.0f) || !(s->SigmaAlbedo > 0.0f))
        return fail(ctx, IDKPT_ERR_INVALID_ARGUMENT, "idkpt_denoise: Iterations must be 0..12 and the sigmas positive");
    DRAIN_PENDING("idkpt_denoise");
    CK(cudaSetDevice(ctx->device));
    int rc = denoise_alloc(ctx);
    if (rc) return rc;
    const int w = ctx->width, h = ctx->height, n = w * h;
    rc = run_timed(ctx, "idkpt_denoise", kernelMs, [&]() -> int {
        DenoisePrepareArgs pa;
        pa.result = (const float4*)ctx->images[0].p; pa.albedo = (const float4*)ctx->images[1].p; pa.normal = (const float4*)ctx->images[2].p;
        pa.oidnBeauty = (float*)ctx->oidn[0].p; pa.oidnAlbedo = (float*)ctx->oidn[1].p; pa.oidnNormal = (float*)ctx->oidn[2].p;
        pa.work = (float4*)ctx->denoiseWork[0].p; pa.count = n; pa.demodulate = s->Demodulate ? 1 : 0;
        k_denoise_prepare<<<(n + 255) / 256, 256, 0, ctx->stream>>>(pa);
        int cur = 0;
        for (int it = 0; it < s->Iterations; it++) {
            const int step = 1 << it;
            const float sc = s->SigmaColor / (float)step;
            DenoiseAtrousArgs a;
            a.in = (const float4*)ctx->denoiseWork[cur].p; a.out = (float4*)ctx->denoiseWork[cur ^ 1].p;
            a.albedo = pa.albedo; a.normal = pa.normal; a.w = w; a.h = h; a.step = step;
            a.invSigmaColor2 = 1.0f / (sc * sc); a.invSigmaNormal2 = 1.0f / (s->SigmaNormal * s->SigmaNormal);
            a.invSigmaAlbedo2 = 1.0f / (s->SigmaAlbedo * s->SigmaAlbedo); a.invStep2 = 1.0f / ((float)step * (float)step);
            k_denoise_atrous<<<dim3((unsigned)((w + 31) / 32), (unsigned)((h + 7) / 8)), 256, 0, ctx->stream>>>(a);
            cur ^= 1;
        }
        if (s->Iterations > 0) {
            DenoiseFinishArgs fa;
            fa.filtered = (const float4*)ctx->denoiseWork[cur].p; fa.albedo = pa.albedo; fa.denoised = (float4*)ctx->denoised.p;
            fa.oidnOutput = (float*)ctx->oidn[3].p; fa.count = n; fa.demodulate = pa.demodulate;
            k_denoise_finish<<<(n + 255) / 256, 256, 0, ctx->stream>>>(fa);
        }
        return IDKPT_OK;
// ... 964 lines not shown
```

Baseline: 2149.

## Fuse raygen, first-hit traversal and first-bounce shading into one kernel

Replaces the separate raygen, first-bounce traverse and first-bounce shade launches with a single persistent first-hit kernel. Camera rays are generated in registers, traced, and shaded directly, without writing PathState and hit records to global memory and reading them back. The TLAS path is also selected at compile time through a template parameter. In exchange the fused kernel carries a larger register footprint and more template variants, which may lower occupancy or hurt coherence in the first-hit trace.

```diff
diff --git a/idkengine_b200/csrc/idk_kernels.cuh b/idkengine_b200/csrc/idk_kernels.cuh
--- a/idkengine_b200/csrc/idk_kernels.cuh
+++ b/idkengine_b200/csrc/idk_kernels.cuh
@@ -1,5 +1,6 @@
 #pragma once
 #include "idk_device.cuh"
+#include "idk_reorder.h"
 #include "../../include/idk_gpu_types.h"
 
 #define IDK_BLOCK 256
@@ -194,7 +195,8 @@
     return true;
 }
 
-template <bool STATS, bool ANY, class Accept = AcceptAll>
+enum TlasMode { TLAS_OFF = 0, TLAS_ON = 1, TLAS_RUNTIME = 2 };
+template <bool STATS, bool ANY, class Accept = AcceptAll, int TLAS = TLAS_RUNTIME>
 __device__ __forceinline__ bool trace_ray(const DeviceScene& sc, f3 o, f3 d, float tMax, bool traceLights,
                                           uint32_t* stack, HitRec& hit, uint32_t& hitXform, uint32_t& S, uint32_t& T, uint32_t& I, float& cost,
                                           const Accept& accept = Accept()) {
@@ -217,7 +219,7 @@
         }
     }
 
-    if (sc.useTlas) {
+    if (TLAS == TLAS_ON || (TLAS == TLAS_RUNTIME && sc.useTlas)) {
         const f3 inv = mk3(1.0f / d.x, 1.0f / d.y, 1.0f / d.z);
         uint32_t tstack[IDK_TLAS_STACK_SIZE];
         uint32_t sp = 0, top = 0;
@@ -272,56 +274,6 @@
     int traceLights;
     int bounce;
 };
-
-template <bool STATS>
-__global__ void __launch_bounds__(IDK_BLOCK) k_traverse(TraverseArgs a) {
-    extern __shared__ uint32_t s_stack[];
-    uint32_t* stack = s_stack + threadIdx.x;
-    const uint32_t lane = threadIdx.x & 31;
-    const uint32_t count = *a.count;
-    uint32_t S = 0, T = 0, I = 0, H = 0;
-    for (;;) {
-        uint32_t base = 0;
-        if (lane == 0) base = atomicAdd(a.ticket, 32u);
-        base = __shfl_sync(0xffffffffu, base, 0);
-        if (base >= count) break;
-        const uint32_t gid = base + lane;
-        if (gid < count) {
-            const uint32_t src = a.perm ? a.perm[gid] : gid;
-            const float4* sp = reinterpret_cast<const float4*>(a.state + src);
-            const float4 s0 = sp[0], s1 = sp[1];
-            const f3 o = mk3(s0.x, s0.y, s0.z);
-            const f3 d = decode_unit_vec(s1.x, s1.y);
-            HitRec hit;
-            uint32_t xf;
-            float cost = 0.0f;
-            const uint32_t stepsBefore = S;
-            trace_ray<STATS, false>(a.sc, o, d, IDK_FLOAT_MAX, a.traceLights != 0, stack, hit, xf, S, T, I, cost);
-            if (STATS) atomicMax(&a.counters->maxSteps[a.bounce & 63], S - stepsBefore);
-            reinterpret_cast<float4*>(a.hits)[gid] = make_float4(hit.bx, hit.by, hit.t, __uint_as_float(hit.tri));
-            a.hitXform[gid] = xf;
-            if (STATS) {
-                a.debugCost[gid] = cost;
-                if (hit.tri != ~0u) H++;
-            }
-        }
-    }
-    if (STATS) {
-        for (int off = 16; off > 0; off >>= 1) {
-            S += __shfl_down_sync(0xffffffffu, S, off);
-            T += __shfl_down_sync(0xffffffffu, T, off);
-            I += __shfl_down_sync(0xffffffffu, I, off);
-            H += __shfl_down_sync(0xffffffffu, H, off);
-        }
-        if (lane == 0) {
-            atomicAdd(&a.counters->steps, (unsigned long long)S);
-            atomicAdd(&a.counters->tris, (unsigned long long)T);
-            atomicAdd(&a.counters->instances, (unsigned long long)I);
-            atomicAdd(&a.counters->hits, (unsigned long long)H);
-        }
-    }
-}
-
 
 struct TraverseTuning { int setupThreshold; int leafThreshold; int packRays; };
 #define IDK_T2_SETUP_THRESHOLD 12
@@ -612,31 +564,16 @@
     int doDebugTraversal, doTraceLights, doRussianRoulette;
 };
 
-__device__ __forceinline__ bool tile_owns_row(const FrameParams& f, int y, int& localRow) {
-    const int stripe = y / f.stripeH;
-    if (f.tileCount > 1 && (stripe % f.tileCount) != f.tileIndex) return false;
-    localRow = (f.tileCount > 1 ? (stripe / f.tileCount) : stripe) * f.stripeH + (y % f.stripeH);
-    return true;
-}
-
-__global__ void __launch_bounds__(64) k_raygen(FrameParams f, PathState* __restrict__ state) {
-    const uint32_t n = 20;
-    const uint32_t idx = blockIdx.y * gridDim.x + blockIdx.x;
-    const uint32_t columnSize = gridDim.y * n;
-    const uint32_t fullColumnCount = gridDim.x / n;
-    const uint32_t lastColumnWidth = gridDim.x % n;
-    const uint32_t columnIdx = idx / columnSize;
-    const uint32_t idxInColumn = idx % columnSize;
-    uint32_t columnWidth = n;
-    if (columnIdx == fullColumnCount) columnWidth = lastColumnWidth;
-    const uint32_t swy = idxInColumn / columnWidth;
-    const uint32_t swx = idxInColumn % columnWidth + columnIdx * n;
-    const int x = (int)(swx * 8 + threadIdx.x), y = (int)(swy * 8 + threadIdx.y);
-    if (x >= f.width || y >= f.height) return;
-    int localRow;
-    if (!tile_owns_row(f, y, localRow)) return;
-
-    const uint32_t gidX = blockIdx.x * 8 + threadIdx.x, gidY = blockIdx.y * 8 + threadIdx.y;
+__device__ __forceinline__ int tile_row_y(const FrameParams& f, int localRow) {
+    const int localStripe = localRow / f.stripeH;
+    const int stripe = f.tileCount > 1 ? localStripe * f.tileCount + f.tileIndex : localStripe;
+    return stripe * f.stripeH + localRow % f.stripeH;
+}
+
+__device__ __forceinline__ PathState camera_ray(const FrameParams& f, int x, int y, uint32_t li) {
+    uint32_t bx, by;
+    reorder_invocations_inverse((uint32_t)(f.width + 7) / 8u, (uint32_t)(f.height + 7) / 8u, (uint32_t)x / 8u, (uint32_t)y / 8u, bx, by);
+    const uint32_t gidX = bx * 8 + (uint32_t)x % 8u, gidY = by * 8 + (uint32_t)y % 8u;
     uint32_t seed = (uint32_t)(y * 4096 + x) * (f.accumulatedSamples + 1u);
     const float sx = rnd01(seed), sy = rnd01(seed);
     const float ndcx = ((float)x + sx) / (float)f.width * 2.0f - 1.0f;
@@ -650,14 +587,13 @@
     const f3 pointOnLense = mat4_mul_xyz(f.invView, f.lenseRadius * dx, f.lenseRadius * dy, 0.0f, 1.0f);
     camDir = normalize3(focalPoint - pointOnLense);
 
-    float pdx, pdy;
-    encode_unit_vec(camDir, pdx, pdy);
-    const uint32_t li = (uint32_t)localRow * (uint32_t)f.width + (uint32_t)x;
-    float4* out = reinterpret_cast<float4*>(state + li);
-    out[0] = make_float4(pointOnLense.x, pointOnLense.y, pointOnLense.z, 1.0f);
-    out[1] = make_float4(pdx, pdy, __uint_as_float(li), __uint_as_float(gidY * 4096u + gidX));
-    out[2] = make_float4(1.0f, 1.0f, 1.0f, __uint_as_float(seed));
-    out[3] = make_float4(0.0f, 0.0f, 0.0f, 0.0f);
+    PathState st;
+    st.ox = pointOnLense.x; st.oy = pointOnLense.y; st.oz = pointOnLense.z; st.prevIor = 1.0f;
+    encode_unit_vec(camDir, st.pdx, st.pdy);
+    st.pix = li; st.reseed = gidY * 4096u + gidX;
+    st.tx = 1.0f; st.ty = 1.0f; st.tz = 1.0f; st.rng = seed;
+    st.rx = 0.0f; st.ry = 0.0f; st.rz = 0.0f; st.pad = 0;
+    return st;
 }
 
 struct Surface {
@@ -793,7 +729,6 @@
     const uint32_t* alive;
     const HitRec* hits;
     const uint32_t* hitXform;
-    const float* debugCost;
     const uint32_t* count;
     uint32_t* survivors;
     uint32_t* keysTmp;
@@ -803,7 +738,6 @@
     const uint32_t* slotDelta;
     uint32_t stripePixels;
     int exportState;
-    int firstHit;
     int lastBounce;
     int outputAovs;
 };
@@ -814,250 +748,305 @@
 }
 __device__ __forceinline__ uint32_t status_epoch(unsigned long long sv) { return (uint32_t)(sv >> 34) & IDK_EPOCH_MASK; }
 
+template <bool TEX, bool FIRST>
+__device__ __forceinline__ void shade_ray(const ShadeArgs& a, uint32_t gid, uint32_t src, PathState st, const HitRec& hit, uint32_t hitXf,
+                                          float debugCost) {
+    const DeviceScene& sc = a.sc;
+    const FrameParams& f = a.f;
+    bool survive = false;
+    float4 aov0 = make_float4(0.0f, 0.0f, 0.0f, 1.0f), aov1 = make_float4(0.0f, 0.0f, 0.0f, 0.0f);
+    uint32_t sortingKey = 0;
+    if (a.outputAovs && !FIRST) { aov0 = a.aov[2 * (size_t)src]; aov1 = a.aov[2 * (size_t)src + 1]; }
+    const uint32_t slot = (a.slotDelta && !FIRST) ? gid + a.slotDelta[src / a.stripePixels] : gid;
+    uint32_t rng = FIRST ? st.rng : (slot * 4096u + f.accumulatedSamples);
+    const uint32_t reseed = FIRST ? st.reseed : slot;
+
+    const float hitT = hit.t;
+    const uint32_t hitTri = hit.tri;
+    const bool hitScene = hitT != IDK_FLOAT_MAX;
+    const f3 rayDir = decode_unit_vec(st.pdx, st.pdy);
+    f3 origin = mk3(st.ox, st.oy, st.oz);
+    f3 thr = mk3(st.tx, st.ty, st.tz);
+    f3 rad = mk3(st.rx, st.ry, st.rz);
+
+    if (FIRST && f.doDebugTraversal) {
+        st.prevIor = debugCost;
+        survive = false;
+    } else if (hitScene) {
+        origin = origin + rayDir * hitT;
+        Surface s;
+        s.Albedo = mk3(1.0f, 1.0f, 1.0f); s.Alpha = 1.0f;
+        s.Normal = mk3(0.0f, 0.0f, 0.0f); s.Emissive = mk3(0.0f, 0.0f, 0.0f); s.Absorbance = mk3(0.0f, 0.0f, 0.0f);
+        s.Metallic = 0.0f; s.Roughness = 0.0f; s.Transmission = 0.0f; s.IOR = 1.5f; s.AlphaCutoff = 0.5f;
+        s.IsVolumetric = false; s.TintOnTransmissive = true;
+        f3 geometricNormal = mk3(0.0f, 0.0f, 0.0f);
+        bool passThrough = false;
+        const bool hitLight = hitTri == ~0u;
+        if (!hitLight) {
+            sortingKey = hitTri;
+            const int4 tri = __ldg(sc.blasTris + hitTri);
+            const float4* vf = sc.vtxFrame;
+            const float4 a0 = ldg4(vf + 2 * (size_t)tri.x), a1 = ldg4(vf + 2 * (size_t)tri.x + 1);
+            const float4 c0 = ldg4(vf + 2 * (size_t)tri.y), c1 = ldg4(vf + 2 * (size_t)tri.y + 1);
+            const float4 e0 = ldg4(vf + 2 * (size_t)tri.z), e1 = ldg4(vf + 2 * (size_t)tri.z + 1);
+            const float4* xf = sc.xforms + 9 * (size_t)hitXf + 3;
+            const float4 r0 = ldg4(xf), r1 = ldg4(xf + 1), r2 = ldg4(xf + 2);
+            const float4* sr = sc.surfRec + 5 * (size_t)tri.w;
+            const float4 s0 = ldg4(sr), s1 = ldg4(sr + 1), s2 = ldg4(sr + 2), s3 = ldg4(sr + 3), s4 = ldg4(sr + 4);
+            const float b0 = hit.bx, b1 = hit.by, b2 = 1.0f - hit.bx - hit.by;
+            const f3 interpNormal = normalize3((mk3(a0.x, a0.y, a0.z) * b0 + mk3(c0.x, c0.y, c0.z) * b1) + mk3(e0.x, e0.y, e0.z) * b2);
+            const f3 interpTangent = normalize3((mk3(a0.w, a1.x, a1.y) * b0 + mk3(c0.w, c1.x, c1.y) * b1) + mk3(e0.w, e1.x, e1.y) * b2);
+            const float normalMapStrength = s3.w;
+
+            s.Albedo = mk3(s0.x, s0.y, s0.z);
+            s.Alpha = s0.w;
+            s.Normal = mk3(1.0f, 1.0f, 0.0f);
+            s.Emissive = mk3(s1.x, s1.y, s1.z);
+            s.Metallic = s1.w;
+            s.Absorbance = mk3(s2.x, s2.y, s2.z);
+            s.Roughness = s2.w;
+            s.Transmission = s3.x;
+            s.IOR = s3.y;
+            s.AlphaCutoff = s3.z;
+            s.IsVolumetric = (__float_as_uint(s4.x) & 1u) != 0;
+            s.TintOnTransmissive = (__float_as_uint(s4.x) & 2u) != 0;
+            if (TEX && (__float_as_uint(s4.x) & 4u)) {
+                float tu, tv;
+                interp_texcoord(sc, tri, b0, b1, b2, tu, tv);
+                surface_textured(sc, tri.w, tu, tv, s);
+            }
+
+            const float alphaCutoff = (s.AlphaCutoff == 2.0f) ? rnd01(rng) : s.AlphaCutoff;
+            if (s.Alpha < alphaCutoff) {
+                origin = origin + rayDir * 0.001f;
+                passThrough = true;
+            } else {
+                const f3 worldNormal = normalize3(xform_normal(r0, r1, r2, interpNormal));
+                const f3 worldTangent = normalize3(xform_normal(r0, r1, r2, interpTangent));
+                const f3 N = normalize3(worldNormal);
+                const f3 T = normalize3(worldTangent);
+                const f3 B = normalize3(cross3(N, T));
+                const f3 tbnN = (T * s.Normal.x + B * s.Normal.y) + N * s.Normal.z;
+                s.Normal = normalize3(mix3(worldNormal, tbnN, normalMapStrength));
+                const float4 tr = ldg4(sc.triRec + 4 * (size_t)hitTri + 2);
+                geometricNormal = normalize3(mk3(tr.y, tr.z, tr.w));
+                geometricNormal = normalize3(xform_normal(r0, r1, r2, geometricNormal));
+            }
+        } else if (f.doTraceLights) {
+            sortingKey = hitXf;
+            const GpuLight& L = sc.lights[hitXf];
+            s.Emissive = mk3(L.Color[0], L.Color[1], L.Color[2]);
+            s.Albedo = s.Emissive;
+            s.Normal = (origin - mk3(L.Position[0], L.Position[1], L.Position[2])) / L.Radius;
+            geometricNormal = s.Normal;
+        }
+
+        if (passThrough) {
+            survive = true;
+        } else {
+            float prevIor = FIRST ? 1.0f : st.prevIor;
+            const bool fromInside = dot3(-rayDir, geometricNormal) < 0.0f;
+            if (fromInside) {
+                if (FIRST) prevIor = s.IOR;
+                geometricNormal = geometricNormal * -1.0f;
+                if (s.IsVolumetric) {
+                    const f3 e = -s.Absorbance * hitT;
+                    thr = thr * mk3(det_exp(e.x), det_exp(e.y), det_exp(e.z));
+                }
+            }
+            float cosTheta = dot3(-rayDir, s.Normal);
+            if (cosTheta < 0.0f) s.Normal = s.Normal * -1.0f;
+
+            rad = rad + s.Emissive * thr;
+
+            Surface m = s;
+            m.Roughness *= m.Roughness;
+            cosTheta = dot3(-rayDir, m.Normal);
+            {
+                const float diffuseChance = 1.0f - m.Metallic - m.Transmission;
+                const float r0f = (prevIor - m.IOR) / (prevIor + m.IOR);
+                const float f0 = r0f * r0f;
+                const float fres = f0 + (1.0f - f0) * pow5f(1.0f - cosTheta);
+                m.Metallic = mix1(m.Metallic, 1.0f, fres);
+                m.Transmission = fmaxf(1.0f - diffuseChance - m.Metallic, 0.0f);
+            }
+            uint32_t bsdfType;
+            {
+                const float rnd = rnd01(rng);
+                if (m.Metallic > rnd) bsdfType = 1u;
+                else if (m.Metallic + m.Transmission > rnd) bsdfType = 2u;
+                else bsdfType = 0u;
+            }
+            f3 diffuseRayDir;
+            {
+                uint32_t tmp = reseed;
+                const float g = 1.32471795724474602596f;
+                const float a1 = 1.0f / g, a2 = 1.0f / (g * g);
+                const float r2u = fract1((float)f.accumulatedSamples * a1), r2v = fract1((float)f.accumulatedSamples * a2);
+                const float po0 = rnd01(tmp), po1 = rnd01(tmp);
+                const float u = fract1(r2u + po0), v = fract1(r2v + po1);
+                diffuseRayDir = normalize3(m.Normal + sample_sphere(u, v));
+            }
+            f3 newDir, bsdf;
+            float newIor;
+            if (bsdfType == 0u) {
+                newDir = diffuseRayDir; newIor = prevIor; bsdf = m.Albedo;
+            } else if (bsdfType == 1u) {
+                newDir = normalize3(mix3(reflect3(rayDir, m.Normal), diffuseRayDir, m.Roughness));
+                bsdf = m.Albedo; newIor = prevIor;
+            } else {
+                newIor = fromInside ? 1.0f : m.IOR;
+                f3 refr;
+                bool tir;
+                if (!m.IsVolumetric) {
+                    refr = rayDir; tir = false; newIor = 1.0f;
+                } else {
+                    refr = refract3(rayDir, m.Normal, prevIor / newIor);
+                    tir = refr.x == 0.0f && refr.y == 0.0f && refr.z == 0.0f;
+                    if (tir) { refr = reflect3(rayDir, m.Normal); newIor = prevIor; }
+                }
+                newDir = normalize3(mix3(refr, !tir ? -diffuseRayDir : diffuseRayDir, m.Roughness));
+                const bool gltfWantsTint = m.IsVolumetric || !fromInside;
+                bsdf = (gltfWantsTint && m.TintOnTransmissive) ? m.Albedo : mk3(1.0f, 1.0f, 1.0f);
+            }
+            thr = thr * bsdf;
+
+            if (a.outputAovs) {
+                const float dc = 1.0f - s.Metallic - s.Transmission;
+                const float weight = dc + s.Metallic * s.Roughness + s.Transmission * s.Roughness;
+                if (FIRST) {
+                    const f3 al = s.Albedo * weight, no = s.Normal * weight;
+                    aov0 = make_float4(al.x, al.y, al.z, 1.0f - weight);
+                    aov1 = make_float4(no.x, no.y, no.z, 0.0f);
+                } else {
+                    const f3 al = mk3(aov0.x, aov0.y, aov0.z) + aov0.w * s.Albedo * weight;
+                    const f3 no = mk3(aov1.x, aov1.y, aov1.z) + aov0.w * s.Normal * weight;
+                    aov0 = make_float4(al.x, al.y, al.z, aov0.w * (1.0f - weight));
+                    aov1 = make_float4(no.x, no.y, no.z, 0.0f);
+                }
+            }
+
+            bool terminate = false;
+            if (!FIRST && f.doRussianRoulette) {
+                const float p = fmaxf(thr.x, fmaxf(thr.y, thr.z));
+                if (rnd01(rng) > p) terminate = true;
+                else thr = thr / p;
+            }
+            if (!terminate) {
+                if (bsdfType == 2u) geometricNormal = geometricNormal * -1.0f;
+                origin = origin + geometricNormal * 0.001f;
+                st.prevIor = newIor;
+                encode_unit_vec(newDir, st.pdx, st.pdy);
+                survive = true;
+            }
+        }
+    } else {
+        const f3 albedo = sample_sky(sc, rayDir);
+        if (a.outputAovs) {
+            const f3 fn = cubemap_face_normal(rayDir);
+            if (FIRST) {
+                aov0 = make_float4(albedo.x, albedo.y, albedo.z, 0.0f);
+                aov1 = make_float4(fn.x, fn.y, fn.z, 0.0f);
+            } else {
+                const f3 al = mk3(aov0.x, aov0.y, aov0.z) + aov0.w * albedo;
+                const f3 no = mk3(aov1.x, aov1.y, aov1.z) + aov0.w * fn;
+                aov0 = make_float4(al.x, al.y, al.z, 0.0f);
+                aov1 = make_float4(no.x, no.y, no.z, 0.0f);
+            }
+        }
+        rad = rad + albedo * thr;
+        survive = false;
+    }
+    st.ox = origin.x; st.oy = origin.y; st.oz = origin.z;
+    st.tx = thr.x; st.ty = thr.y; st.tz = thr.z;
+    st.rx = rad.x; st.ry = rad.y; st.rz = rad.z;
+
+    if (!survive || a.lastBounce) {
+        a.radiance[src] = make_float4(st.rx, st.ry, st.rz, st.prevIor);
+        if (a.outputAovs) { a.aovAlbedoFinal[src] = aov0; a.aovNormalFinal[src] = aov1; }
+    }
+    if ((survive && !a.lastBounce) || a.exportState) {
+        float4* op = reinterpret_cast<float4*>(a.state + src);
+        op[0] = make_float4(st.ox, st.oy, st.oz, st.prevIor);
+        op[1] = make_float4(st.pdx, st.pdy, __uint_as_float(src), 0.0f);
+        op[2] = make_float4(st.tx, st.ty, st.tz, 0.0f);
+        op[3] = make_float4(st.rx, st.ry, st.rz, 0.0f);
+        if (a.outputAovs) { a.aov[2 * (size_t)src] = aov0; a.aov[2 * (size_t)src + 1] = aov1; }
+    }
+    if (!a.lastBounce) {
+        a.survivors[gid] = survive ? src : ~0u;
+        if (a.keysTmp) a.keysTmp[gid] = sortingKey & 0x1FFFFFu;
+    }
+}
+
 template <bool TEX>
 __global__ void __launch_bounds__(IDK_BLOCK, 3) k_shade(ShadeArgs a) {
     const uint32_t count = *a.count;
-    const DeviceScene& sc = a.sc;
-    const FrameParams& f = a.f;
-
     for (uint32_t gid = blockIdx.x * blockDim.x + threadIdx.x; gid < count; gid += gridDim.x * blockDim.x) {
-        bool survive = false;
+        const uint32_t src = a.alive[gid];
         PathState st;
-        float4 aov0 = make_float4(0.0f, 0.0f, 0.0f, 1.0f), aov1 = make_float4(0.0f, 0.0f, 0.0f, 0.0f);
-        uint32_t sortingKey = 0;
-        const uint32_t src = a.alive ? a.alive[gid] : gid;
-        {
-            {
-                const float4* sp = reinterpret_cast<const float4*>(a.state + src);
-                float4 v0 = sp[0], v1 = sp[1], v2 = sp[2], v3 = sp[3];
-                st.ox = v0.x; st.oy = v0.y; st.oz = v0.z; st.prevIor = v0.w;
-                st.pdx = v1.x; st.pdy = v1.y; st.pix = __float_as_uint(v1.z); st.reseed = __float_as_uint(v1.w);
-                st.tx = v2.x; st.ty = v2.y; st.tz = v2.z; st.rng = __float_as_uint(v2.w);
-                st.rx = v3.x; st.ry = v3.y; st.rz = v3.z; st.pad = 0;
-            }
-            if (a.outputAovs && !a.firstHit) { aov0 = a.aov[2 * (size_t)src]; aov1 = a.aov[2 * (size_t)src + 1]; }
-            const uint32_t slot = (a.slotDelta && !a.firstHit) ? gid + a.slotDelta[src / a.stripePixels] : gid;
-            uint32_t rng = a.firstHit ? st.rng : (slot * 4096u + f.accumulatedSamples);
-            const uint32_t reseed = a.firstHit ? st.reseed : slot;
-
-            const float4 hv = reinterpret_cast<const float4*>(a.hits)[gid];
-            const float hitT = hv.z;
-            const uint32_t hitTri = __float_as_uint(hv.w);
-            const uint32_t hitXf = a.hitXform[gid];
-            const bool hitScene = hitT != IDK_FLOAT_MAX;
-            const f3 rayDir = decode_unit_vec(st.pdx, st.pdy);
-            f3 origin = mk3(st.ox, st.oy, st.oz);
-            f3 thr = mk3(st.tx, st.ty, st.tz);
-            f3 rad = mk3(st.rx, st.ry, st.rz);
-
-            if (a.firstHit && f.doDebugTraversal) {
-                st.prevIor = a.debugCost[gid];
-                survive = false;
-            } else if (hitScene) {
-                origin = origin + rayDir * hitT;
-                Surface s;
-                s.Albedo = mk3(1.0f, 1.0f, 1.0f); s.Alpha = 1.0f;
-                s.Normal = mk3(0.0f, 0.0f, 0.0f); s.Emissive = mk3(0.0f, 0.0f, 0.0f); s.Absorbance = mk3(0.0f, 0.0f, 0.0f);
-                s.Metallic = 0.0f; s.Roughness = 0.0f; s.Transmission = 0.0f; s.IOR = 1.5f; s.AlphaCutoff = 0.5f;
-                s.IsVolumetric = false; s.TintOnTransmissive = true;
-                f3 geometricNormal = mk3(0.0f, 0.0f, 0.0f);
-                bool passThrough = false;
-                const bool hitLight = hitTri == ~0u;
-                if (!hitLight) {
-                    sortingKey = hitTri;
-                    const int4 tri = __ldg(sc.blasTris + hitTri);
-                    const float4* vf = sc.vtxFrame;
-                    const float4 a0 = ldg4(vf + 2 * (size_t)tri.x), a1 = ldg4(vf + 2 * (size_t)tri.x + 1);
-                    const float4 c0 = ldg4(vf + 2 * (size_t)tri.y), c1 = ldg4(vf + 2 * (size_t)tri.y + 1);
-                    const float4 e0 = ldg4(vf + 2 * (size_t)tri.z), e1 = ldg4(vf + 2 * (size_t)tri.z + 1);
-                    const float4* xf = sc.xforms + 9 * (size_t)hitXf + 3;
-                    const float4 r0 = ldg4(xf), r1 = ldg4(xf + 1), r2 = ldg4(xf + 2);
-                    const float4* sr = sc.surfRec + 5 * (size_t)tri.w;
-                    const float4 s0 = ldg4(sr), s1 = ldg4(sr + 1), s2 = ldg4(sr + 2), s3 = ldg4(sr + 3), s4 = ldg4(sr + 4);
-                    const float b0 = hv.x, b1 = hv.y, b2 = 1.0f - hv.x - hv.y;
-                    const f3 interpNormal = normalize3((mk3(a0.x, a0.y, a0.z) * b0 + mk3(c0.x, c0.y, c0.z) * b1) + mk3(e0.x, e0.y, e0.z) * b2);
-                    const f3 interpTangent = normalize3((mk3(a0.w, a1.x, a1.y) * b0 + mk3(c0.w, c1.x, c1.y) * b1) + mk3(e0.w, e1.x, e1.y) * b2);
-                    const float normalMapStrength = s3.w;
-
-                    s.Albedo = mk3(s0.x, s0.y, s0.z);
-                    s.Alpha = s0.w;
-                    s.Normal = mk3(1.0f, 1.0f, 0.0f);
-                    s.Emissive = mk3(s1.x, s1.y, s1.z);
-                    s.Metallic = s1.w;
-                    s.Absorbance = mk3(s2.x, s2.y, s2.z);
-                    s.Roughness = s2.w;
-                    s.Transmission = s3.x;
-                    s.IOR = s3.y;
-                    s.AlphaCutoff = s3.z;
-                    s.IsVolumetric = (__float_as_uint(s4.x) & 1u) != 0;
-                    s.TintOnTransmissive = (__float_as_uint(s4.x) & 2u) != 0;
-                    if (TEX && (__float_as_uint(s4.x) & 4u)) {
-                        float tu, tv;
-                        interp_texcoord(sc, tri, b0, b1, b2, tu, tv);
-                        surface_textured(sc, tri.w, tu, tv, s);
-                    }
-
-                    const float alphaCutoff = (s.AlphaCutoff == 2.0f) ? rnd01(rng) : s.AlphaCutoff;
-                    if (s.Alpha < alphaCutoff) {
-                        origin = origin + rayDir * 0.001f;
-                        passThrough = true;
-                    } else {
-                        const f3 worldNormal = normalize3(xform_normal(r0, r1, r2, interpNormal));
-                        const f3 worldTangent = normalize3(xform_normal(r0, r1, r2, interpTangent));
-                        const f3 N = normalize3(worldNormal);
-                        const f3 T = normalize3(worldTangent);
-                        const f3 B = normalize3(cross3(N, T));
-                        const f3 tbnN = (T * s.Normal.x + B * s.Normal.y) + N * s.Normal.z;
-                        s.Normal = normalize3(mix3(worldNormal, tbnN, normalMapStrength));
-                        const float4 tr = ldg4(sc.triRec + 4 * (size_t)hitTri + 2);
-                        geometricNormal = normalize3(mk3(tr.y, tr.z, tr.w));
-                        geometricNormal = normalize3(xform_normal(r0, r1, r2, geometricNormal));
-                    }
-                } else if (f.doTraceLights) {
-                    sortingKey = hitXf;
-                    const GpuLight& L = sc.lights[hitXf];
-                    s.Emissive = mk3(L.Color[0], L.Color[1], L.Color[2]);
-                    s.Albedo = s.Emissive;
-                    s.Normal = (origin - mk3(L.Position[0], L.Position[1], L.Position[2])) / L.Radius;
-                    geometricNormal = s.Normal;
-                }
-
-                if (passThrough) {
-                    survive = true;
-                } else {
-                    float prevIor = a.firstHit ? 1.0f : st.prevIor;
-                    const bool fromInside = dot3(-rayDir, geometricNormal) < 0.0f;
-                    if (fromInside) {
-                        if (a.firstHit) prevIor = s.IOR;
-                        geometricNormal = geometricNormal * -1.0f;
-                        if (s.IsVolumetric) {
-                            const f3 e = -s.Absorbance * hitT;
-                            thr = thr * mk3(det_exp(e.x), det_exp(e.y), det_exp(e.z));
-                        }
-                    }
-                    float cosTheta = dot3(-rayDir, s.Normal);
-                    if (cosTheta < 0.0f) s.Normal = s.Normal * -1.0f;
-
-                    rad = rad + s.Emissive * thr;
-
-                    Surface m = s;
-                    m.Roughness *= m.Roughness;
-                    cosTheta = dot3(-rayDir, m.Normal);
-                    {
-                        const float diffuseChance = 1.0f - m.Metallic - m.Transmission;
-                        const float r0f = (prevIor - m.IOR) / (prevIor + m.IOR);
-                        const float f0 = r0f * r0f;
-                        const float fres = f0 + (1.0f - f0) * pow5f(1.0f - cosTheta);
-                        m.Metallic = mix1(m.Metallic, 1.0f, fres);
-                        m.Transmission = fmaxf(1.0f - diffuseChance - m.Metallic, 0.0f);
-                    }
-                    uint32_t bsdfType;
-                    {
-                        const float rnd = rnd01(rng);
-                        if (m.Metallic > rnd) bsdfType = 1u;
-                        else if (m.Metallic + m.Transmission > rnd) bsdfType = 2u;
-                        else bsdfType = 0u;
-                    }
-                    f3 diffuseRayDir;
-                    {
-                        uint32_t tmp = reseed;
-                        const float g = 1.32471795724474602596f;
-                        const float a1 = 1.0f / g, a2 = 1.0f / (g * g);
-                        const float r2u = fract1((float)f.accumulatedSamples * a1), r2v = fract1((float)f.accumulatedSamples * a2);
-                        const float po0 = rnd01(tmp), po1 = rnd01(tmp);
-                        const float u = fract1(r2u + po0), v = fract1(r2v + po1);
-                        diffuseRayDir = normalize3(m.Normal + sample_sphere(u, v));
-                    }
-                    f3 newDir, bsdf;
-                    float newIor;
-                    if (bsdfType == 0u) {
-                        newDir = diffuseRayDir; newIor = prevIor; bsdf = m.Albedo;
-                    } else if (bsdfType == 1u) {
-                        newDir = normalize3(mix3(reflect3(rayDir, m.Normal), diffuseRayDir, m.Roughness));
-                        bsdf = m.Albedo; newIor = prevIor;
-                    } else {
-                        newIor = fromInside ? 1.0f : m.IOR;
-                        f3 refr;
-                        bool tir;
-                        if (!m.IsVolumetric) {
-                            refr = rayDir; tir = false; newIor = 1.0f;
-                        } else {
-                            refr = refract3(rayDir, m.Normal, prevIor / newIor);
-                            tir = refr.x == 0.0f && refr.y == 0.0f && refr.z == 0.0f;
-                            if (tir) { refr = reflect3(rayDir, m.Normal); newIor = prevIor; }
-                        }
-                        newDir = normalize3(mix3(refr, !tir ? -diffuseRayDir : diffuseRayDir, m.Roughness));
-                        const bool gltfWantsTint = m.IsVolumetric || !fromInside;
-                        bsdf = (gltfWantsTint && m.TintOnTransmissive) ? m.Albedo : mk3(1.0f, 1.0f, 1.0f);
-                    }
-                    thr = thr * bsdf;
-
-                    if (a.outputAovs) {
-                        const float dc = 1.0f - s.Metallic - s.Transmission;
-                        const float weight = dc + s.Metallic * s.Roughness + s.Transmission * s.Roughness;
-                        if (a.firstHit) {
-                            const f3 al = s.Albedo * weight, no = s.Normal * weight;
-                            aov0 = make_float4(al.x, al.y, al.z, 1.0f - weight);
-                            aov1 = make_float4(no.x, no.y, no.z, 0.0f);
-                        } else {
-                            const f3 al = mk3(aov0.x, aov0.y, aov0.z) + aov0.w * s.Albedo * weight;
-                            const f3 no = mk3(aov1.x, aov1.y, aov1.z) + aov0.w * s.Normal * weight;
-                            aov0 = make_float4(al.x, al.y, al.z, aov0.w * (1.0f - weight));
-                            aov1 = make_float4(no.x, no.y, no.z, 0.0f);
-                        }
-                    }
-
-                    bool terminate = false;
-                    if (!a.firstHit && f.doRussianRoulette) {
-                        const float p = fmaxf(thr.x, fmaxf(thr.y, thr.z));
-                        if (rnd01(rng) > p) terminate = true;
-                        else thr = thr / p;
-                    }
-                    if (!terminate) {
-                        if (bsdfType == 2u) geometricNormal = geometricNormal * -1.0f;
-                        origin = origin + geometricNormal * 0.001f;
-                        st.prevIor = newIor;
-                        encode_unit_vec(newDir, st.pdx, st.pdy);
-                        survive = true;
-                    }
-                }
-            } else {
-                const f3 albedo = sample_sky(sc, rayDir);
-                if (a.outputAovs) {
-                    const f3 fn = cubemap_face_normal(rayDir);
-                    if (a.firstHit) {
-                        aov0 = make_float4(albedo.x, albedo.y, albedo.z, 0.0f);
-                        aov1 = make_float4(fn.x, fn.y, fn.z, 0.0f);
-                    } else {
-                        const f3 al = mk3(aov0.x, aov0.y, aov0.z) + aov0.w * albedo;
-                        const f3 no = mk3(aov1.x, aov1.y, aov1.z) + aov0.w * fn;
-                        aov0 = make_float4(al.x, al.y, al.z, 0.0f);
-                        aov1 = make_float4(no.x, no.y, no.z, 0.0f);
-                    }
-                }
-                rad = rad + albedo * thr;
-                survive = false;
-            }
-            st.ox = origin.x; st.oy = origin.y; st.oz = origin.z;
-            st.tx = thr.x; st.ty = thr.y; st.tz = thr.z;
-            st.rx = rad.x; st.ry = rad.y; st.rz = rad.z;
-
-            if (!survive || a.lastBounce) {
-                a.radiance[src] = make_float4(st.rx, st.ry, st.rz, st.prevIor);
-                if (a.outputAovs) { a.aovAlbedoFinal[src] = aov0; a.aovNormalFinal[src] = aov1; }
-            }
-            if ((survive && !a.lastBounce) || a.exportState) {
-                float4* op = reinterpret_cast<float4*>(a.state + src);
-                op[0] = make_float4(st.ox, st.oy, st.oz, st.prevIor);
-                op[1] = make_float4(st.pdx, st.pdy, __uint_as_float(src), 0.0f);
-                op[2] = make_float4(st.tx, st.ty, st.tz, 0.0f);
-                op[3] = make_float4(st.rx, st.ry, st.rz, 0.0f);
-                if (a.outputAovs) { a.aov[2 * (size_t)src] = aov0; a.aov[2 * (size_t)src + 1] = aov1; }
-            }
-            if (!a.lastBounce) {
-                a.survivors[gid] = survive ? src : ~0u;
-                if (a.keysTmp) a.keysTmp[gid] = sortingKey & 0x1FFFFFu;
-            }
+        const float4* sp = reinterpret_cast<const float4*>(a.state + src);
+        const float4 v0 = sp[0], v1 = sp[1], v2 = sp[2], v3 = sp[3];
+        st.ox = v0.x; st.oy = v0.y; st.oz = v0.z; st.prevIor = v0.w;
+        st.pdx = v1.x; st.pdy = v1.y; st.pix = __float_as_uint(v1.z); st.reseed = __float_as_uint(v1.w);
+        st.tx = v2.x; st.ty = v2.y; st.tz = v2.z; st.rng = __float_as_uint(v2.w);
+        st.rx = v3.x; st.ry = v3.y; st.rz = v3.z; st.pad = 0;
+        const float4 hv = reinterpret_cast<const float4*>(a.hits)[gid];
+        const HitRec hit = {hv.x, hv.y, hv.z, __float_as_uint(hv.w)};
+        shade_ray<TEX, false>(a, gid, src, st, hit, a.hitXform[gid], 0.0f);
+    }
+}
+
+struct FirstHitArgs {
+    ShadeArgs s;
+    uint32_t* ticket;
+    TraceCounters* counters;
+    uint32_t rows;
+};
+
+template <bool STATS, bool TLAS, bool TEX>
+__global__ void __launch_bounds__(IDK_BLOCK, 3) k_first_hit(FirstHitArgs a) {
+    extern __shared__ uint32_t s_stack[];
+    uint32_t* stack = s_stack + threadIdx.x;
+    const uint32_t lane = threadIdx.x & 31;
+    const FrameParams& f = a.s.f;
+    const uint32_t width = (uint32_t)f.width;
+    const uint32_t blocksX = (width + 7) / 8, blocks = blocksX * ((a.rows + 3) / 4);
+    uint32_t S = 0, T = 0, I = 0, H = 0;
+    for (;;) {
+        uint32_t b = 0;
+        if (lane == 0) b = atomicAdd(a.ticket, 1u);
+        b = __shfl_sync(0xffffffffu, b, 0);
+        if (b >= blocks) break;
+        const uint32_t x = (b % blocksX) * 8 + (lane & 7), row = (b / blocksX) * 4 + (lane >> 3);
+        if (x < width && row < a.rows) {
+            const uint32_t li = row * width + x;
+            const PathState st = camera_ray(f, (int)x, tile_row_y(f, (int)row), li);
+            HitRec hit;
+            uint32_t xf;
+            float cost = 0.0f;
+            const uint32_t stepsBefore = S;
+            trace_ray<STATS, false, AcceptAll, TLAS ? TLAS_ON : TLAS_OFF>(a.s.sc, mk3(st.ox, st.oy, st.oz), decode_unit_vec(st.pdx, st.pdy),
+                                                                         IDK_FLOAT_MAX, f.doTraceLights != 0, stack, hit, xf, S, T, I, cost);
+            if (STATS) {
+                atomicMax(&a.counters->maxSteps[0], S - stepsBefore);
+                if (hit.tri != ~0u) H++;
+            }
+            shade_ray<TEX, true>(a.s, li, li, st, hit, xf, cost);
+        }
+    }
+    if (STATS) {
+        for (int off = 16; off > 0; off >>= 1) {
+            S += __shfl_down_sync(0xffffffffu, S, off);
+            T += __shfl_down_sync(0xffffffffu, T, off);
+            I += __shfl_down_sync(0xffffffffu, I, off);
+            H += __shfl_down_sync(0xffffffffu, H, off);
+        }
+        if (lane == 0) {
+            atomicAdd(&a.counters->steps, (unsigned long long)S);
+            atomicAdd(&a.counters->tris, (unsigned long long)T);
+            atomicAdd(&a.counters->instances, (unsigned long long)I);
+            atomicAdd(&a.counters->hits, (unsigned long long)H);
         }
     }
 }
diff --git a/idkengine_b200/csrc/idk_reorder.h b/idkengine_b200/csrc/idk_reorder.h
--- /dev/null
+++ b/idkengine_b200/csrc/idk_reorder.h
@@ -0,0 +1,18 @@
+#pragma once
+#include <stdint.h>
+
+#if defined(__CUDACC__)
+#define IDK_HD __host__ __device__ __forceinline__
+#else
+#define IDK_HD inline
+#endif
+
+#define IDK_REORDER_COLUMN 20u
+
+IDK_HD void reorder_invocations_inverse(uint32_t gx, uint32_t gy, uint32_t sx, uint32_t sy, uint32_t& bx, uint32_t& by) {
+    const uint32_t columnIdx = sx / IDK_REORDER_COLUMN;
+    const uint32_t columnWidth = columnIdx == gx / IDK_REORDER_COLUMN ? gx % IDK_REORDER_COLUMN : IDK_REORDER_COLUMN;
+    const uint32_t idx = columnIdx * (gy * IDK_REORDER_COLUMN) + sy * columnWidth + sx % IDK_REORDER_COLUMN;
+    bx = idx % gx;
+    by = idx / gx;
+}
diff --git a/idkengine_b200/csrc/idkpt.cu b/idkengine_b200/csrc/idkpt.cu
--- a/idkengine_b200/csrc/idkpt.cu
+++ b/idkengine_b200/csrc/idkpt.cu
@@ -130,8 +130,8 @@
     bool exportEnabled = false;
 
     int traverseBlocks = 0, traverseBlocksStats = 0, shadeBlocks = 0, traceRaysBlocks = 0, compactBlocks = 0;
-    int traverse1Blocks = 0, traverse1BlocksStats = 0;
-    int traverseBlocksLane = 0, traverse1BlocksLane = 0;
+    int firstHitBlocks[2][2] = {};
+    int traverseBlocksLane = 0, firstHitBlocksLane[2] = {};
     size_t stackBytes = 0;
     size_t traverse2Smem = 0;
 
@@ -240,12 +240,15 @@
         if (ctx->tileCount <= 1 || (s % ctx->tileCount) == ctx->tileIndex) ctx->nLocalStripes++;
 }
 
+using FirstHitKernel = void (*)(FirstHitArgs);
+static const FirstHitKernel kFirstHit[2][2][2] = {
+    {{k_first_hit<false, false, false>, k_first_hit<false, false, true>}, {k_first_hit<true, false, false>, k_first_hit<true, false, true>}},
+    {{k_first_hit<false, true, false>, k_first_hit<false, true, true>}, {k_first_hit<true, true, false>, k_first_hit<true, true, true>}}};
+
 static int configure_launches(IdkPtCtx* ctx) {
     const int stackSize = std::max(1, ctx->sc.stackSize);
     ctx->stackBytes = (size_t)stackSize * IDK_BLOCK * sizeof(uint32_t);
     if (ctx->stackBytes > 200 * 1024) return fail(ctx, IDKPT_ERR_UNSUPPORTED, "BlasStackSize too large for the shared-memory traversal stack");
-    CK(cudaFuncSetAttribute(k_traverse<false>, cudaFuncAttributeMaxDynamicSharedMemorySize, (int)ctx->stackBytes));
-    CK(cudaFuncSetAttribute(k_traverse<true>, cudaFuncAttributeMaxDynamicSharedMemorySize, (int)ctx->stackBytes));
     CK(cudaFuncSetAttribute(k_trace_rays, cudaFuncAttributeMaxDynamicSharedMemorySize, (int)ctx->stackBytes));
     CK(cudaFuncSetAttribute(k_trace_rays_any, cudaFuncAttributeMaxDynamicSharedMemorySize, (int)ctx->stackBytes));
     CK(cudaFuncSetAttribute(k_shadows_ray_traced, cudaFuncAttributeMaxDynamicSharedMemorySize, (int)ctx->stackBytes));
@@ -259,10 +262,13 @@
     CK(cudaFuncSetAttribute(k_traverse2<false, true>, cudaFuncAttributeMaxDynamicSharedMemorySize, (int)ctx->traverse2Smem));
     CK(cudaFuncSetAttribute(k_traverse2<true, true>, cudaFuncAttributeMaxDynamicSharedMemorySize, (int)ctx->traverse2Smem));
     int n = 0;
-    CK(cudaOccupancyMaxActiveBlocksPerMultiprocessor(&n, k_traverse<false>, IDK_BLOCK, ctx->stackBytes));
-    ctx->traverse1Blocks = std::max(1, n) * ctx->smCount;
-    CK(cudaOccupancyMaxActiveBlocksPerMultiprocessor(&n, k_traverse<true>, IDK_BLOCK, ctx->stackBytes));
-    ctx->traverse1BlocksStats = std::max(1, n) * ctx->smCount;
+    for (int stats = 0; stats < 2; stats++)
+        for (int tex = 0; tex < 2; tex++) {
+            const FirstHitKernel k = kFirstHit[ctx->sc.useTlas ? 1 : 0][stats][tex];
+            CK(cudaFuncSetAttribute(k, cudaFuncAttributeMaxDynamicSharedMemorySize, (int)ctx->stackBytes));
+            CK(cudaOccupancyMaxActiveBlocksPerMultiprocessor(&n, k, IDK_BLOCK, ctx->stackBytes));
+            ctx->firstHitBlocks[stats][tex] = std::max(1, n) * ctx->smCount;
+        }
     if (ctx->sc.useTlas) {
         CK(cudaOccupancyMaxActiveBlocksPerMultiprocessor(&n, k_traverse2<false, true>, IDK_T2_BLOCK, ctx->traverse2Smem));
         ctx->traverseBlocks = std::max(1, n) * ctx->smCount;
@@ -282,9 +288,10 @@
     ctx->compactBlocks = std::max(1, std::min(n, 4)) * ctx->smCount;
     {
         const int lanes = std::max(1, ctx->laneCount);
-        const int perSm2 = (ctx->traverseBlocks / ctx->smCount + lanes - 1) / lanes, perSm1 = (ctx->traverse1Blocks / ctx->smCount + lanes - 1) / lanes;
+        const int perSm2 = (ctx->traverseBlocks / ctx->smCount + lanes - 1) / lanes;
         ctx->traverseBlocksLane = std::max(1, perSm2) * ctx->smCount;
-        ctx->traverse1BlocksLane = std::max(1, perSm1) * ctx->smCount;
+        for (int tex = 0; tex < 2; tex++)
+            ctx->firstHitBlocksLane[tex] = std::max(1, (ctx->firstHitBlocks[0][tex] / ctx->smCount + lanes - 1) / lanes) * ctx->smCount;
     }
     return IDKPT_OK;
 }
@@ -947,7 +954,6 @@
     if (stats) CK(ensure(countLog, hostCounts.size() * sizeof(uint32_t)));
     if (wantStats) CK(cudaMemsetAsync(ctx->counters.p, 0, sizeof(TraceCounters), ctx->stream));
 
-    const dim3 rgGrid((ctx->width + 7) / 8, (ctx->height + 7) / 8), rgBlock(8, 8);
     const int accBlocks = std::min<int>((int)((n + IDK_BLOCK - 1) / IDK_BLOCK), ctx->smCount * 8);
 
     for (int s = 0; s < st->SamplesPerPixel; s++) {
@@ -972,11 +978,7 @@
         k_init_sample<<<1, 256, 0, ls>>>(counts, IDKPT_MAX_RAY_DEPTH + 1, tickets, 2 * (IDKPT_MAX_RAY_DEPTH + 1), n);
         launches++;
 
-        size_t e0 = ev.begin();
-        k_raygen<<<rgGrid, rgBlock, 0, ls>>>(f, (PathState*)ln.state.p);
-        ev.end(e0, 3);
-        launches++;
-
+        size_t e0 = 0;
         for (int j = 0; j < st->RayDepth; j++) {
             const bool first = j == 0;
             const bool last = j == st->RayDepth - 1;
@@ -1010,23 +1012,49 @@
                 launches++;
             }
 
-            TraverseArgs ta;
-            ta.sc = ctx->sc;
-            ta.state = (const PathState*)ln.state.p;
-            ta.perm = alive;
-            ta.count = counts + j;
-            ta.ticket = tickets + 2 * j;
-            ta.hits = (HitRec*)ln.hits.p;
-            ta.hitXform = (uint32_t*)ln.hitXform.p;
-            ta.debugCost = (float*)ln.debugCost.p;
-            ta.counters = (TraceCounters*)ctx->counters.p;
-            ta.traceLights = st->Gpu.DoTraceLights;
-            ta.bounce = j;
+            ShadeArgs sa;
+            sa.sc = ctx->sc;
+            sa.f = f;
+            sa.state = (PathState*)ln.state.p;
+            sa.aov = (float4*)ln.aov.p;
+            sa.alive = alive;
+            sa.hits = (const HitRec*)ln.hits.p;
+            sa.hitXform = (const uint32_t*)ln.hitXform.p;
+            sa.count = counts + j;
+            sa.survivors = (uint32_t*)ln.survivors.p;
+            sa.keysTmp = sorting ? (uint32_t*)ln.keysTmp.p : nullptr;
+            sa.radiance = (float4*)ln.radiance.p;
+            sa.aovAlbedoFinal = (float4*)ln.aovAlbedoFinal.p;
+            sa.aovNormalFinal = (float4*)ln.aovNormalFinal.p;
+            sa.slotDelta = (globalSlots && !first) ? (const uint32_t*)ln.slotDelta.p : nullptr;
+            sa.stripePixels = (uint32_t)ctx->stripeH * (uint32_t)ctx->width;
+            sa.exportState = ctx->exportEnabled ? 1 : 0;
+            sa.lastBounce = last ? 1 : 0;
+            sa.outputAovs = aovs ? 1 : 0;
+            const int tex = ctx->sc.textureCount ? 1 : 0;
+
             e0 = ev.begin();
             if (first) {
-                if (wantStats) k_traverse<true><<<ctx->traverse1BlocksStats, IDK_BLOCK, ctx->stackBytes, ls>>>(ta);
-                else k_traverse<false><<<async ? ctx->traverse1BlocksLane : ctx->traverse1Blocks, IDK_BLOCK, ctx->stackBytes, ls>>>(ta);
+                FirstHitArgs fa;
+                fa.s = sa;
+                fa.ticket = tickets;
+                fa.counters = (TraceCounters*)ctx->counters.p;
+                fa.rows = n / (uint32_t)ctx->width;
+                const int fb = wantStats ? ctx->firstHitBlocks[1][tex] : async ? ctx->firstHitBlocksLane[tex] : ctx->firstHitBlocks[0][tex];
+                kFirstHit[ctx->sc.useTlas ? 1 : 0][wantStats ? 1 : 0][tex]<<<fb, IDK_BLOCK, ctx->stackBytes, ls>>>(fa);
             } else {
+                TraverseArgs ta;
+                ta.sc = ctx->sc;
+                ta.state = (const PathState*)ln.state.p;
+                ta.perm = alive;
+                ta.count = counts + j;
+                ta.ticket = tickets + 2 * j;
+                ta.hits = (HitRec*)ln.hits.p;
+                ta.hitXform = (uint32_t*)ln.hitXform.p;
+                ta.debugCost = (float*)ln.debugCost.p;
+                ta.counters = (TraceCounters*)ctx->counters.p;
+                ta.traceLights = st->Gpu.DoTraceLights;
+                ta.bounce = j;
                 const int tb = async ? ctx->traverseBlocksLane : ctx->traverseBlocks;
                 const TraverseTuning tune = {IDK_T2_SETUP_THRESHOLD, IDK_T2_LEAF_THRESHOLD, async ? 1 : 0};
                 if (ctx->sc.useTlas) {
@@ -1041,31 +1069,12 @@
             launches++;
             traverseLaunches++;
 
-            ShadeArgs sa;
-            sa.sc = ctx->sc;
-            sa.f = f;
-            sa.state = (PathState*)ln.state.p;
-            sa.aov = (float4*)ln.aov.p;
-            sa.alive = alive;
-            sa.hits = (const HitRec*)ln.hits.p;
-            sa.hitXform = (const uint32_t*)ln.hitXform.p;
-            sa.debugCost = (const float*)ln.debugCost.p;
-            sa.count = counts + j;
-            sa.survivors = (uint32_t*)ln.survivors.p;
-            sa.keysTmp = sorting ? (uint32_t*)ln.keysTmp.p : nullptr;
-            sa.radiance = (float4*)ln.radiance.p;
-            sa.aovAlbedoFinal = (float4*)ln.aovAlbedoFinal.p;
-            sa.aovNormalFinal = (float4*)ln.aovNormalFinal.p;
-            sa.slotDelta = (globalSlots && !first) ? (const uint32_t*)ln.slotDelta.p : nullptr;
-            sa.stripePixels = (uint32_t)ctx->stripeH * (uint32_t)ctx->width;
-            sa.exportState = ctx->exportEnabled ? 1 : 0;
-            sa.firstHit = first ? 1 : 0;
-            sa.lastBounce = last ? 1 : 0;
-            sa.outputAovs = aovs ? 1 : 0;
             e0 = ev.begin();
-            if (ctx->sc.textureCount) k_shade<true><<<ctx->shadeBlocks, IDK_BLOCK, 0, ls>>>(sa);
-            else k_shade<false><<<ctx->shadeBlocks, IDK_BLOCK, 0, ls>>>(sa);
-            launches++;
+            if (!first) {
+                if (tex) k_shade<true><<<ctx->shadeBlocks, IDK_BLOCK, 0, ls>>>(sa);
+                else k_shade<false><<<ctx->shadeBlocks, IDK_BLOCK, 0, ls>>>(sa);
+                launches++;
+            }
             if (!last) {
                 CompactArgs ca;
                 ca.survivors = (const uint32_t*)ln.survivors.p;
@@ -1273,7 +1282,9 @@
     cudaFuncAttributes fa;
 #define IDK_PRELOAD(k) CK(cudaFuncGetAttributes(&fa, k))
     IDK_PRELOAD(k_init_sample); IDK_PRELOAD(k_prepare_triangles); IDK_PRELOAD(k_prepare_vertices); IDK_PRELOAD(k_prepare_surfaces);
-    IDK_PRELOAD(k_raygen); IDK_PRELOAD(k_traverse<false>); IDK_PRELOAD(k_traverse<true>);
+    for (const auto& byStats : kFirstHit)
+        for (const auto& byTex : byStats)
+            for (FirstHitKernel k : byTex) IDK_PRELOAD(k);
     IDK_PRELOAD((k_traverse2<false, false>)); IDK_PRELOAD((k_traverse2<true, false>));
     IDK_PRELOAD((k_traverse2<false, true>)); IDK_PRELOAD((k_traverse2<true, true>));
     IDK_PRELOAD(k_shade<false>); IDK_PRELOAD(k_shade<true>); IDK_PRELOAD(k_compact); IDK_PRELOAD(k_slot_exchange);
```

New measurement: 2288 (median of 6 runs). 1.06x the previous value.
